# xudoong/EdgeVisionTransformer

Hardware: NVIDIA B200
Metric: images_per_sec (higher is better)
Workload: dtype bf16

## Files before the change

### edgevisiontransformer_b200/_lib.py

```python
from __future__ import annotations

import ctypes as C
import os
import threading

HERE = os.path.dirname(os.path.abspath(__file__))
LIB_PATH = os.environ.get("EVT_LIB_PATH") or os.path.join(HERE, "libevt.so")

EVT_OK, EVT_ERR_INVALID, EVT_ERR_CUDA, EVT_ERR_UNSUPPORTED, EVT_ERR_STATE = 0, -1, -2, -3, -4
EVT_F32, EVT_BF16 = 0, 1
ACT_NONE, ACT_GELU_ERF, ACT_GELU_TANH = 0, 1, 2
DIALECT_HF, DIALECT_TF = 0, 1
PREC_BF16, PREC_TF32 = 0, 1
MAX_LAYERS = 64
STAGES = ("embed", "layernorm", "qkv", "attention", "out_proj", "fc1", "fc2", "head")


class ModelSpec(C.Structure):
    _fields_ = [
        ("dialect", C.c_int), ("hidden", C.c_int), ("layers", C.c_int), ("tokens", C.c_int),
        ("image", C.c_int), ("patch", C.c_int), ("head_size", C.c_int), ("num_labels", C.c_int),
        ("act", C.c_int), ("eps", C.c_float),
        ("heads", C.c_int * MAX_LAYERS), ("inter", C.c_int * MAX_LAYERS),
        ("final_ln", C.c_int), ("head_hidden", C.c_int), ("t2t", C.c_int), ("precision", C.c_int), ("embed_k", C.c_int),
        ("head_rows", C.c_int),
    ]


class ForwardOpts(C.Structure):
    _fields_ = [("pixel_dtype", C.c_int), ("pixel_scale", C.c_float * 3), ("pixel_bias", C.c_float * 3),
                ("head_mask", C.c_void_p), ("head_mask_ld", C.c_int), ("ctx_out", C.POINTER(C.c_void_p))]


PIX_F32, PIX_BF16, PIX_U8 = 0, 1, 2


SWIN_MAX_STAGES = 8


class SwinSpec(C.Structure):
    _fields_ = [("image", C.c_int), ("patch", C.c_int), ("window", C.c_int), ("embed_dim", C.c_int), ("stages", C.c_int),
                ("depths", C.c_int * SWIN_MAX_STAGES), ("heads", C.c_int * SWIN_MAX_STAGES), ("num_labels", C.c_int),
                ("eps", C.c_float)]


class TensorView(C.Structure):
    _fields_ = [("name", C.c_char_p), ("data", C.c_void_p), ("ndim", C.c_int), ("shape", C.c_int64 * 4)]


_i, _i64, _f, _p, _sz = C.c_int, C.c_int64, C.c_float, C.c_void_p, C.c_size_t

SIGNATURES = {
    "evt_last_error": (C.c_char_p, []),
    "evt_version": (_i, []),
    "evt_device_check": (_i, []),
    "evt_launch_count": (_i64, []),
    "evt_launch_count_reset": (None, []),
    "evt_gemm_set_pair_mode": (None, [_i]),
    "evt_gemm_set_split_k": (None, [_i]),
    "evt_gemm_weights_static": (None, [_i]),
    "evt_layernorm_fwd": (_i, [_p, _i64, _p, _p, _p, _i, _i64, _p, _i64, _i, _f, _p]),
    "evt_layernorm2d_fwd": (_i, [_p, _p, _p, _p, _p, _i64, _i64, _f, _p]),
    "evt_gemm_bias_act": (_i, [_p, _i64, _p, _i64, _p, _p, _i64, _i, _i, _p, _i, _i64, _i, _i, _i, _i64, _i, _i, _i, _p]),
    "evt_gemm_bias_act_tf32": (_i, [_p, _i64, _p, _i64, _p, _p, _i64, _i, _i, _p, _i64, _i, _i, _i, _i64, _i, _i, _i, _p]),
    "evt_layernorm_gemm": (_i, [_p, _i64, _p, _p, _f, _p, _p, _i64, _p, _p, _i64, _i64, _i, _i, _i, _p]),
    "evt_gemm_residual_layernorm": (_i, [_p, _i64, _p, _i64, _p, _p, _i64, _p, _p, _f, _p, _i64, _i64, _i, _i, _p]),
    "evt_gemm_residual_layernorm_ex": (_i, [_p, _i64, _p, _i64, _p, _p, _i64, _p, _p, _f, _i, _p, _i64, _i64, _i, _i, _p]),
    "evt_attention_fwd": (_i, [_p, _i64, _p, _i64, _p, _i, _i, _i, _i, _f, _p]),
    "evt_attention_fwd_tf32": (_i, [_p, _i64, _p, _i64, _p, _i, _i, _i, _i, _f, _p]),
    "evt_attention_query_rows_fwd": (_i, [_p, _i64, _p, _i64, _p, _i, _i, _i, _i, _i, _f, _p]),
    "evt_im2col_patch": (_i, [_p, _p, _i, _i, _i, _i, _p]),
    "evt_patch_embed_workspace_bytes": (_i, [_i, _i, _i, _i, _i, C.POINTER(C.c_size_t)]),
    "evt_patch_embed_fwd": (_i, [_p, _i, _p, _p, _p, _i64, _p, _p, _p, _p, _p, _i, _i, _i, _i, _i, _i, _p]),
    "evt_prefix_tokens": (_i, [_p, _p, _p, _i, _i, _i, _i, _p]),
    "evt_cast_f32_bf16": (_i, [_p, _p, _i64, _p]),
    "evt_unfold_nhwc": (_i, [_p, _i, _p, _i64, _i, _i, _i, _i, _i, _i, _i, _p]),
    "evt_gather_layernorm": (_i, [_p, _p, _p, _p, _p, _i, _p, _i64, _i, _i, _i, _i, _f, _p]),
    "evt_window_attention_fwd": (_i, [_p, _i64, _p, _i64, _p, _i, _i64, _i, _i, _i, _f, _p]),
    "evt_layernorm_mean_tokens": (_i, [_p, _p, _p, _p, _i64, _i, _i, _f, _p]),
    "evt_model_create": (_i, [C.POINTER(ModelSpec), C.POINTER(_p)]),
    "evt_model_load_weights": (_i, [_p, C.POINTER(TensorView), _i, _p]),
    "evt_model_workspace_bytes": (_i, [_p, _i, C.POINTER(_sz)]),
    "evt_model_forward": (_i, [_p, _p, _i, _p, _p, _sz, _p]),
    "evt_model_forward_ex": (_i, [_p, _p, C.POINTER(ForwardOpts), _i, _p, _p, _sz, _p]),
    "evt_model_forward_embedded": (_i, [_p, _p, _i64, _i, _p, _p, _sz, _p]),
    "evt_unfold_ln_nhwc": (_i, [_p, _i, _p, _i64, _p, _p, _f, _i, _i, _i, _i, _i, _i, _i, _p]),
    "evt_performer_workspace_bytes": (_i, [_i, _i, C.POINTER(_sz)]),
    "evt_performer_fwd": (_i, [_p, _i64, _p, _p, _p, _p, _i, _i, _i, _i, _f, _p]),
    "evt_performer_mlp_fwd": (_i, [_p, _p, _p, _p, _p, _p, _p, _p, _p, _p, _i64, _f, _p]),
    "evt_performer_block_fwd": (_i, [_p, _i64, _p, _p, _p, _i, _i, _f, _p, _p, _p, _p, _p, _p, _p, _p, _f, _p]),
    "evt_model_launches_per_forward": (_i, [_p]),
    "evt_model_profile_begin": (_i, [_p]),
    "evt_model_profile_end": (_i, [_p, C.POINTER(_f), C.POINTER(_i)]),
    "evt_model_destroy": (_i, [_p]),
    "evt_swin_create": (_i, [C.POINTER(SwinSpec), C.POINTER(_p)]),
    "evt_swin_load_weights": (_i, [_p, C.POINTER(TensorView), _i, _p]),
    "evt_swin_workspace_bytes": (_i, [_p, _i, C.POINTER(_sz)]),
    "evt_swin_forward": (_i, [_p, _p, _i, _p, _p, _sz, _p]),
    "evt_swin_launches_per_forward": (_i, [_p]),
    "evt_swin_destroy": (_i, [_p]),
}

_lib = None
_lock = threading.Lock()


def load(build_if_missing: bool = True) -> C.CDLL:
    global _lib
    with _lock:
        if _lib is not None:
            return _lib
        if not os.path.exists(LIB_PATH):
            if not build_if_missing:
                raise RuntimeError(f"{LIB_PATH} not built; run python -m edgevisiontransformer_b200.build")
            from . import build as _build
            _build.build()
        lib = C.CDLL(LIB_PATH)
        for name, (res, args) in SIGNATURES.items():
            fn = getattr(lib, name)
            fn.restype = res
            fn.argtypes = args
        _lib = lib
        return lib


class EvtError(RuntimeError):
    pass


def check(rc: int, what: str = "") -> None:
    if rc == EVT_OK:
        return
    msg = load().evt_last_error().decode("utf-8", "replace")
    text = f"libevt {what} failed ({rc}): {msg}"
    if rc == EVT_ERR_INVALID:
        raise ValueError(text)
    raise EvtError(text)
```

### edgevisiontransformer_b200/csrc/gemm.cu

```cuda
#include "gemm_common.cuh"
#include "ops.h"

namespace evt {
namespace {

using namespace gemm_detail;

template <int BN, bool TF32, bool OUT_F32, int ACT, bool TMA_OUT>
__global__ void __launch_bounds__(kThreads, 1)
gemm_kernel(const __grid_constant__ CUtensorMap tmA, const __grid_constant__ CUtensorMap tmW,
            const __grid_constant__ CUtensorMap tmO, const GemmParams p) {
  using C = Cfg<BN>;
  extern __shared__ uint8_t smem_raw[];
  uint8_t* smem = reinterpret_cast<uint8_t*>((reinterpret_cast<uintptr_t>(smem_raw) + 1023) & ~uintptr_t(1023));
  uint8_t* stage_base = smem;
  uint8_t* staging = smem + C::kStages * C::kStageBytes;
  uint64_t* bars = reinterpret_cast<uint64_t*>(smem + C::kStages * C::kStageBytes + C::kStagingBytes);
  uint64_t* full = bars;
  uint64_t* empty = bars + C::kStages;
  uint64_t* tfull = bars + 2 * C::kStages;
  uint64_t* tempty = tfull + 2;
  uint32_t* tmem_ptr = reinterpret_cast<uint32_t*>(tempty + 2);

  const int warp = threadIdx.x >> 5;
  const int lane = threadIdx.x & 31;
  const int num_tiles = p.tiles_m * p.tiles_n * p.k_splits;

  if (warp == kProducerWarp && lane == 0) {
    ptx::prefetch_tmap(&tmA);
    ptx::prefetch_tmap(&tmW);
    if (TMA_OUT) ptx::prefetch_tmap(&tmO);
    for (int s = 0; s < C::kStages; ++s) {
      ptx::mbar_init(&full[s], 1);
      ptx::mbar_init(&empty[s], 1);
    }
    for (int s = 0; s < 2; ++s) {
      ptx::mbar_init(&tfull[s], 1);
      ptx::mbar_init(&tempty[s], kEpiWarps);
    }
    ptx::fence_mbar_init();
  }
  if (warp == kMmaWarp) ptx::tmem_alloc<C::kTmemCols>(tmem_ptr);
  ptx::tc_fence_before();
  __syncthreads();
  ptx::tc_fence_after();
  const uint32_t tmem_base = *tmem_ptr;
  ptx::grid_dep_launch();
  int w_pre = 0;
  if (p.w_static && warp == kProducerWarp && static_cast<int>(blockIdx.x) < num_tiles) {
    const int item = blockIdx.x;
    const int tile = item / p.k_splits;
    const int kb0 = (item - tile * p.k_splits) * p.kb_per_split;
    const int kb1 = min(p.num_kb, kb0 + p.kb_per_split);
    const int n0 = (tile % p.tiles_n) * BN;
    w_pre = min(C::kStages, kb1 - kb0);
    if (ptx::elect_one()) {
      for (int i = 0; i < w_pre; ++i) {
        ptx::mbar_arrive_expect_tx(&full[i], C::kStageBytes);
        ptx::tma_load_2d_hint(stage_base + i * C::kStageBytes + C::kABytes, &tmW, &full[i], (kb0 + i) * p.k_step, n0, ptx::kEvictLast);
      }
    }
  }
  ptx::grid_dep_wait();

  if (warp == kProducerWarp) {
    if (ptx::elect_one()) {
      int stage = 0;
      uint32_t phase = 0;
      for (int item = blockIdx.x; item < num_tiles; item += gridDim.x) {
        const int tile = item / p.k_splits;
        const int kb0 = (item - tile * p.k_splits) * p.kb_per_split;
        const int kb1 = min(p.num_kb, kb0 + p.kb_per_split);
        const int m0 = (tile / p.tiles_n) * BM;
        const int n0 = (tile % p.tiles_n) * BN;
        for (int kb = kb0; kb < kb1; ++kb) {
          uint8_t* sa = stage_base + stage * C::kStageBytes;
          uint8_t* sb = sa + C::kABytes;
          if (w_pre > 0) {
            --w_pre;
            ptx::tma_load_2d(sa, &tmA, &full[stage], kb * p.k_step, m0);
            if (++stage == C::kStages) {
              stage = 0;
              phase ^= 1;
            }
            continue;
          }
          ptx::mbar_wait(&empty[stage], phase ^ 1);
          ptx::mbar_arrive_expect_tx(&full[stage], C::kStageBytes);
          ptx::tma_load_2d(sa, &tmA, &full[stage], kb * p.k_step, m0);
          ptx::tma_load_2d_hint(sb, &tmW, &full[stage], kb * p.k_step, n0, ptx::kEvictLast);
          if (++stage == C::kStages) {
            stage = 0;
            phase ^= 1;
          }
        }
      }
    }
  } else if (warp == kMmaWarp) {
    if (ptx::elect_one()) {
      constexpr uint32_t idesc = ptx::make_idesc(BM, BN, TF32 ? 2 : 1, 0, 0);
      int stage = 0;
      uint32_t phase = 0;
      int as = 0;
      uint32_t aphase = 0;
      for (int item = blockIdx.x; item < num_tiles; item += gridDim.x) {
        const int kb0 = (item % p.k_splits) * p.kb_per_split;
        const int kb1 = min(p.num_kb, kb0 + p.kb_per_split);
        ptx::mbar_wait(&tempty[as], aphase ^ 1);
        ptx::tc_fence_after();
        const uint32_t d_tmem = tmem_base + as * BN;
        for (int kb = kb0; kb < kb1; ++kb) {
          ptx::mbar_wait(&full[stage], phase);
          ptx::tc_fence_after();
          const uint32_t sa = ptx::smem_u32(stage_base + stage * C::kStageBytes);
          const uint64_t adesc = ptx::smem_desc_sw128(sa);
          const uint64_t bdesc = ptx::smem_desc_sw128(sa + C::kABytes);
#pragma unroll
          for (int k = 0; k < 4; ++k) {
            const uint32_t acc = (kb != kb0 || k != 0) ? 1u : 0u;
            if (TF32) ptx::mma_tf32_ss(d_tmem, adesc + 2 * k, bdesc + 2 * k, idesc, acc);
            else ptx::mma_f16_ss(d_tmem, adesc + 2 * k, bdesc + 2 * k, idesc, acc);
          }
          ptx::mma_commit(&empty[stage]);
          if (++stage == C::kStages) {
            stage = 0;
            phase ^= 1;
          }
        }
        ptx::mma_commit(&tfull[as]);
        if (++as == 2) {
          as = 0;
          aphase ^= 1;
        }
      }
    }
  } else {
    const int quad = warp & 3;
    const int grp = warp >> 2;
    uint8_t* stg = staging + warp * kStgBytes;
    int as = 0;
    uint32_t aphase = 0;
    GemmParams pe = p;
    for (int item = blockIdx.x; item < num_tiles; item += gridDim.x) {
      const int tile = item / p.k_splits;
      pe.bias = item - tile * p.k_splits == 0 ? p.bias : nullptr;
      const int m0 = (tile / p.tiles_n) * BM + quad * 32;
      const int nt0 = (tile % p.tiles_n) * BN;
      prefetch_bias<BN, OUT_F32>(pe, grp, lane, nt0);
      ptx::mbar_wait(&tfull[as], aphase);
      ptx::tc_fence_after();
      const uint32_t t_row = tmem_base + (static_cast<uint32_t>(quad * 32) << 16) + as * BN;
      epilogue_tile<BN, TF32, OUT_F32, ACT, TMA_OUT>(pe, &tmO, stg, grp, lane, m0, nt0, t_row);
      ptx::tc_fence_before();
      __syncwarp();
      if (lane == 0) ptx::mbar_arrive(&tempty[as]);
      if (++as == 2) {
        as = 0;
        aphase ^= 1;
      }
    }
    if (TMA_OUT && ptx::elect_one()) ptx::bulk_wait<0>();
  }

  ptx::tc_fence_before();
  __syncthreads();
  if (warp == kMmaWarp) {
    ptx::tc_fence_after();
    ptx::tmem_dealloc<C::kTmemCols>(tmem_base);
  }
}

int choose_bn(int64_t M, int N) {
  const int cands[4] = {256, 192, 128, 64};
  const long tiles_m = static_cast<long>((M + BM - 1) / BM);
  int best = 256;
  long best_cost = -1;
  for (int bn : cands) {
    long cost = static_cast<long>((N + bn - 1) / bn) * bn;
    if (best_cost < 0 || cost < best_cost) {
      best_cost = cost;
      best = bn;
    }
  }
  const long sms = num_sms();
  if (tiles_m * ((N + best - 1) / best) >= sms) return best;
  long best_busy = -1;
  for (int bn : cands) {
    if (bn > best) continue;
    const long tiles = tiles_m * ((N + bn - 1) / bn);
    const long busy = tiles < sms ? tiles : sms;
    if (busy > best_busy) {
      best_busy = busy;
      best = bn;
    }
  }
  return best;
}

template <int BN, bool TF32, bool OUT_F32, int ACT, bool TMA_OUT>
int launch(const CUtensorMap& tmA, const CUtensorMap& tmW, const CUtensorMap& tmO, const GemmParams& p, cudaStream_t stream) {
  using C = Cfg<BN>;
  constexpr auto kern = gemm_kernel<BN, TF32, OUT_F32, ACT, TMA_OUT>;
  EVT_TRY(opt_in_smem<kern>(C::kSmemBytes));
  const int num_tiles = p.tiles_m * p.tiles_n * p.k_splits;
  const int grid = num_tiles < num_sms() ? num_tiles : num_sms();
  EVT_CUDA(launch_pdl(kern, dim3(grid), dim3(kThreads), C::kSmemBytes, stream, pdl_for_gemm(p.M, p.N, p.K), tmA, tmW, tmO, p));
  EVT_LAUNCH_CHECK("gemm_kernel");
  return EVT_OK;
}

template <int BN, bool TF32, bool TMA_OUT>
int dispatch_epi(const CUtensorMap& a, const CUtensorMap& w, const CUtensorMap& o, const GemmParams& p, bool out_f32, int act,
                 cudaStream_t s) {
  if (out_f32) {
    switch (act) {
      case EVT_ACT_NONE: return launch<BN, TF32, true, EVT_ACT_NONE, TMA_OUT>(a, w, o, p, s);
      case EVT_ACT_GELU_ERF: return launch<BN, TF32, true, EVT_ACT_GELU_ERF, TMA_OUT>(a, w, o, p, s);
      default: return launch<BN, TF32, true, EVT_ACT_GELU_TANH, TMA_OUT>(a, w, o, p, s);
    }
  }
  switch (act) {
    case EVT_ACT_NONE: return launch<BN, TF32, false, EVT_ACT_NONE, TMA_OUT>(a, w, o, p, s);
    case EVT_ACT_GELU_ERF: return launch<BN, TF32, false, EVT_ACT_GELU_ERF, TMA_OUT>(a, w, o, p, s);
    default: return launch<BN, TF32, false, EVT_ACT_GELU_TANH, TMA_OUT>(a, w, o, p, s);
  }
}

bool tma_out_ok(const GemmOp& op) {
  const int oeb = op.out_dtype != EVT_BF16 ? 4 : 2;
  return op.map.out_group == 0 && op.map.res_row_mod == 0 && reinterpret_cast<uintptr_t>(op.out) % 16 == 0 && (op.ldo * oeb) % 16 == 0 &&
         (op.residual == nullptr || (oeb == 4 && op.residual == reinterpret_cast<const float*>(op.out) && op.ldr == op.ldo));
}

int k_splits(const GemmOp& op, bool tma_out, long tiles, int num_kb) {
  if (op.in_dtype == EVT_F32 || !tma_out || op.residual == nullptr || gemm_pair_mode() >= 0 || !gemm_split_k_enabled()) return 1;
  if (tiles * 2 > num_sms() || num_kb < 4) return 1;
  int splits = static_cast<int>(num_sms() / tiles);
  if (splits > num_kb / 2) splits = num_kb / 2;
  if (op.max_k_splits > 0 && splits > op.max_k_splits) splits = op.max_k_splits;
  return splits > 1 ? splits : 1;
}

}

int gemm_k_splits(const GemmOp& op) {
  const int k_step = kStageRowBytes / (op.in_dtype == EVT_F32 ? 4 : 2);
  const int bn = choose_bn(op.M, op.N);
  const long tiles = static_cast<long>((op.M + BM - 1) / BM) * ((op.N + bn - 1) / bn);
  const int num_kb = (op.K + k_step - 1) / k_step;
  const int splits = k_splits(op, tma_out_ok(op), tiles, num_kb);
  if (splits == 1) return 1;
  const int kb_per_split = (num_kb + splits - 1) / splits;
  return (num_kb + kb_per_split - 1) / kb_per_split;
}

int gemm_launch(const GemmOp& op, cudaStream_t stream) {
  EVT_CHECK_ARG(op.A && op.W && op.out, "gemm: null pointer");
  EVT_CHECK_ARG(op.M > 0 && op.N > 0 && op.K > 0, "gemm: M, N, K must be positive");
  EVT_CHECK_ARG(op.M < (1ll << 31) - 256, "gemm: M too large");
  EVT_CHECK_ARG(op.in_dtype == EVT_BF16 || op.in_dtype == EVT_F32, "gemm: input dtype must be bf16 or f32(tf32)");
  EVT_CHECK_ARG(op.out_dtype == EVT_BF16 || op.out_dtype == EVT_F32 || op.out_dtype == EVT_TF32, "gemm: out dtype must be bf16, f32 or tf32");
  EVT_CHECK_ARG(!(op.out_dtype == EVT_TF32 && op.residual != nullptr), "gemm: a tf32-rounded output cannot take a residual");
  EVT_CHECK_ARG(op.act >= EVT_ACT_NONE && op.act <= EVT_ACT_GELU_TANH, "gemm: unknown activation");
  EVT_CHECK_ARG(op.lda >= op.K && op.ldw >= op.K && op.ldo >= op.N, "gemm: leading dimension smaller than the row length");
  EVT_CHECK_ARG(op.map.out_group >= 0 && op.map.res_row_mod >= 0, "gemm: negative row-group parameter");
  EVT_CHECK_ARG(op.residual == nullptr || op.ldr >= op.N, "gemm: residual leading dimension smaller than N");
  const bool tf32 = op.in_dtype == EVT_F32;
  const int eb = tf32 ? 4 : 2;
  const int k_step = kStageRowBytes / eb;
  const int bn = choose_bn(op.M, op.N);
  CUtensorMap tmA, tmW;
  int rc = make_tmap_2d(&tmA, op.A, eb, static_cast<uint64_t>(op.M), static_cast<uint64_t>(op.K), static_cast<uint64_t>(op.lda), BM, k_step);
  if (rc != EVT_OK) return rc;
  rc = make_tmap_2d(&tmW, op.W, eb, static_cast<uint64_t>(op.N), static_cast<uint64_t>(op.K), static_cast<uint64_t>(op.ldw), bn, k_step);
  if (rc != EVT_OK) return rc;
  GemmParams p;
  p.bias = op.bias;
  p.residual = op.residual;
  p.out = op.out;
  p.ldr = op.ldr;
  p.ldo = op.ldo;
  p.M = static_cast<int>(op.M);
  p.N = op.N;
  p.K = op.K;
  p.res_row_mod = op.map.res_row_mod;
  p.res_row_off = op.map.res_row_off;
  p.out_group = op.map.out_group;
  p.out_group_stride = op.map.out_group_stride;
  p.out_group_off = op.map.out_group_off;
  p.tiles_m = static_cast<int>((op.M + BM - 1) / BM);
  p.tiles_n = (op.N + bn - 1) / bn;
  p.num_kb = (op.K + k_step - 1) / k_step;
  p.k_step = k_step;
  p.w_static = gemm_weights_static() ? 1 : 0;
  {
    const int oe = op.out_dtype != EVT_BF16 ? 4 : 2;
    bool ok = reinterpret_cast<uintptr_t>(op.out) % 16 == 0 && (op.ldo * oe) % 16 == 0;
    if (op.bias) ok = ok && reinterpret_cast<uintptr_t>(op.bias) % 16 == 0;
    if (op.residual) ok = ok && reinterpret_cast<uintptr_t>(op.residual) % 16 == 0 && (op.ldr * 4) % 16 == 0;
    p.vec_ok = ok ? 1 : 0;
  }
  const bool of32 = op.out_dtype != EVT_BF16;
  p.round_tf32 = op.out_dtype == EVT_TF32 ? 1 : 0;
  const int oeb = of32 ? 4 : 2;
  const bool tma_out = tma_out_ok(op);
  CUtensorMap tmO = tmA;
  if (tma_out) {
    rc = make_tmap_2d(&tmO, op.out, oeb, static_cast<uint64_t>(op.M), static_cast<uint64_t>(op.N), static_cast<uint64_t>(op.ldo), 32,
                      128 / oeb);
    if (rc != EVT_OK) return rc;
  }
  p.k_splits = 1;
  p.kb_per_split = p.num_kb;
  const int splits = k_splits(op, tma_out, static_cast<long>(p.tiles_m) * p.tiles_n, p.num_kb);
  if (splits > 1) {
    p.kb_per_split = (p.num_kb + splits - 1) / splits;
    p.k_splits = (p.num_kb + p.kb_per_split - 1) / p.kb_per_split;
  }
  if (!tf32 && tma_out && pair_supported(bn)) {
    const int pair_mode = gemm_pair_mode();
    const long pair_tiles = static_cast<long>((op.M + 2 * BM - 1) / (2 * BM)) * p.tiles_n;
    const bool use_pair = pair_mode < 0 ? pair_tiles >= num_sms() : pair_mode != 0;
    if (use_pair) return gemm_pair_launch(bn, op.W, op.ldw, tmA, tmO, p, of32, op.act, stream);
  }
#define EVT_BN_CASE(BNV)                                                                                      \
  case BNV:                                                                                                   \
    if (tma_out)                                                                                              \
      return tf32 ? dispatch_epi<BNV, true, true>(tmA, tmW, tmO, p, of32, op.act, stream)                     \
                  : dispatch_epi<BNV, false, true>(tmA, tmW, tmO, p, of32, op.act, stream);                   \
    return tf32 ? dispatch_epi<BNV, true, false>(tmA, tmW, tmO, p, of32, op.act, stream)                      \
                : dispatch_epi<BNV, false, false>(tmA, tmW, tmO, p, of32, op.act, stream);
  switch (bn) {
    EVT_BN_CASE(256)
    EVT_BN_CASE(192)
    EVT_BN_CASE(128)
    EVT_BN_CASE(64)
  }
#undef EVT_BN_CASE
  return fail(EVT_ERR_INVALID, "gemm: no tile configuration");
}

}

extern "C" int evt_gemm_bias_act(const void* A, int64_t lda, const void* W, int64_t ldw, const float* bias,
                                 const float* residual, int64_t ldr, int res_row_mod, int res_row_off, void* out,
                                 int out_dtype, int64_t ldo, int out_group, int out_group_stride, int out_group_off,
                                 int64_t M, int N, int K, int act, evt_stream stream) {
  int rc = evt_device_check();
  if (rc != EVT_OK) return rc;
  return evt::gemm_launch({.A = A, .lda = lda, .W = W, .ldw = ldw, .in_dtype = EVT_BF16, .bias = bias, .residual = residual, .ldr = ldr,
                           .out = out, .out_dtype = out_dtype, .ldo = ldo, .M = M, .N = N, .K = K, .act = act,
                           .map = {.res_row_mod = res_row_mod, .res_row_off = res_row_off, .out_group = out_group, .out_group_stride = out_group_stride,
                                    .out_group_off = out_group_off}}, static_cast<cudaStream_t>(stream));
}

extern "C" int evt_gemm_bias_act_tf32(const float* A, int64_t lda, const float* W, int64_t ldw, const float* bias,
                                      const float* residual, int64_t ldr, int res_row_mod, int res_row_off, float* out,
                                      int64_t ldo, int out_group, int out_group_stride, int out_group_off, int64_t M,
                                      int N, int K, int act, evt_stream stream) {
  int rc = evt_device_check();
  if (rc != EVT_OK) return rc;
  return evt::gemm_launch({.A = A, .lda = lda, .W = W, .ldw = ldw, .in_dtype = EVT_F32, .bias = bias, .residual = residual, .ldr = ldr,
                           .out = out, .out_dtype = EVT_F32, .ldo = ldo, .M = M, .N = N, .K = K, .act = act,
                           .map = {.res_row_mod = res_row_mod, .res_row_off = res_row_off, .out_group = out_group, .out_group_stride = out_group_stride,
                                    .out_group_off = out_group_off}}, static_cast<cudaStream_t>(stream));
}
```

### edgevisiontransformer_b200/csrc/gemm2.cu

```cuda
#include <stdio.h>
#include <stdlib.h>

#include "gemm_common.cuh"
#include "ops.h"

namespace evt {
namespace {

using namespace gemm_detail;

template <int BN, int EW>
struct Cfg2 {
  static constexpr int kABytes = BM * kStageRowBytes;
  static constexpr int kBBytes = (BN / 2) * kStageRowBytes;
  static constexpr int kStageBytes = kABytes + kBBytes;
  static constexpr int kStagingBytes = EW * kStgBytes;
  static constexpr int kMaxStages = (232448 - 1024 - kStagingBytes - 256) / kStageBytes;
  static constexpr int kStages = kMaxStages < (BN == 128 ? 8 : 6) ? kMaxStages : (BN == 128 ? 8 : 6);
  static constexpr int kTmemCols = BN == 128 ? 256 : 512;
  static constexpr int kProducer = EW, kMma = EW + 1, kThreadsCta = 32 * (EW + 2);
  static constexpr int kBarBytes = (2 * kStages + 4) * 8 + 16;
  static constexpr int kSmemBytes = 1024  + kStages * kStageBytes + kStagingBytes + kBarBytes;
  static_assert(kSmemBytes <= 232448, "exceeds the 227 KB of shared memory a CTA can opt in to");
};

template <int BN, bool OUT_F32, int ACT, int EW>
__global__ void __cluster_dims__(2, 1, 1) __launch_bounds__(32 * (EW + 2), 1)
gemm_pair_kernel(const __grid_constant__ CUtensorMap tmA, const __grid_constant__ CUtensorMap tmW,
                 const __grid_constant__ CUtensorMap tmO, const GemmParams p) {
  using C = Cfg2<BN, EW>;
  constexpr int kProducerWarp = C::kProducer, kMmaWarp = C::kMma, kEpiWarps = EW;
  extern __shared__ uint8_t smem_raw[];
  uint8_t* smem = reinterpret_cast<uint8_t*>((reinterpret_cast<uintptr_t>(smem_raw) + 1023) & ~uintptr_t(1023));
  uint8_t* stage_base = smem;
  uint8_t* staging = smem + C::kStages * C::kStageBytes;
  uint64_t* bars = reinterpret_cast<uint64_t*>(smem + C::kStages * C::kStageBytes + C::kStagingBytes);
  uint64_t* full = bars;
  uint64_t* empty = bars + C::kStages;
  uint64_t* tfull = bars + 2 * C::kStages;
  uint64_t* tempty = tfull + 2;
  uint32_t* tmem_ptr = reinterpret_cast<uint32_t*>(tempty + 2);

  const int warp = threadIdx.x >> 5;
  const int lane = threadIdx.x & 31;
  const uint32_t rank = ptx::cluster_ctarank();
  const int pair = blockIdx.x >> 1;
  const int num_pairs = gridDim.x >> 1;
  const int num_tiles = p.tiles_m * p.tiles_n;

  if (warp == kProducerWarp && lane == 0) {
    ptx::prefetch_tmap(&tmA);
    ptx::prefetch_tmap(&tmW);
    ptx::prefetch_tmap(&tmO);
    for (int s = 0; s < C::kStages; ++s) {
      ptx::mbar_init(&full[s], 1);
      ptx::mbar_init(&empty[s], 1);
    }
    for (int s = 0; s < 2; ++s) {
      ptx::mbar_init(&tfull[s], 1);
      ptx::mbar_init(&tempty[s], 2 * kEpiWarps);
    }
    ptx::fence_mbar_init();
  }
  if (warp == kMmaWarp) ptx::tmem_alloc_pair<C::kTmemCols>(tmem_ptr);
  ptx::tc_fence_before();
  __syncthreads();
  ptx::cluster_sync();
  ptx::tc_fence_after();
  const uint32_t tmem_base = *tmem_ptr;
  ptx::grid_dep_launch();
  int w_pre = 0;
  if (p.w_static && warp == kProducerWarp && pair < num_tiles) {
    const int n0 = (pair % p.tiles_n) * BN + static_cast<int>(rank) * (BN / 2);
    w_pre = min(C::kStages, p.num_kb);
    if (ptx::elect_one()) {
      for (int i = 0; i < w_pre; ++i) {
        if (rank == 0) ptx::mbar_arrive_expect_tx(&full[i], 2 * C::kStageBytes);
        ptx::tma_load_2d_pair(stage_base + i * C::kStageBytes + C::kABytes, &tmW, ptx::mapa(&full[i], 0), i * p.k_step, n0, ptx::kEvictLast);
      }
    }
  }
  ptx::grid_dep_wait();

  if (warp == kProducerWarp) {
    if (ptx::elect_one()) {
      int stage = 0;
      uint32_t phase = 0;
      for (int tile = pair; tile < num_tiles; tile += num_pairs) {
        const int m0 = (tile / p.tiles_n) * (2 * BM) + static_cast<int>(rank) * BM;
        const int n0 = (tile % p.tiles_n) * BN + static_cast<int>(rank) * (BN / 2);
        for (int kb = 0; kb < p.num_kb; ++kb) {
          uint8_t* sa = stage_base + stage * C::kStageBytes;
          uint8_t* sb = sa + C::kABytes;
          const uint32_t lead_full = ptx::mapa(&full[stage], 0);
          if (w_pre > 0) {
            --w_pre;
            ptx::tma_load_2d_pair(sa, &tmA, lead_full, kb * p.k_step, m0, ptx::kEvictNormal);
          } else {
            ptx::mbar_wait(&empty[stage], phase ^ 1);
            if (rank == 0) ptx::mbar_arrive_expect_tx(&full[stage], 2 * C::kStageBytes);
            ptx::tma_load_2d_pair(sa, &tmA, lead_full, kb * p.k_step, m0, ptx::kEvictNormal);
            ptx::tma_load_2d_pair(sb, &tmW, lead_full, kb * p.k_step, n0, ptx::kEvictLast);
          }
          if (++stage == C::kStages) {
            stage = 0;
            phase ^= 1;
          }
        }
      }
    }
  } else if (warp == kMmaWarp) {
    if (rank == 0 && ptx::elect_one()) {
      constexpr uint32_t idesc = ptx::make_idesc(2 * BM, BN, 1, 0, 0);
      int stage = 0;
      uint32_t phase = 0;
      int as = 0;
      uint32_t aphase = 0;
      for (int tile = pair; tile < num_tiles; tile += num_pairs) {
        ptx::mbar_wait(&tempty[as], aphase ^ 1);
        ptx::tc_fence_after();
        const uint32_t d_tmem = tmem_base + as * BN;
        for (int kb = 0; kb < p.num_kb; ++kb) {
          ptx::mbar_wait(&full[stage], phase);
          ptx::tc_fence_after();
          const uint32_t sa = ptx::smem_u32(stage_base + stage * C::kStageBytes);
          const uint64_t adesc = ptx::smem_desc_sw128(sa);
          const uint64_t bdesc = ptx::smem_desc_sw128(sa + C::kABytes);
#pragma unroll
          for (int k = 0; k < 4; ++k)
            ptx::mma_f16_ss_pair(d_tmem, adesc + 2 * k, bdesc + 2 * k, idesc, (kb | k) != 0 ? 1u : 0u);
          ptx::mma_commit_pair(&empty[stage], 3);
          if (++stage == C::kStages) {
            stage = 0;
            phase ^= 1;
          }
        }
        ptx::mma_commit_pair(&tfull[as], 3);
        if (++as == 2) {
          as = 0;
          aphase ^= 1;
        }
      }
    }
  } else {
    const int quad = warp & 3;
    uint8_t* stg = staging + warp * kStgBytes;
    int as = 0;
    uint32_t aphase = 0;
    constexpr int kGroups = EW / 4;
    constexpr bool kRotate = ((BN / (OUT_F32 ? 32 : 64)) % kGroups) != 0;
    const int grp0 = warp >> 2;
    int rot = 0;
    for (int tile = pair; tile < num_tiles; tile += num_pairs) {
      const int m0 = (tile / p.tiles_n) * (2 * BM) + static_cast<int>(rank) * BM + quad * 32;
      const int nt0 = (tile % p.tiles_n) * BN;
      int grp = grp0;
      if (kRotate) {
        grp = grp0 + rot;
        if (grp >= kGroups) grp -= kGroups;
        if (++rot == kGroups) rot = 0;
      }
      prefetch_bias<BN, OUT_F32, EW / 4>(p, grp, lane, nt0);
      ptx::mbar_wait(&tfull[as], aphase);
      ptx::tc_fence_after();
      const uint32_t t_row = tmem_base + (static_cast<uint32_t>(quad * 32) << 16) + as * BN;
      epilogue_tile<BN, false, OUT_F32, ACT, true, EW / 4>(p, &tmO, stg, grp, lane, m0, nt0, t_row);
      ptx::tc_fence_before();
      __syncwarp();
      if (lane == 0) ptx::mbar_arrive_cluster(ptx::mapa(&tempty[as], 0));
      if (++as == 2) {
        as = 0;
        aphase ^= 1;
      }
    }
    if (ptx::elect_one()) ptx::bulk_wait<0>();
  }

  ptx::tc_fence_before();
  __syncthreads();
  ptx::cluster_sync();
  if (warp == kMmaWarp) {
    ptx::tc_fence_after();
    ptx::tmem_dealloc_pair<C::kTmemCols>(tmem_base);
  }
}

template <int BN, bool OUT_F32, int ACT, int EW>
int launch_pair_ew(const void* W, int64_t ldw, const CUtensorMap& tmA, const CUtensorMap& tmO, GemmParams p, cudaStream_t stream) {
  using C = Cfg2<BN, EW>;
  constexpr int kThreads = C::kThreadsCta;
  constexpr auto kern = gemm_pair_kernel<BN, OUT_F32, ACT, EW>;
  EVT_TRY(opt_in_smem<kern>(C::kSmemBytes));
  static int pairs_dev = -1;
  static int max_pairs = 0;
  int dev = 0;
  EVT_CUDA(cudaGetDevice(&dev));
  if (pairs_dev != dev) {
    cudaLaunchConfig_t cfg = {};
    cfg.gridDim = dim3(num_sms() & ~1, 1, 1);
    cfg.blockDim = dim3(kThreads, 1, 1);
    cfg.dynamicSmemBytes = C::kSmemBytes;
    int n = 0;
    EVT_CUDA(cudaOccupancyMaxActiveClusters(&n, kern, &cfg));
    if (n <= 0) return fail(EVT_ERR_CUDA, "gemm: no CTA pair of this configuration fits on the device");
    max_pairs = n;
    if (getenv("EVT_DEBUG")) fprintf(stderr, "evt: gemm_pair_kernel<%d> max active clusters %d, smem %d\n", BN, n, C::kSmemBytes);
    pairs_dev = dev;
  }
  CUtensorMap tmW;
  int rc = make_tmap_2d(&tmW, W, 2, static_cast<uint64_t>(p.N), static_cast<uint64_t>(p.K), static_cast<uint64_t>(ldw), BN / 2,
                        p.k_step);
  if (rc != EVT_OK) return rc;
  p.tiles_m = (p.M + 2 * BM - 1) / (2 * BM);
  const int num_tiles = p.tiles_m * p.tiles_n;
  const int pairs = num_tiles < max_pairs ? num_tiles : max_pairs;
  EVT_CUDA(launch_pdl(kern, dim3(2 * pairs), dim3(kThreads), C::kSmemBytes, stream, pdl_for_gemm(p.M, p.N, p.K), tmA, tmW, tmO, p));
  EVT_LAUNCH_CHECK("gemm_pair_kernel");
  return EVT_OK;
}

template <int BN, bool OUT_F32, int ACT>
int launch_pair(const void* W, int64_t ldw, const CUtensorMap& tmA, const CUtensorMap& tmO, const GemmParams& p, cudaStream_t stream) {
  if constexpr (ACT != EVT_ACT_NONE && !OUT_F32) {
    if (p.K <= 384) return launch_pair_ew<BN, OUT_F32, ACT, 16>(W, ldw, tmA, tmO, p, stream);
    return launch_pair_ew<BN, OUT_F32, ACT, 8>(W, ldw, tmA, tmO, p, stream);
  } else {
    return launch_pair_ew<BN, OUT_F32, ACT, 8>(W, ldw, tmA, tmO, p, stream);
  }
}

template <int BN>
int dispatch_pair(const void* W, int64_t ldw, const CUtensorMap& a, const CUtensorMap& o, const GemmParams& p, bool out_f32,
                  int act, cudaStream_t s) {
  if (out_f32) {
    switch (act) {
      case EVT_ACT_NONE: return launch_pair<BN, true, EVT_ACT_NONE>(W, ldw, a, o, p, s);
      case EVT_ACT_GELU_ERF: return launch_pair<BN, true, EVT_ACT_GELU_ERF>(W, ldw, a, o, p, s);
      default: return launch_pair<BN, true, EVT_ACT_GELU_TANH>(W, ldw, a, o, p, s);
    }
  }
  switch (act) {
    case EVT_ACT_NONE: return launch_pair<BN, false, EVT_ACT_NONE>(W, ldw, a, o, p, s);
    case EVT_ACT_GELU_ERF: return launch_pair<BN, false, EVT_ACT_GELU_ERF>(W, ldw, a, o, p, s);
    default: return launch_pair<BN, false, EVT_ACT_GELU_TANH>(W, ldw, a, o, p, s);
  }
}

}

namespace gemm_detail {

bool pair_supported(int bn) { return bn == 256 || bn == 192 || bn == 128; }

int gemm_pair_launch(int bn, const void* W, int64_t ldw, const CUtensorMap& tmA, const CUtensorMap& tmO, const GemmParams& p,
                     bool out_f32, int act, cudaStream_t stream) {
  switch (bn) {
    case 256: return dispatch_pair<256>(W, ldw, tmA, tmO, p, out_f32, act, stream);
    case 192: return dispatch_pair<192>(W, ldw, tmA, tmO, p, out_f32, act, stream);
    case 128: return dispatch_pair<128>(W, ldw, tmA, tmO, p, out_f32, act, stream);
  }
  return fail(EVT_ERR_INVALID, "gemm: no CTA-pair tile configuration");
}

}
}
```

### edgevisiontransformer_b200/csrc/gemm_common.cuh

```cuda
#pragma once
#include <cuda_bf16.h>

#include "common.h"
#include "ptx.cuh"

namespace evt {
namespace gemm_detail {


constexpr int BM = 128;
constexpr int kStageRowBytes = 128;
constexpr int kEpiWarps = 8;
constexpr int kProducerWarp = kEpiWarps;
constexpr int kMmaWarp = kEpiWarps + 1;
constexpr int kThreads = 32 * (kEpiWarps + 2);
constexpr int kStgBytes = 32 * 128;

template <int BN>
struct Cfg {
  static constexpr int kABytes = BM * kStageRowBytes;
  static constexpr int kBBytes = BN * kStageRowBytes;
  static constexpr int kStageBytes = kABytes + kBBytes;
  static constexpr int kStages = BN == 256 ? 4 : BN == 192 ? 4 : BN == 128 ? 6 : 8;
  static constexpr int kTmemCols = BN == 256 ? 512 : BN == 192 ? 512 : BN == 128 ? 256 : 128;
  static constexpr int kStagingBytes = kEpiWarps * kStgBytes;
  static constexpr int kBarBytes = (2 * kStages + 4) * 8 + 16;
  static constexpr int kSmemBytes = 1024  + kStages * kStageBytes + kStagingBytes + kBarBytes;
  static_assert(kSmemBytes <= 232448, "exceeds the 227 KB of shared memory a CTA can opt in to");
};

struct GemmParams {
  const float* bias;
  const float* residual;
  void* out;
  long long ldr, ldo;
  int M, N, K;
  int res_row_mod, res_row_off;
  int out_group, out_group_stride, out_group_off;
  int tiles_m, tiles_n, num_kb;
  int k_splits, kb_per_split;
  int k_step;
  int vec_ok;
  int round_tf32;
  int w_static;
};

__device__ __forceinline__ long long map_out_row(const GemmParams& p, long long row) {
  if (p.out_group <= 0) return row;
  const long long g = row / p.out_group;
  return g * p.out_group_stride + p.out_group_off + (row - g * p.out_group);
}
__device__ __forceinline__ uint32_t pack_bf16x2(float a, float b) {
  __nv_bfloat162 h = __floats2bfloat162_rn(a, b);
  return *reinterpret_cast<uint32_t*>(&h);
}

__device__ __forceinline__ float ex2_approx(float x) {
  float y;
  asm("ex2.approx.ftz.f32 %0, %1;" : "=f"(y) : "f"(x));
  return y;
}
__device__ __forceinline__ float rcp_approx(float x) {
  float y;
  asm("rcp.approx.ftz.f32 %0, %1;" : "=f"(y) : "f"(x));
  return y;
}

__device__ __forceinline__ uint64_t pk2(float lo, float hi) {
  uint64_t r;
  asm("mov.b64 %0, {%1, %2};" : "=l"(r) : "f"(lo), "f"(hi));
  return r;
}
__device__ __forceinline__ void upk2(uint64_t v, float& lo, float& hi) {
  asm("mov.b64 {%0, %1}, %2;" : "=f"(lo), "=f"(hi) : "l"(v));
}
__device__ __forceinline__ uint64_t fma2(uint64_t a, uint64_t b, uint64_t c) {
  uint64_t d;
  asm("fma.rn.f32x2 %0, %1, %2, %3;" : "=l"(d) : "l"(a), "l"(b), "l"(c));
  return d;
}
__device__ __forceinline__ uint64_t mul2(uint64_t a, uint64_t b) {
  uint64_t d;
  asm("mul.rn.f32x2 %0, %1, %2;" : "=l"(d) : "l"(a), "l"(b));
  return d;
}
__device__ __forceinline__ uint64_t add2(uint64_t a, uint64_t b) {
  uint64_t d;
  asm("add.rn.f32x2 %0, %1, %2;" : "=l"(d) : "l"(a), "l"(b));
  return d;
}

template <bool HI>
__device__ __forceinline__ void gelu_erf_pair(float& x0, float& x1) {
  constexpr float kAmax = 5.65685424949238f;
  const uint64_t a = pk2(fminf(fabsf(x0), kAmax), fminf(fabsf(x1), kAmax));
  uint64_t q;
  if (HI) {
    q = fma2(a, pk2(-1.765649017e-06f, -1.765649017e-06f), pk2(6.025074981e-05f, 6.025074981e-05f));
    q = fma2(q, a, pk2(-9.201008943e-04f, -9.201008943e-04f));
    q = fma2(q, a, pk2(8.467212319e-03f, 8.467212319e-03f));
    q = fma2(q, a, pk2(-5.387612060e-02f, -5.387612060e-02f));
    q = fma2(q, a, pk2(-4.585517347e-01f, -4.585517347e-01f));
    q = fma2(q, a, pk2(-1.151212096e+00f, -1.151212096e+00f));
  } else {
    q = fma2(a, pk2(2.554092680e-05f, 2.554092680e-05f), pk2(-6.528479280e-04f, -6.528479280e-04f));
    q = fma2(q, a, pk2(7.452332415e-03f, 7.452332415e-03f));
    q = fma2(q, a, pk2(-5.191940814e-02f, -5.191940814e-02f));
    q = fma2(q, a, pk2(-4.602991641e-01f, -4.602991641e-01f));
    q = fma2(q, a, pk2(-1.150684714e+00f, -1.150684714e+00f));
  }
  float t0, t1;
  upk2(fma2(q, a, pk2(-1.0f, -1.0f)), t0, t1);
  const float e0 = ex2_approx(t0), e1 = ex2_approx(t1);
  x0 = fmaf(-fabsf(x0), e0, fmaxf(x0, 0.0f));
  x1 = fmaf(-fabsf(x1), e1, fmaxf(x1, 0.0f));
}
__device__ __forceinline__ void gelu_tanh_pair(float& x0, float& x1) {
  constexpr float k0 = -2.0f * 1.4426950408889634f * 0.7978845608028654f;
  constexpr float k1 = k0 * 0.044715f;
  const uint64_t x = pk2(x0, x1);
  const uint64_t w = fma2(mul2(x, x), pk2(k1, k1), pk2(k0, k0));
  float t0, t1;
  upk2(mul2(x, w), t0, t1);
  x0 *= rcp_approx(1.0f + ex2_approx(t0));
  x1 *= rcp_approx(1.0f + ex2_approx(t1));
}
template <int ACT, bool EXACT, bool HI>
__device__ __forceinline__ void apply_act_pair(float& x0, float& x1) {
  if (ACT == EVT_ACT_GELU_ERF) {
    if (EXACT) {
      x0 = 0.5f * x0 * (1.0f + erff(x0 * 0.70710678118654752f));
      x1 = 0.5f * x1 * (1.0f + erff(x1 * 0.70710678118654752f));
    } else {
      gelu_erf_pair<HI>(x0, x1);
    }
  } else if (ACT == EVT_ACT_GELU_TANH) {
    if (EXACT) {
      x0 = 0.5f * x0 * (1.0f + tanhf(0.7978845608028654f * (x0 + 0.044715f * x0 * x0 * x0)));
      x1 = 0.5f * x1 * (1.0f + tanhf(0.7978845608028654f * (x1 + 0.044715f * x1 * x1 * x1)));
    } else {
      gelu_tanh_pair(x0, x1);
    }
  }
}
template <int CH, int ACT, bool EXACT, bool HI>
__device__ __forceinline__ void bias_act(float (&v)[CH], const float* __restrict__ bias, int n0, int N, bool full) {
  if (bias != nullptr) {
    if (full) {
      const float4* b4 = reinterpret_cast<const float4*>(bias + n0);
#pragma unroll
      for (int i = 0; i < CH / 4; ++i) {
        const float4 b = __ldg(b4 + i);
        upk2(add2(pk2(v[4 * i], v[4 * i + 1]), pk2(b.x, b.y)), v[4 * i], v[4 * i + 1]);
        upk2(add2(pk2(v[4 * i + 2], v[4 * i + 3]), pk2(b.z, b.w)), v[4 * i + 2], v[4 * i + 3]);
      }
    } else {
#pragma unroll
      for (int j = 0; j < CH; ++j)
        if (n0 + j < N) v[j] += __ldg(bias + n0 + j);
    }
  }
  if (ACT != EVT_ACT_NONE) {
#pragma unroll
    for (int j = 0; j < CH; j += 2) apply_act_pair<ACT, EXACT, HI>(v[j], v[j + 1]);
  }
}


template <int BN, bool OUT_F32, int NGRP = 2>
__device__ __forceinline__ void prefetch_bias(const GemmParams& p, int grp, int lane, int nt0) {
  constexpr int CH = OUT_F32 ? 32 : 64;
  constexpr int NCH = BN / CH;
  if (p.bias == nullptr) return;
  constexpr int kLinesPerChunk = CH / 32;
  const int k = lane / kLinesPerChunk;
  const int c = grp + NGRP * k;
  const int col = nt0 + c * CH + (lane % kLinesPerChunk) * 32;
  if (c < NCH && col < p.N) asm volatile("prefetch.global.L1 [%0];" ::"l"(p.bias + col));
}

template <int BN, bool TF32, bool OUT_F32, int ACT, bool TMA_OUT, int NGRP = 2>
__device__ __forceinline__ void epilogue_tile(const GemmParams& p, const CUtensorMap* tmO, uint8_t* stg, int grp, int lane,
                                              int m0, int nt0, uint32_t t_row) {
  constexpr int CH = OUT_F32 ? 32 : 64;
  constexpr int NCH = BN / CH;
  const int sw = lane & 7;
  const bool has_res = p.residual != nullptr;
  const int rows_here = min(32, p.M - m0);
  float4 rnext[8];
  auto load_res = [&](int n0c) {
#pragma unroll
    for (int it = 0; it < 8; ++it) {
      const int rr = it * 4 + (lane >> 3);
      rnext[it] = make_float4(0.f, 0.f, 0.f, 0.f);
      if (rr < rows_here && p.vec_ok && n0c + CH <= p.N) {
        const long long row = m0 + rr;
        const long long rrow = p.res_row_mod > 0 ? p.res_row_off + row % p.res_row_mod : map_out_row(p, row);
        rnext[it] = *reinterpret_cast<const float4*>(p.residual + rrow * p.ldr + n0c + (lane & 7) * 4);
      }
    }
  };
  if constexpr (OUT_F32 && !TMA_OUT) {
    if (has_res && grp < NCH) load_res(nt0 + grp * CH);
  }
  if (rows_here > 0) {
#pragma unroll 1
    for (int c = grp; c < NCH; c += NGRP) {
      const int n0 = nt0 + c * CH;
      if (n0 >= p.N) break;
      float v[CH];
      {
        uint32_t r[32];
        ptx::tmem_ld_x32(t_row + c * CH, r);
        if constexpr (CH == 64) {
          uint32_t r2[32];
          ptx::tmem_ld_x32(t_row + c * CH + 32, r2);
          ptx::tmem_ld_wait();
#pragma unroll
          for (int j = 0; j < 32; ++j) v[32 + j] = __uint_as_float(r2[j]);
        } else {
          ptx::tmem_ld_wait();
        }
#pragma unroll
        for (int j = 0; j < 32; ++j) v[j] = __uint_as_float(r[j]);
      }
      const bool full = p.vec_ok && (n0 + CH <= p.N);
      float4 rcur[8];
      if constexpr (OUT_F32 && !TMA_OUT) {
        if (has_res) {
#pragma unroll
          for (int it = 0; it < 8; ++it) rcur[it] = rnext[it];
          if (c + NGRP < NCH && n0 + NGRP * CH < p.N) load_res(n0 + NGRP * CH);
        }
      }
      bias_act<CH, ACT, TF32, OUT_F32>(v, p.bias, n0, p.N, full);
      if constexpr (OUT_F32) {
        if (p.round_tf32) {
#pragma unroll
          for (int j = 0; j < CH; ++j) v[j] = ptx::round_tf32(v[j]);
        }
      }
      if constexpr (!OUT_F32) if (has_res && lane < rows_here) {
        const long long orow = map_out_row(p, m0 + lane);
        const long long rrow = p.res_row_mod > 0 ? p.res_row_off + (m0 + lane) % p.res_row_mod : orow;
#pragma unroll
        for (int j = 0; j < CH; ++j)
          if (n0 + j < p.N) v[j] += p.residual[rrow * p.ldr + n0 + j];
      }
      if constexpr (TMA_OUT) {
        if (ptx::elect_one()) ptx::bulk_wait_read<0>();
      }
      __syncwarp();
      const uint32_t sb = ptx::smem_u32(stg) + lane * 128;
      if constexpr (OUT_F32) {
#pragma unroll
        for (int i = 0; i < 8; ++i) ptx::sts_f4(sb + ((i ^ sw) << 4), v[4 * i], v[4 * i + 1], v[4 * i + 2], v[4 * i + 3]);
      } else {
#pragma unroll
        for (int i = 0; i < 8; ++i)
          ptx::sts_u4(sb + ((i ^ sw) << 4), pack_bf16x2(v[8 * i], v[8 * i + 1]), pack_bf16x2(v[8 * i + 2], v[8 * i + 3]),
                      pack_bf16x2(v[8 * i + 4], v[8 * i + 5]), pack_bf16x2(v[8 * i + 6], v[8 * i + 7]));
      }
      if constexpr (TMA_OUT) {
        ptx::fence_proxy_async_smem();
        __syncwarp();
        if (ptx::elect_one()) {
          if (has_res) ptx::tma_reduce_add_2d(tmO, stg, n0, m0);
          else ptx::tma_store_2d(tmO, stg, n0, m0);
          ptx::bulk_commit();
        }
        continue;
      }
      __syncwarp();
      const int piece = lane & 7;
#pragma unroll
      for (int it = 0; it < 8; ++it) {
        const int rr = it * 4 + (lane >> 3);
        if (rr < rows_here) {
          const long long row = m0 + rr;
          const long long orow = map_out_row(p, row);
          const uint8_t* src = stg + rr * 128 + ((piece ^ (rr & 7)) << 4);
          if constexpr (OUT_F32) {
            float4 val = *reinterpret_cast<const float4*>(src);
            const int col = n0 + piece * 4;
            float* dst = reinterpret_cast<float*>(p.out) + orow * p.ldo + col;
            if (full) {
              if (has_res) {
                const float4 rs = rcur[it];
                val.x += rs.x;
                val.y += rs.y;
                val.z += rs.z;
                val.w += rs.w;
              }
              *reinterpret_cast<float4*>(dst) = val;
            } else {
              const float e[4] = {val.x, val.y, val.z, val.w};
              const long long rrow = p.res_row_mod > 0 ? p.res_row_off + row % p.res_row_mod : orow;
#pragma unroll
              for (int q = 0; q < 4; ++q)
                if (col + q < p.N) dst[q] = e[q] + (has_res ? p.residual[rrow * p.ldr + col + q] : 0.f);
            }
          } else {
            const uint4 val = *reinterpret_cast<const uint4*>(src);
            const int col = n0 + piece * 8;
            __nv_bfloat16* dst = reinterpret_cast<__nv_bfloat16*>(p.out) + orow * p.ldo + col;
            if (full) {
              *reinterpret_cast<uint4*>(dst) = val;
            } else {
              const uint32_t e[4] = {val.x, val.y, val.z, val.w};
#pragma unroll
              for (int q = 0; q < 8; ++q)
                if (col + q < p.N) {
                  const uint16_t h = static_cast<uint16_t>(e[q >> 1] >> ((q & 1) * 16));
                  reinterpret_cast<uint16_t*>(dst)[q] = h;
                }
            }
          }
        }
      }
    }
  }
}

bool pair_supported(int bn);
int gemm_pair_launch(int bn, const void* W, int64_t ldw, const CUtensorMap& tmA, const CUtensorMap& tmO, const GemmParams& p,
                     bool out_f32, int act, cudaStream_t stream);

}
}
```

### edgevisiontransformer_b200/csrc/layernorm.cu

```cuda
#include <cuda_bf16.h>

#include "common.h"
#include "ptx.cuh"

namespace evt {
namespace {

constexpr int kMaxVec = 16;

__device__ __forceinline__ float warp_sum(float v) {
#pragma unroll
  for (int o = 16; o > 0; o >>= 1) v += __shfl_xor_sync(0xffffffffu, v, o);
  return v;
}

template <int NV, int OUT>
__global__ void __launch_bounds__(256) ln_rows_kernel(const float* x, long long x_stride,
                                                      const float* __restrict__ gamma, const float* __restrict__ beta,
                                                      void* __restrict__ y, long long y_stride, float* y_copy,
                                                      long long rows, int D, float eps) {
  ptx::grid_dep_launch();
  ptx::grid_dep_wait();
  const int lane = threadIdx.x & 31;
  const long long row = static_cast<long long>(blockIdx.x) * (blockDim.x >> 5) + (threadIdx.x >> 5);
  if (row >= rows) return;
  const float* xr = x + row * x_stride;
  float2 v[NV];
  float s = 0.f;
#pragma unroll
  for (int i = 0; i < NV; ++i) {
    const int c = i * 64 + lane * 2;
    if (c < D) {
      v[i] = *reinterpret_cast<const float2*>(xr + c);
      s += v[i].x + v[i].y;
    } else {
      v[i] = make_float2(0.f, 0.f);
    }
  }
  const float mean = warp_sum(s) / static_cast<float>(D);
  float q = 0.f;
#pragma unroll
  for (int i = 0; i < NV; ++i) {
    const int c = i * 64 + lane * 2;
    if (c < D) {
      const float a = v[i].x - mean, b = v[i].y - mean;
      q += a * a + b * b;
    }
  }
  const float rstd = rsqrtf(warp_sum(q) / static_cast<float>(D) + eps);
#pragma unroll
  for (int i = 0; i < NV; ++i) {
    const int c = i * 64 + lane * 2;
    if (c < D) {
      const float2 g = *reinterpret_cast<const float2*>(gamma + c);
      const float2 b = *reinterpret_cast<const float2*>(beta + c);
      float o0 = (v[i].x - mean) * rstd * g.x + b.x;
      float o1 = (v[i].y - mean) * rstd * g.y + b.y;
      if (y_copy != nullptr) *reinterpret_cast<float2*>(y_copy + row * x_stride + c) = make_float2(o0, o1);
      if (OUT == EVT_TF32) {
        o0 = ptx::round_tf32(o0);
        o1 = ptx::round_tf32(o1);
      }
      if (OUT == EVT_BF16) {
        __nv_bfloat162 h = __floats2bfloat162_rn(o0, o1);
        *reinterpret_cast<__nv_bfloat162*>(reinterpret_cast<__nv_bfloat16*>(y) + row * y_stride + c) = h;
      } else {
        *reinterpret_cast<float2*>(reinterpret_cast<float*>(y) + row * y_stride + c) = make_float2(o0, o1);
      }
    }
  }
}

template <int NV, int OUT, bool PRE = false>
__global__ void __launch_bounds__(256) ln_rows4_kernel(const float* x, long long x_stride,
                                                       const float* __restrict__ gamma, const float* __restrict__ beta,
                                                       void* __restrict__ y, long long y_stride, float* y_copy,
                                                       long long rows, int D, float eps) {
  ptx::grid_dep_launch();
  const int lane = threadIdx.x & 31;
  float4 gpre[PRE ? NV : 1], bpre[PRE ? NV : 1];
  if (PRE) {
#pragma unroll
    for (int i = 0; i < NV; ++i) {
      const int c = i * 128 + lane * 4;
      if (c < D) {
        gpre[i] = __ldg(reinterpret_cast<const float4*>(gamma + c));
        bpre[i] = __ldg(reinterpret_cast<const float4*>(beta + c));
      }
    }
  }
  ptx::grid_dep_wait();
  const long long row = static_cast<long long>(blockIdx.x) * (blockDim.x >> 5) + (threadIdx.x >> 5);
  if (row >= rows) return;
  const float* xr = x + row * x_stride;
  float4 v[NV];
  float s = 0.f;
#pragma unroll
  for (int i = 0; i < NV; ++i) {
    const int c = i * 128 + lane * 4;
    v[i] = make_float4(0.f, 0.f, 0.f, 0.f);
    if (c < D) {
      asm volatile("ld.global.L1::no_allocate.v4.f32 {%0, %1, %2, %3}, [%4];"
                   : "=f"(v[i].x), "=f"(v[i].y), "=f"(v[i].z), "=f"(v[i].w)
                   : "l"(xr + c));
      s += (v[i].x + v[i].y) + (v[i].z + v[i].w);
    }
  }
  const float mean = warp_sum(s) / static_cast<float>(D);
  float q = 0.f;
#pragma unroll
  for (int i = 0; i < NV; ++i) {
    const int c = i * 128 + lane * 4;
    if (c < D) {
      const float a0 = v[i].x - mean, a1 = v[i].y - mean, a2 = v[i].z - mean, a3 = v[i].w - mean;
      q += (a0 * a0 + a1 * a1) + (a2 * a2 + a3 * a3);
    }
  }
  const float rstd = rsqrtf(warp_sum(q) / static_cast<float>(D) + eps);
#pragma unroll
  for (int i = 0; i < NV; ++i) {
    const int c = i * 128 + lane * 4;
    if (c < D) {
      const float4 g = PRE ? gpre[i] : __ldg(reinterpret_cast<const float4*>(gamma + c));
      const float4 b = PRE ? bpre[i] : __ldg(reinterpret_cast<const float4*>(beta + c));
      float o0 = (v[i].x - mean) * rstd * g.x + b.x;
      float o1 = (v[i].y - mean) * rstd * g.y + b.y;
      float o2 = (v[i].z - mean) * rstd * g.z + b.z;
      float o3 = (v[i].w - mean) * rstd * g.w + b.w;
      if (y_copy != nullptr) *reinterpret_cast<float4*>(y_copy + row * x_stride + c) = make_float4(o0, o1, o2, o3);
      if (OUT == EVT_TF32) {
        o0 = ptx::round_tf32(o0);
        o1 = ptx::round_tf32(o1);
        o2 = ptx::round_tf32(o2);
        o3 = ptx::round_tf32(o3);
      }
      if (OUT == EVT_BF16) {
        __nv_bfloat162 h0 = __floats2bfloat162_rn(o0, o1), h1 = __floats2bfloat162_rn(o2, o3);
        uint2 w;
        w.x = *reinterpret_cast<uint32_t*>(&h0);
        w.y = *reinterpret_cast<uint32_t*>(&h1);
        *reinterpret_cast<uint2*>(reinterpret_cast<__nv_bfloat16*>(y) + row * y_stride + c) = w;
      } else {
        *reinterpret_cast<float4*>(reinterpret_cast<float*>(y) + row * y_stride + c) = make_float4(o0, o1, o2, o3);
      }
    }
  }
}

template <int LPR, int NV, int OUT>
__global__ void __launch_bounds__(256) ln_rows4_sub_kernel(const float* x, long long x_stride, const float* __restrict__ gamma,
                                                           const float* __restrict__ beta, void* __restrict__ y,
                                                           long long y_stride, float* y_copy, long long rows, float eps) {
  ptx::grid_dep_launch();
  ptx::grid_dep_wait();
  constexpr int D = 4 * LPR * NV;
  constexpr int RPW = 32 / LPR;
  const int lane = threadIdx.x & 31;
  const int sub = lane / LPR, l = lane % LPR;
  const long long row = (static_cast<long long>(blockIdx.x) * (blockDim.x >> 5) + (threadIdx.x >> 5)) * RPW + sub;
  const bool live = row < rows;
  const float* xr = x + (live ? row : 0) * x_stride;
  float4 v[NV];
  float s = 0.f;
#pragma unroll
  for (int i = 0; i < NV; ++i) {
    const int c = (i * LPR + l) * 4;
    asm volatile("ld.global.L1::no_allocate.v4.f32 {%0, %1, %2, %3}, [%4];"
                 : "=f"(v[i].x), "=f"(v[i].y), "=f"(v[i].z), "=f"(v[i].w)
                 : "l"(xr + c));
    s += (v[i].x + v[i].y) + (v[i].z + v[i].w);
  }
#pragma unroll
  for (int o = LPR / 2; o > 0; o >>= 1) s += __shfl_xor_sync(0xffffffffu, s, o);
  const float mean = s / static_cast<float>(D);
  float q = 0.f;
#pragma unroll
  for (int i = 0; i < NV; ++i) {
    const float a0 = v[i].x - mean, a1 = v[i].y - mean, a2 = v[i].z - mean, a3 = v[i].w - mean;
    q += (a0 * a0 + a1 * a1) + (a2 * a2 + a3 * a3);
  }
#pragma unroll
  for (int o = LPR / 2; o > 0; o >>= 1) q += __shfl_xor_sync(0xffffffffu, q, o);
  const float rstd = rsqrtf(q / static_cast<float>(D) + eps);
  if (!live) return;
#pragma unroll
  for (int i = 0; i < NV; ++i) {
    const int c = (i * LPR + l) * 4;
    const float4 g = __ldg(reinterpret_cast<const float4*>(gamma + c));
    const float4 b = __ldg(reinterpret_cast<const float4*>(beta + c));
    float o0 = (v[i].x - mean) * rstd * g.x + b.x;
    float o1 = (v[i].y - mean) * rstd * g.y + b.y;
    float o2 = (v[i].z - mean) * rstd * g.z + b.z;
    float o3 = (v[i].w - mean) * rstd * g.w + b.w;
    if (y_copy != nullptr) *reinterpret_cast<float4*>(y_copy + row * x_stride + c) = make_float4(o0, o1, o2, o3);
    if (OUT == EVT_TF32) {
      o0 = ptx::round_tf32(o0);
      o1 = ptx::round_tf32(o1);
      o2 = ptx::round_tf32(o2);
      o3 = ptx::round_tf32(o3);
    }
    if (OUT == EVT_BF16) {
      __nv_bfloat162 h0 = __floats2bfloat162_rn(o0, o1), h1 = __floats2bfloat162_rn(o2, o3);
      uint2 w;
      w.x = *reinterpret_cast<uint32_t*>(&h0);
      w.y = *reinterpret_cast<uint32_t*>(&h1);
      *reinterpret_cast<uint2*>(reinterpret_cast<__nv_bfloat16*>(y) + row * y_stride + c) = w;
    } else {
      *reinterpret_cast<float4*>(reinterpret_cast<float*>(y) + row * y_stride + c) = make_float4(o0, o1, o2, o3);
    }
  }
}

template <int OUT>
__global__ void __launch_bounds__(256) ln_rows_generic_kernel(const float* x, long long x_stride,
                                                              const float* __restrict__ gamma,
                                                              const float* __restrict__ beta, void* __restrict__ y,
                                                              long long y_stride, float* y_copy, long long rows, int D,
                                                              float eps) {
  ptx::grid_dep_launch();
  ptx::grid_dep_wait();
  const int lane = threadIdx.x & 31;
  const long long row = static_cast<long long>(blockIdx.x) * (blockDim.x >> 5) + (threadIdx.x >> 5);
  if (row >= rows) return;
  const float* xr = x + row * x_stride;
  float s = 0.f;
  for (int c = lane; c < D; c += 32) s += xr[c];
  const float mean = warp_sum(s) / static_cast<float>(D);
  float q = 0.f;
  for (int c = lane; c < D; c += 32) {
    const float a = xr[c] - mean;
    q += a * a;
  }
  const float rstd = rsqrtf(warp_sum(q) / static_cast<float>(D) + eps);
  for (int c = lane; c < D; c += 32) {
    float o = (xr[c] - mean) * rstd * gamma[c] + beta[c];
    if (y_copy != nullptr) y_copy[row * x_stride + c] = o;
    if (OUT == EVT_TF32) o = ptx::round_tf32(o);
    if (OUT == EVT_BF16) reinterpret_cast<__nv_bfloat16*>(y)[row * y_stride + c] = __float2bfloat16_rn(o);
    else reinterpret_cast<float*>(y)[row * y_stride + c] = o;
  }
}

__global__ void __launch_bounds__(1024) ln2d_kernel(const float* __restrict__ x, const float* __restrict__ addend,
                                                    const float* __restrict__ gamma, const float* __restrict__ beta,
                                                    float* __restrict__ y, long long nh, float eps) {
  __shared__ float red[32];
  __shared__ float stat;
  const long long base = static_cast<long long>(blockIdx.x) * nh;
  const int tid = threadIdx.x, lane = tid & 31, warp = tid >> 5, nwarp = blockDim.x >> 5;
  auto block_sum = [&](float v) -> float {
    v = warp_sum(v);
    if (lane == 0) red[warp] = v;
    __syncthreads();
    if (warp == 0) {
      float t = lane < nwarp ? red[lane] : 0.f;
      t = warp_sum(t);
      if (lane == 0) stat = t;
    }
    __syncthreads();
    const float r = stat;
    __syncthreads();
    return r;
  };
  float s = 0.f;
  for (long long i = tid; i < nh; i += blockDim.x) s += x[base + i] + (addend ? addend[base + i] : 0.f);
  const float mean = block_sum(s) / static_cast<float>(nh);
  float q = 0.f;
  for (long long i = tid; i < nh; i += blockDim.x) {
    const float a = x[base + i] + (addend ? addend[base + i] : 0.f) - mean;
    q += a * a;
  }
  const float rstd = rsqrtf(block_sum(q) / static_cast<float>(nh) + eps);
  for (long long i = tid; i < nh; i += blockDim.x) {
    const float a = x[base + i] + (addend ? addend[base + i] : 0.f);
    y[base + i] = (a - mean) * rstd * gamma[i] + beta[i];
  }
}

template <int OUT>
int launch_rows(const float* x, long long xs, const float* g, const float* b, void* y, long long ys, float* yc,
                long long rows, int D, float eps, cudaStream_t st) {
  constexpr int wpb = 4;
  const unsigned grid = static_cast<unsigned>((rows + wpb - 1) / wpb);
  const bool fast = (D % 2 == 0) && D <= 64 * kMaxVec && (xs % 2 == 0) && (ys % 2 == 0) &&
                    (reinterpret_cast<uintptr_t>(x) % 8 == 0) && (reinterpret_cast<uintptr_t>(y) % 8 == 0) &&
                    (reinterpret_cast<uintptr_t>(g) % 8 == 0) && (reinterpret_cast<uintptr_t>(b) % 8 == 0) &&
                    (yc == nullptr || reinterpret_cast<uintptr_t>(yc) % 8 == 0);
  const bool fast4 = (D % 4 == 0) && D <= 1024 && (xs % 4 == 0) && (ys % 4 == 0) &&
                     (reinterpret_cast<uintptr_t>(x) % 16 == 0) && (reinterpret_cast<uintptr_t>(y) % 16 == 0) &&
                     (reinterpret_cast<uintptr_t>(g) % 16 == 0) && (reinterpret_cast<uintptr_t>(b) % 16 == 0) &&
                     (yc == nullptr || reinterpret_cast<uintptr_t>(yc) % 16 == 0);
  int lpr = 0, nvs = 0;
  if (fast4 && D == 64) lpr = 16, nvs = 1;
  else if (fast4 && D == 96) lpr = 8, nvs = 3;
  else if (fast4 && D == 192) lpr = 16, nvs = 3;
  if (lpr != 0) {
    const int rpw = 32 / lpr;
    const unsigned gsub = static_cast<unsigned>((rows + wpb * rpw - 1) / (wpb * rpw));
    if (D == 64)
      EVT_CUDA(launch_pdl(ln_rows4_sub_kernel<16, 1, OUT>, dim3(gsub), dim3(wpb * 32), 0, st, pdl_for_work(rows, D), x, xs, g, b, y, ys, yc, rows, eps));
    else if (D == 96)
      EVT_CUDA(launch_pdl(ln_rows4_sub_kernel<8, 3, OUT>, dim3(gsub), dim3(wpb * 32), 0, st, pdl_for_work(rows, D), x, xs, g, b, y, ys, yc, rows, eps));
    else
      EVT_CUDA(launch_pdl(ln_rows4_sub_kernel<16, 3, OUT>, dim3(gsub), dim3(wpb * 32), 0, st, pdl_for_work(rows, D), x, xs, g, b, y, ys, yc, rows, eps));
  } else if (fast4) {
    const int nv = (D + 127) / 128;
#define EVT_LN4_CASE(NVV)                                                                          \
  case NVV:                                                                                        \
    if (rows <= 4096)                                                                              \
      EVT_CUDA(launch_pdl(ln_rows4_kernel<NVV, OUT, true>, dim3(grid), dim3(wpb * 32), 0, st, pdl_for_work(rows, D), x, xs, g, b, y, ys, yc, rows, D, eps)); \
    else                                                                                           \
      EVT_CUDA(launch_pdl(ln_rows4_kernel<NVV, OUT>, dim3(grid), dim3(wpb * 32), 0, st, pdl_for_work(rows, D), x, xs, g, b, y, ys, yc, rows, D, eps)); \
    break;
    switch (nv) {
      EVT_LN4_CASE(1) EVT_LN4_CASE(2) EVT_LN4_CASE(3) EVT_LN4_CASE(4) EVT_LN4_CASE(5) EVT_LN4_CASE(6) EVT_LN4_CASE(7)
      EVT_LN4_CASE(8)
    }
#undef EVT_LN4_CASE
  } else if (!fast) {
    EVT_CUDA(launch_pdl(ln_rows_generic_kernel<OUT>, dim3(grid), dim3(wpb * 32), 0, st, pdl_for_work(rows, D), x, xs, g, b, y, ys, yc, rows, D, eps));
  } else {
    const int nv = (D + 63) / 64;
#define EVT_LN_CASE(NVV)                                                                          \
  case NVV:                                                                                       \
    EVT_CUDA(launch_pdl(ln_rows_kernel<NVV, OUT>, dim3(grid), dim3(wpb * 32), 0, st, pdl_for_work(rows, D), x, xs, g, b, y, ys, yc, rows, D, eps)); \
    break;
    switch (nv) {
      EVT_LN_CASE(1) EVT_LN_CASE(2) EVT_LN_CASE(3) EVT_LN_CASE(4) EVT_LN_CASE(5) EVT_LN_CASE(6) EVT_LN_CASE(7)
      EVT_LN_CASE(8) EVT_LN_CASE(9) EVT_LN_CASE(10) EVT_LN_CASE(11) EVT_LN_CASE(12) EVT_LN_CASE(13) EVT_LN_CASE(14)
      EVT_LN_CASE(15) EVT_LN_CASE(16)
    }
#undef EVT_LN_CASE
  }
  EVT_LAUNCH_CHECK("layernorm");
  return EVT_OK;
}

}

int layernorm_launch(const float* x, int64_t x_stride, const float* gamma, const float* beta, void* y, int y_dtype,
                     int64_t y_stride, float* y_copy, int64_t rows, int D, float eps, cudaStream_t st) {
  EVT_CHECK_ARG(x && gamma && beta && y, "layernorm: null pointer");
  EVT_CHECK_ARG(rows > 0 && D > 0, "layernorm: rows and D must be positive");
  EVT_CHECK_ARG(x_stride >= D && y_stride >= D, "layernorm: stride smaller than D");
  EVT_CHECK_ARG(y_dtype == EVT_BF16 || y_dtype == EVT_F32 || y_dtype == EVT_TF32, "layernorm: y dtype must be bf16, f32 or tf32");
  EVT_CHECK_ARG(eps >= 0.f, "layernorm: negative eps");
  if (y_dtype == EVT_BF16) return launch_rows<EVT_BF16>(x, x_stride, gamma, beta, y, y_stride, y_copy, rows, D, eps, st);
  if (y_dtype == EVT_TF32) return launch_rows<EVT_TF32>(x, x_stride, gamma, beta, y, y_stride, y_copy, rows, D, eps, st);
  return launch_rows<EVT_F32>(x, x_stride, gamma, beta, y, y_stride, y_copy, rows, D, eps, st);
}

}

extern "C" int evt_layernorm_fwd(const float* x, int64_t x_stride, const float* gamma, const float* beta, void* y,
                                 int y_dtype, int64_t y_stride, float* y_copy_f32, int64_t rows, int D, float eps,
                                 evt_stream stream) {
  int rc = evt_device_check();
  if (rc != EVT_OK) return rc;
  return evt::layernorm_launch(x, x_stride, gamma, beta, y, y_dtype, y_stride, y_copy_f32, rows, D, eps,
                               static_cast<cudaStream_t>(stream));
}

extern "C" int evt_layernorm2d_fwd(const float* x, const float* addend, const float* gamma, const float* beta, float* y,
                                   int64_t batch, int64_t nh, float eps, evt_stream stream) {
  int rc = evt_device_check();
  if (rc != EVT_OK) return rc;
  EVT_CHECK_ARG(x && gamma && beta && y, "layernorm2d: null pointer");
  EVT_CHECK_ARG(batch > 0 && nh > 0, "layernorm2d: batch and nh must be positive");
  evt::ln2d_kernel<<<static_cast<unsigned>(batch), 1024, 0, static_cast<cudaStream_t>(stream)>>>(x, addend, gamma, beta,
                                                                                                 y, nh, eps);
  EVT_LAUNCH_CHECK("layernorm2d");
  return EVT_OK;
}
```

### edgevisiontransformer_b200/csrc/loader.h

```cpp
#pragma once
#include <cuda_bf16.h>

#include <map>
#include <string>
#include <vector>

#include "common.h"

namespace evt {

struct Loader {
  std::vector<void*>* allocs;
  cudaStream_t st;
  int es;
  std::map<std::string, const evt_tensor_view*> by_name = {};

  int index(const evt_tensor_view* tensors, int n);
  const evt_tensor_view* find(const std::string& name) const;
  int need(const std::string& name, int64_t n, const evt_tensor_view** out) const;
  int alloc(size_t bytes, void** out);
  int vec_into(const std::string& name, int64_t n, bool optional, float* dst);
  int vec(const std::string& name, int64_t n, bool optional, float** out);
  int mat_into(const std::string& name, int64_t rows, int cols, int ld, void* dst);
  template <typename T>
  int mat(const std::string& name, int64_t rows, int cols, int ld, T** out) {
    void* p;
    EVT_TRY(alloc(static_cast<size_t>(rows) * ld * es, &p));
    *out = static_cast<T*>(p);
    return mat_into(name, rows, cols, ld, p);
  }
  int mat_t(const std::string& name, int rows_out, int cols_out, int ld, __nv_bfloat16** out);
  template <typename T>
  int upload(const std::vector<T>& h, T** out) {
    void* p;
    EVT_TRY(alloc(h.size() * sizeof(T), &p));
    EVT_CUDA(cudaMemcpyAsync(p, h.data(), h.size() * sizeof(T), cudaMemcpyHostToDevice, st));
    EVT_CUDA(cudaStreamSynchronize(st));
    *out = static_cast<T*>(p);
    return EVT_OK;
  }
  int host_copy(const std::string& name, int64_t n, std::vector<float>* out);
};

}
```

### edgevisiontransformer_b200/csrc/model.cu

```cuda
#include <cuda_bf16.h>

#include <string>
#include <vector>

#include "loader.h"
#include "ops.h"
#include "ptx.cuh"

namespace evt {
namespace {

__device__ __forceinline__ void store_as(__nv_bfloat16* p, float v) { *p = __float2bfloat16_rn(v); }
__device__ __forceinline__ void store_as(float* p, float v) { *p = ptx::round_tf32(v); }

template <typename T>
__global__ void __launch_bounds__(256) convert_pad_kernel(const float* __restrict__ src, T* __restrict__ dst, long long rows,
                                                          int cols, int ld) {
  const long long t = static_cast<long long>(blockIdx.x) * blockDim.x + threadIdx.x;
  if (t >= rows * ld) return;
  const int c = static_cast<int>(t % ld);
  const long long r = t / ld;
  store_as(dst + t, c < cols ? src[r * cols + c] : 0.f);
}

__global__ void __launch_bounds__(256) convert_pad_transposed_kernel(const float* __restrict__ src, __nv_bfloat16* __restrict__ dst,
                                                                     int rows_out, int cols_out, int ld) {
  const long long t = static_cast<long long>(blockIdx.x) * blockDim.x + threadIdx.x;
  if (t >= static_cast<long long>(rows_out) * ld) return;
  const int c = static_cast<int>(t % ld);
  const int r = static_cast<int>(t / ld);
  dst[t] = __float2bfloat16_rn(c < cols_out ? src[static_cast<long long>(c) * rows_out + r] : 0.f);
}

template <typename T>
__global__ void __launch_bounds__(256) gather_rows_cast_kernel(const float* __restrict__ x, long long x_stride,
                                                               T* __restrict__ y, long long rows, int D) {
  ptx::grid_dep_launch();
  ptx::grid_dep_wait();
  const long long t = static_cast<long long>(blockIdx.x) * blockDim.x + threadIdx.x;
  if (t >= rows * D) return;
  const int c = static_cast<int>(t % D);
  const long long r = t / D;
  store_as(y + t, x[r * x_stride + c]);
}

inline int padn(int v, int n) { return (v + n - 1) / n * n; }

struct LayerW {
  uint8_t *wqkv = nullptr, *wo = nullptr, *w1 = nullptr, *w2 = nullptr;
  float *bqkv = nullptr, *bo = nullptr, *b1 = nullptr, *b2 = nullptr;
  float *ln1_g = nullptr, *ln1_b = nullptr, *ln2_g = nullptr, *ln2_b = nullptr;
  int a = 0, inter = 0, inter_ld = 0;
};

struct PerformerW {
  int in_dim = 0, in_ld = 0;
  float *g1 = nullptr, *b1 = nullptr;
  __nv_bfloat16 *wkqv = nullptr, *wo = nullptr, *w1 = nullptr, *w2 = nullptr;
  float *bkqv = nullptr, *w = nullptr, *bo = nullptr, *g2 = nullptr, *b2 = nullptr, *bb1 = nullptr, *bb2 = nullptr;
};

}
}

struct evt_model {
  evt_model_spec spec;
  int device = 0;
  bool loaded = false;
  int patches = 0, n_prefix = 0, patch_k = 0;
  int es = 2;
  int pad = 8;
  std::vector<evt::LayerW> layers;
  uint8_t* w_patch = nullptr;
  float* b_patch = nullptr;
  float* prefix = nullptr;
  float* pos = nullptr;
  float *lnf_g = nullptr, *lnf_b = nullptr;
  uint8_t* w_pre = nullptr;
  float* b_pre = nullptr;
  uint8_t* w_cls = nullptr;
  float* b_cls = nullptr;
  evt::PerformerW perf[2];
  std::vector<void*> allocs;
  bool profiling = false;
  std::vector<cudaEvent_t> prof_events;
  size_t prof_used = 0;
  std::vector<std::pair<int, std::pair<size_t, size_t>>> prof_spans;
};

namespace evt {
namespace {

struct Workspace {
  float* resid;
  uint8_t *xn, *qkv, *ctx, *big, *clsn, *hh;
  uint8_t *t_x[2], *t_kqv[2], *t_ws[2], *t_pm;
  float* t_y[2];
  size_t bytes;
};

inline int t2t_side(int image, int stage) {
  int s = (image + 2 * 2 - 7) / 4 + 1;
  for (int i = 0; i < stage; ++i) s = (s + 2 * 1 - 3) / 2 + 1;
  return s;
}

Workspace plan_workspace(const evt_model* m, int batch, uint8_t* base) {
  const evt_model_spec& s = m->spec;
  const size_t M = static_cast<size_t>(batch) * s.tokens;
  const size_t Mp = static_cast<size_t>(batch) * m->patches;
  int amax = 0, imax_ld = 0;
  for (int l = 0; l < s.layers; ++l) {
    amax = std::max(amax, s.heads[l] * s.head_size);
    imax_ld = std::max(imax_ld, padn(s.inter[l], m->pad));
  }
  WorkspaceCarver c{base};
  Workspace w;
  const size_t es = m->es;
  w.resid = c.take<float>(M * s.hidden * 4);
  w.xn = c.take(M * s.hidden * es);
  w.qkv = c.take(M * 3 * amax * es);
  w.ctx = c.take(M * amax * es);
  w.big = c.take(std::max(M * imax_ld, (s.embed_k > 0 ? Mp : M) * static_cast<size_t>(m->patch_k)) * es);
  w.clsn = c.take(static_cast<size_t>(batch) * s.hidden * (s.head_rows > 1 ? s.head_rows : 1) * es);
  w.hh = c.take(static_cast<size_t>(batch) * std::max(padn(s.head_hidden, m->pad), 8) * es);
  if (s.t2t) {
    for (int i = 0; i < 2; ++i) {
      const size_t T = static_cast<size_t>(t2t_side(s.image, i)) * t2t_side(s.image, i) * batch;
      const size_t in_ld = i == 0 ? 152 : 576;
      w.t_x[i] = c.take(T * in_ld * 2);
      w.t_kqv[i] = c.take(T * 192 * 2);
      w.t_y[i] = c.take<float>(T * 64 * 4);
      w.t_ws[i] = c.take(performer_workspace_bytes(batch, t2t_side(s.image, i) * t2t_side(s.image, i)));
    }
    w.t_pm = c.take(Mp * 576 * 2);
  }
  w.bytes = c.bytes;
  return w;
}

int validate_spec(const evt_model_spec* s) {
  EVT_CHECK_ARG(s != nullptr, "model spec is null");
  EVT_CHECK_ARG(s->dialect == EVT_DIALECT_HF || s->dialect == EVT_DIALECT_TF, "unknown dialect");
  EVT_CHECK_ARG(s->hidden > 0 && s->hidden % 8 == 0, "hidden size must be a positive multiple of 8");
  EVT_CHECK_ARG(s->layers > 0 && s->layers <= EVT_MAX_LAYERS, "layer count out of range");
  EVT_CHECK_ARG(s->patch > 0 && s->image > 0 && s->image % s->patch == 0, "image size must be a multiple of the patch size");
  EVT_CHECK_ARG(s->patch % 8 == 0, "patch size must be a multiple of 8");
  const int patches = (s->image / s->patch) * (s->image / s->patch);
  EVT_CHECK_ARG(s->tokens == patches + 1 || s->tokens == patches + 2, "tokens must be patches + 1 (cls) or + 2 (cls, distillation)");
  if (s->tokens > EVT_ATTN_MAX_TOKENS)
    return fail(EVT_ERR_UNSUPPORTED, "more than " + std::to_string(EVT_ATTN_MAX_TOKENS) + " tokens per image is not implemented");
  if (s->tokens > 256 && s->precision == EVT_PREC_TF32)
    return fail(EVT_ERR_UNSUPPORTED, "the tf32 mode supports at most 256 tokens per image; use the bf16 mode");
  if (s->head_size != 64) return fail(EVT_ERR_UNSUPPORTED, "only head size 64 is implemented");
  EVT_CHECK_ARG(s->num_labels > 0, "num_labels must be positive");
  EVT_CHECK_ARG(s->act == EVT_ACT_GELU_ERF || s->act == EVT_ACT_GELU_TANH, "FFN activation must be erf- or tanh-GELU");
  EVT_CHECK_ARG(s->eps > 0.f, "LayerNorm eps must be positive");
  EVT_CHECK_ARG(s->head_hidden >= 0, "head_hidden must be >= 0");
  EVT_CHECK_ARG(s->head_rows >= 0 && s->head_rows <= 2, "head_rows must be 0 / 1 (cls row) or 2 (cls + distillation rows)");
  if (s->head_rows == 2)
    EVT_CHECK_ARG(s->tokens == patches + 2 && s->final_ln != 0 && s->head_hidden == 0,
                  "head_rows = 2 (two-head distilled DeiT) needs 198 tokens, the final LayerNorm and a single Linear head");
  EVT_CHECK_ARG(s->precision == EVT_PREC_BF16 || s->precision == EVT_PREC_TF32, "precision must be bf16 (0) or tf32 (1)");
  EVT_CHECK_ARG(s->embed_k >= 0 && s->embed_k % 8 == 0, "embed_k must be a non-negative multiple of 8");
  if (s->t2t) {
    EVT_CHECK_ARG(s->embed_k == 576 && s->precision == EVT_PREC_BF16, "the T2T front-end needs embed_k = 576 (3 x 3 x 64) and the bf16 mode");
    EVT_CHECK_ARG(t2t_side(s->image, 2) * t2t_side(s->image, 2) == patches, "image size does not give image/16 squared T2T tokens");
  }
  for (int l = 0; l < s->layers; ++l) {
    EVT_CHECK_ARG(s->heads[l] > 0, "every layer must keep at least one head");
    EVT_CHECK_ARG(s->inter[l] > 0, "every layer must keep at least one FFN unit");
  }
  return EVT_OK;
}

}

int Loader::index(const evt_tensor_view* tensors, int n) {
  for (int i = 0; i < n; ++i) {
    EVT_CHECK_ARG(tensors[i].name != nullptr, "tensor view without a name");
    EVT_CHECK_ARG(tensors[i].ndim >= 1 && tensors[i].ndim <= 4, "tensor view rank must be 1..4");
    by_name[tensors[i].name] = &tensors[i];
  }
  return EVT_OK;
}

const evt_tensor_view* Loader::find(const std::string& name) const {
  auto it = by_name.find(name);
  return it == by_name.end() ? nullptr : it->second;
}

int Loader::need(const std::string& name, int64_t n, const evt_tensor_view** out) const {
  const evt_tensor_view* v = find(name);
  if (!v) return fail(EVT_ERR_INVALID, "missing weight '" + name + "'");
  if (!v->data) return fail(EVT_ERR_INVALID, "weight '" + name + "' has a null data pointer");
  int64_t numel = 1;
  for (int i = 0; i < v->ndim; ++i) numel *= v->shape[i];
  if (numel != n)
    return fail(EVT_ERR_INVALID, "weight '" + name + "' has " + std::to_string(numel) + " elements, expected " + std::to_string(n));
  *out = v;
  return EVT_OK;
}

int Loader::alloc(size_t bytes, void** out) {
  void* p = nullptr;
  cudaError_t e = cudaMalloc(&p, std::max<size_t>(bytes, 16));
  if (e != cudaSuccess) return fail(EVT_ERR_CUDA, std::string("cudaMalloc: ") + cudaGetErrorString(e));
  allocs->push_back(p);
  *out = p;
  return EVT_OK;
}

int Loader::vec_into(const std::string& name, int64_t n, bool optional, float* dst) {
  const evt_tensor_view* v = find(name);
  if (!v && optional) {
    EVT_CUDA(cudaMemsetAsync(dst, 0, n * 4, st));
  } else {
    EVT_TRY(need(name, n, &v));
    EVT_CUDA(cudaMemcpyAsync(dst, v->data, n * 4, cudaMemcpyDeviceToDevice, st));
  }
  return EVT_OK;
}

int Loader::vec(const std::string& name, int64_t n, bool optional, float** out) {
  void* p;
  EVT_TRY(alloc(n * 4, &p));
  *out = static_cast<float*>(p);
  return vec_into(name, n, optional, *out);
}

int Loader::mat_into(const std::string& name, int64_t rows, int cols, int ld, void* dst) {
  const evt_tensor_view* v;
  EVT_TRY(need(name, rows * cols, &v));
  const long long total = rows * ld;
  const unsigned grid = static_cast<unsigned>((total + 255) / 256);
  const float* src = static_cast<const float*>(v->data);
  if (es == 2) convert_pad_kernel<<<grid, 256, 0, st>>>(src, static_cast<__nv_bfloat16*>(dst), rows, cols, ld);
  else convert_pad_kernel<<<grid, 256, 0, st>>>(src, static_cast<float*>(dst), rows, cols, ld);
  cudaError_t e = cudaGetLastError();
  if (e != cudaSuccess) return fail(EVT_ERR_CUDA, std::string("convert_pad: ") + cudaGetErrorString(e));
  return EVT_OK;
}

int Loader::mat_t(const std::string& name, int rows_out, int cols_out, int ld, __nv_bfloat16** out) {
  const evt_tensor_view* v;
  EVT_TRY(need(name, static_cast<int64_t>(rows_out) * cols_out, &v));
  void* p;
  EVT_TRY(alloc(static_cast<size_t>(rows_out) * ld * 2, &p));
  *out = static_cast<__nv_bfloat16*>(p);
  const long long total = static_cast<long long>(rows_out) * ld;
  convert_pad_transposed_kernel<<<static_cast<unsigned>((total + 255) / 256), 256, 0, st>>>(static_cast<const float*>(v->data), *out,
                                                                                             rows_out, cols_out, ld);
  cudaError_t e = cudaGetLastError();
  if (e != cudaSuccess) return fail(EVT_ERR_CUDA, std::string("convert_pad_transposed: ") + cudaGetErrorString(e));
  return EVT_OK;
}

int Loader::host_copy(const std::string& name, int64_t n, std::vector<float>* out) {
  const evt_tensor_view* v;
  EVT_TRY(need(name, n, &v));
  out->resize(n);
  EVT_CUDA(cudaMemcpyAsync(out->data(), v->data, n * 4, cudaMemcpyDeviceToHost, st));
  EVT_CUDA(cudaStreamSynchronize(st));
  return EVT_OK;
}

}

using namespace evt;

extern "C" int evt_model_create(const evt_model_spec* spec, evt_model** out) {
  int rc = evt_device_check();
  if (rc != EVT_OK) return rc;
  EVT_CHECK_ARG(out != nullptr, "evt_model_create: out is null");
  rc = validate_spec(spec);
  if (rc != EVT_OK) return rc;
  evt_model* m = new evt_model();
  m->spec = *spec;
  cudaGetDevice(&m->device);
  m->patches = (spec->image / spec->patch) * (spec->image / spec->patch);
  m->n_prefix = spec->tokens - m->patches;
  m->patch_k = spec->embed_k > 0 ? spec->embed_k : 3 * spec->patch * spec->patch;
  m->es = spec->precision == EVT_PREC_TF32 ? 4 : 2;
  m->pad = 16 / m->es;
  m->layers.resize(spec->layers);
  *out = m;
  return EVT_OK;
}

extern "C" int evt_model_destroy(evt_model* m) {
  if (!m) return EVT_OK;
  for (void* p : m->allocs) cudaFree(p);
  for (cudaEvent_t ev : m->prof_events) cudaEventDestroy(ev);
  delete m;
  return EVT_OK;
}

extern "C" int evt_model_load_weights(evt_model* m, const evt_tensor_view* tensors, int n, evt_stream stream) {
  EVT_CHECK_ARG(m != nullptr && tensors != nullptr && n > 0, "evt_model_load_weights: bad arguments");
  if (m->loaded) return fail(EVT_ERR_STATE, "weights already loaded; create a new model to reload");
  const evt_model_spec& s = m->spec;
  Loader L{&m->allocs, static_cast<cudaStream_t>(stream), m->es};
  EVT_TRY(L.index(tensors, n));
  const int D = s.hidden;
  const std::string e = "vit.embeddings.";
  EVT_TRY(L.mat(e + "patch_embeddings.projection.weight", D, m->patch_k, m->patch_k, &m->w_patch));
  EVT_TRY(L.vec(e + "patch_embeddings.projection.bias", D, false, &m->b_patch));
  EVT_TRY(L.vec(e + "position_embeddings", static_cast<int64_t>(s.tokens) * D, false, &m->pos));
  {
    void* p;
    EVT_TRY(L.alloc(static_cast<size_t>(m->n_prefix) * D * 4, &p));
    m->prefix = reinterpret_cast<float*>(p);
    EVT_TRY(L.vec_into(e + "cls_token", D, false, m->prefix));
    if (m->n_prefix == 2) EVT_TRY(L.vec_into(e + "distillation_token", D, false, m->prefix + D));
  }
  for (int l = 0; l < s.layers; ++l) {
    LayerW& w = m->layers[l];
    const std::string p = "vit.encoder.layer." + std::to_string(l) + ".";
    w.a = s.heads[l] * s.head_size;
    w.inter = s.inter[l];
    w.inter_ld = padn(w.inter, m->pad);
    void* q;
    EVT_TRY(L.alloc(static_cast<size_t>(3) * w.a * D * m->es, &q));
    w.wqkv = reinterpret_cast<uint8_t*>(q);
    EVT_TRY(L.alloc(static_cast<size_t>(3) * w.a * 4, &q));
    w.bqkv = reinterpret_cast<float*>(q);
    const char* names[3] = {"query", "key", "value"};
    for (int t = 0; t < 3; ++t) {
      const std::string base = p + "attention.attention." + names[t];
      EVT_TRY(L.mat_into(base + ".weight", w.a, D, D, w.wqkv + static_cast<size_t>(t) * w.a * D * m->es));
      EVT_TRY(L.vec_into(base + ".bias", w.a, true, w.bqkv + t * w.a));
    }
    EVT_TRY(L.mat(p + "attention.output.dense.weight", D, w.a, w.a, &w.wo));
    EVT_TRY(L.vec(p + "attention.output.dense.bias", D, true, &w.bo));
    EVT_TRY(L.mat(p + "intermediate.dense.weight", w.inter, D, D, &w.w1));
    EVT_TRY(L.vec(p + "intermediate.dense.bias", w.inter, true, &w.b1));
    EVT_TRY(L.mat(p + "output.dense.weight", D, w.inter, w.inter_ld, &w.w2));
    EVT_TRY(L.vec(p + "output.dense.bias", D, true, &w.b2));
    EVT_TRY(L.vec(p + "layernorm_before.weight", D, false, &w.ln1_g));
    EVT_TRY(L.vec(p + "layernorm_before.bias", D, false, &w.ln1_b));
    EVT_TRY(L.vec(p + "layernorm_after.weight", D, false, &w.ln2_g));
    EVT_TRY(L.vec(p + "layernorm_after.bias", D, false, &w.ln2_b));
  }
  if (s.t2t) {
    for (int i = 0; i < 2; ++i) {
      PerformerW& pw = m->perf[i];
      const std::string p = "t2t.performer" + std::to_string(i + 1) + ".";
      pw.in_dim = i == 0 ? 7 * 7 * 3 : 3 * 3 * 64;
      pw.in_ld = padn(pw.in_dim, 8);
      EVT_TRY(L.vec(p + "norm1.gamma", pw.in_dim, false, &pw.g1));
      EVT_TRY(L.vec(p + "norm1.beta", pw.in_dim, false, &pw.b1));
      EVT_TRY(L.mat_t(p + "kqv.kernel", 192, pw.in_dim, pw.in_ld, &pw.wkqv));
      EVT_TRY(L.vec(p + "kqv.bias", 192, true, &pw.bkqv));
      EVT_TRY(L.vec(p + "w", 32 * 64, false, &pw.w));
      EVT_TRY(L.mat_t(p + "attn_output.kernel", 64, 64, 64, &pw.wo));
      EVT_TRY(L.vec(p + "attn_output.bias", 64, true, &pw.bo));
      EVT_TRY(L.vec(p + "norm2.gamma", 64, false, &pw.g2));
      EVT_TRY(L.vec(p + "norm2.beta", 64, false, &pw.b2));
      EVT_TRY(L.mat_t(p + "mlp.fc1.kernel", 64, 64, 64, &pw.w1));
      EVT_TRY(L.vec(p + "mlp.fc1.bias", 64, true, &pw.bb1));
      EVT_TRY(L.mat_t(p + "mlp.fc2.kernel", 64, 64, 64, &pw.w2));
      EVT_TRY(L.vec(p + "mlp.fc2.bias", 64, true, &pw.bb2));
    }
  }
  if (s.final_ln) {
    EVT_TRY(L.vec("vit.layernorm.weight", D, false, &m->lnf_g));
    EVT_TRY(L.vec("vit.layernorm.bias", D, false, &m->lnf_b));
  }
  int cls_in = D * (s.head_rows > 1 ? s.head_rows : 1);
  if (s.head_hidden > 0) {
    EVT_TRY(L.mat("pre_classifier.weight", s.head_hidden, D, D, &m->w_pre));
    EVT_TRY(L.vec("pre_classifier.bias", s.head_hidden, true, &m->b_pre));
    cls_in = s.head_hidden;
  }
  EVT_TRY(L.mat("classifier.weight", s.num_labels, cls_in, padn(cls_in, m->pad), &m->w_cls));
  EVT_TRY(L.vec("classifier.bias", s.num_labels, true, &m->b_cls));
  EVT_CUDA(cudaStreamSynchronize(L.st));
  m->loaded = true;
  return EVT_OK;
}

extern "C" int evt_model_workspace_bytes(const evt_model* m, int batch, size_t* out) {
  EVT_CHECK_ARG(m != nullptr && out != nullptr, "evt_model_workspace_bytes: null argument");
  EVT_CHECK_ARG(batch > 0, "batch must be positive");
  *out = plan_workspace(m, batch, nullptr).bytes + 1024;
  return EVT_OK;
}

extern "C" int evt_model_launches_per_forward(const evt_model* m) {
  if (!m) return 0;
  const evt_model_spec& s = m->spec;
  return (s.t2t ? 2 * 5 + 1 : 0) + (s.embed_k > 0 ? 2 : 3) + 7 * s.layers + (s.final_ln && s.head_rows > 1 ? s.head_rows : 1) + (s.head_hidden > 0 ? 2 : 1);
}

static int forward_impl(evt_model* m, const void* pixels, const evt_forward_opts* opts, const void* patch_matrix, int64_t patch_ld,
                        int batch, float* logits, void* workspace, size_t workspace_bytes, evt_stream stream) {
  EVT_CHECK_ARG(m != nullptr, "evt_model_forward: model is null");
  if (!m->loaded) return fail(EVT_ERR_STATE, "evt_model_forward called before evt_model_load_weights");
  EVT_CHECK_ARG((pixels || patch_matrix) && logits && workspace, "evt_model_forward: null pointer");
  EVT_CHECK_ARG(batch > 0 && batch <= 65535, "batch must be in 1..65535");
  const evt_model_spec& s = m->spec;
  static const evt_forward_opts kNoOpts = {};
  const evt_forward_opts& o = opts != nullptr ? *opts : kNoOpts;
  EVT_CHECK_ARG(o.head_mask == nullptr || o.head_mask_ld > 0, "head_mask_ld must be positive when a head mask is given");
  Workspace w;
  EVT_TRY(place_workspace(workspace, workspace_bytes, [&](uint8_t* base) { return plan_workspace(m, batch, base); }, &w,
                          "workspace too small for this batch (see evt_model_workspace_bytes)"));
  cudaStream_t st = static_cast<cudaStream_t>(stream);
  StaticWeightsScope weights_are_static;
  const int D = s.hidden;
  const int64_t M = static_cast<int64_t>(batch) * s.tokens;
  const int64_t Mp = static_cast<int64_t>(batch) * m->patches;
  const bool tf = s.dialect == EVT_DIALECT_TF;
  const float scale = 1.0f / sqrtf(static_cast<float>(s.head_size));
  auto mark = [&](int stage) -> int {
    if (!m->profiling) return EVT_OK;
    if (m->prof_used == m->prof_events.size()) {
      cudaEvent_t ev;
      EVT_CUDA(cudaEventCreate(&ev));
      m->prof_events.push_back(ev);
    }
    EVT_CUDA(cudaEventRecord(m->prof_events[m->prof_used], st));
    if (stage >= 0) m->prof_spans.push_back({stage, {m->prof_used - 1, m->prof_used}});
    ++m->prof_used;
    return EVT_OK;
  };
#define EVT_STAGE(stage, expr) \
  do {                         \
    EVT_TRY(expr);             \
    EVT_TRY(mark(stage));      \
  } while (0)
  EVT_TRY(mark(-1));
  const bool tf32 = s.precision == EVT_PREC_TF32;
  const int dt = tf32 ? EVT_F32 : EVT_BF16;
  const int adt = tf32 ? EVT_TF32 : EVT_BF16;
  if (s.t2t && patch_matrix == nullptr) {
    const float tf_eps = 1e-5f;
    const void* src = pixels;
    int src_dt = EVT_F32, side = s.image, ch = 3;
    EVT_CHECK_ARG(o.pixel_dtype == EVT_PIX_F32, "the T2T front-end takes f32 NHWC pixels");
    for (int i = 0; i < 2; ++i) {
      const PerformerW& pw = m->perf[i];
      const int k = i == 0 ? 7 : 3, st_ = i == 0 ? 4 : 2, pad_ = i == 0 ? 2 : 1;
      const int so = t2t_side(s.image, i), T = so * so;
      const int64_t rows = static_cast<int64_t>(batch) * T;
      EVT_STAGE(EVT_STAGE_EMBED, unfold_ln_launch(src, src_dt, w.t_x[i], pw.in_ld, pw.g1, pw.b1, tf_eps, batch, side, side, ch, k, st_, pad_, st));
      EVT_STAGE(EVT_STAGE_EMBED, gemm_launch({.A = w.t_x[i], .lda = pw.in_ld, .W = pw.wkqv, .ldw = pw.in_ld, .bias = pw.bkqv, .out = w.t_kqv[i],
                                              .out_dtype = EVT_BF16, .ldo = 192, .M = rows, .N = 192, .K = pw.in_dim}, st));
      EVT_TRY(performer_block_launch(w.t_kqv[i], 192, pw.w, w.t_y[i], w.t_ws[i], batch, T, 1e-8f, pw.wo, pw.bo, pw.g2, pw.b2, pw.w1,
                                     pw.bb1, pw.w2, pw.bb2, tf_eps, st));
      EVT_TRY(mark(EVT_STAGE_EMBED));
      src = w.t_y[i], src_dt = EVT_F32, side = so, ch = 64;
    }
    EVT_STAGE(EVT_STAGE_EMBED, unfold_ln_launch(src, src_dt, w.t_pm, 576, nullptr, nullptr, tf_eps, batch, side, side, 64, 3, 2, 1, st));
    patch_matrix = w.t_pm;
    patch_ld = 576;
  }
  if (patch_matrix == nullptr) {
    EVT_CHECK_ARG(s.embed_k == 0, "this model takes a caller-built patch matrix (evt_model_forward_embedded)");
    const size_t row_bytes = static_cast<size_t>(m->patch_k) * m->es;
    EVT_CUDA(cudaMemset2DAsync(w.big, s.tokens * row_bytes, 0, m->n_prefix * row_bytes, batch, st));
    EVT_STAGE(EVT_STAGE_EMBED, im2col_launch(pixels, o.pixel_dtype, o.pixel_scale, o.pixel_bias, w.big, dt, batch, s.image, s.image, s.patch, st,
                                             s.tokens, m->n_prefix));
    EVT_STAGE(EVT_STAGE_EMBED, embed_fill_launch(m->prefix, m->pos, m->b_patch, w.resid, batch, s.tokens, m->n_prefix, D, st));
    EVT_STAGE(EVT_STAGE_EMBED, gemm_launch({.A = w.big, .lda = m->patch_k, .W = m->w_patch, .ldw = m->patch_k, .in_dtype = dt, .residual = w.resid,
                                            .ldr = D, .out = w.resid, .out_dtype = EVT_F32, .ldo = D, .M = M, .N = D, .K = m->patch_k}, st));
  } else {
    EVT_CHECK_ARG(patch_ld >= m->patch_k, "patch matrix leading dimension smaller than the embedding K");
    EVT_STAGE(EVT_STAGE_EMBED,
              gemm_launch({.A = patch_matrix, .lda = patch_ld, .W = m->w_patch, .ldw = m->patch_k, .in_dtype = dt, .bias = m->b_patch,
                           .residual = m->pos, .ldr = D, .out = w.resid, .out_dtype = EVT_F32, .ldo = D, .M = Mp, .N = D, .K = m->patch_k,
                           .map = {.res_row_mod = m->patches, .res_row_off = m->n_prefix, .out_group = m->patches,
                                   .out_group_stride = s.tokens, .out_group_off = m->n_prefix}}, st));
    EVT_STAGE(EVT_STAGE_EMBED, prefix_tokens_launch(m->prefix, m->pos, w.resid, batch, s.tokens, m->n_prefix, D, st));
  }
  const bool row_ln = !tf32 && gemm_rowln_supported(M, D, D, tf);
  const int64_t tok_stride = static_cast<int64_t>(s.tokens) * D;
  const bool cls_tail = !tf32 && s.head_rows <= 1 && !(o.ctx_out != nullptr && o.ctx_out[s.layers - 1] != nullptr);
  bool xn_ready = false;
  for (int l = 0; l < s.layers; ++l) {
    const LayerW& lw = m->layers[l];
    const int a = lw.a;
    const bool tail = cls_tail && l == s.layers - 1;
    const int64_t rows = tail ? batch : M;
    const int64_t rs = tail ? tok_stride : D;
    auto on_rows = [&](GemmOp op) {
      if (!tail) return op;
      op.max_k_splits = gemm_k_splits(op) > 1 ? 0 : 1;
      op.M = rows;
      op.ldr = op.ldo = rs;
      return op;
    };
    if (!xn_ready)
      EVT_STAGE(EVT_STAGE_LN, layernorm_launch(w.resid, D, lw.ln1_g, lw.ln1_b, w.xn, adt, D, tf ? w.resid : nullptr, M, D, s.eps, st));
    EVT_STAGE(EVT_STAGE_QKV, gemm_launch({.A = w.xn, .lda = D, .W = lw.wqkv, .ldw = D, .in_dtype = dt, .bias = lw.bqkv, .out = w.qkv,
                                          .out_dtype = adt, .ldo = 3 * a, .M = M, .N = 3 * a, .K = D}, st));
    xn_ready = false;
    const float* hmask = o.head_mask != nullptr ? o.head_mask + static_cast<size_t>(l) * o.head_mask_ld : nullptr;
    EVT_CHECK_ARG(hmask == nullptr || o.head_mask_ld >= s.heads[l], "head_mask_ld smaller than a layer's head count");
    uint8_t* ctx = (o.ctx_out != nullptr && o.ctx_out[l] != nullptr) ? reinterpret_cast<uint8_t*>(o.ctx_out[l]) : w.ctx;
    EVT_CHECK_ARG(reinterpret_cast<uintptr_t>(ctx) % 16 == 0, "ctx_out pointers must be 16-byte aligned");
    if (tf32)
      EVT_STAGE(EVT_STAGE_ATTN, attention_tf32_launch(reinterpret_cast<const float*>(w.qkv), 3 * a, reinterpret_cast<float*>(ctx), a, hmask,
                                    batch, s.tokens, s.heads[l], s.head_size, scale, st));
    else
      EVT_STAGE(EVT_STAGE_ATTN, attention_launch(w.qkv, 3 * a, ctx, a, hmask, batch, s.tokens, tail ? 1 : s.tokens, s.heads[l], s.head_size,
                                                 scale, st));
    if (!tail && row_ln && gemm_rowln_pays(D, a, tf)) {
      EVT_STAGE(EVT_STAGE_OPROJ, gemm_rowln_launch(ctx, a, lw.wo, a, lw.bo, w.resid, D, lw.ln2_g, lw.ln2_b, s.eps, tf, w.xn, D, M, D, a, st));
    } else {
      EVT_STAGE(EVT_STAGE_OPROJ, gemm_launch(on_rows({.A = ctx, .lda = a, .W = lw.wo, .ldw = a, .in_dtype = dt, .bias = lw.bo, .residual = w.resid,
                                                      .ldr = D, .out = w.resid, .out_dtype = EVT_F32, .ldo = D, .M = M, .N = D, .K = a}), st));
      EVT_STAGE(EVT_STAGE_LN, layernorm_launch(w.resid, rs, lw.ln2_g, lw.ln2_b, w.xn, adt, D, tf ? w.resid : nullptr, rows, D, s.eps, st));
    }
    EVT_STAGE(EVT_STAGE_FC1, gemm_launch({.A = w.xn, .lda = D, .W = lw.w1, .ldw = D, .in_dtype = dt, .bias = lw.b1, .out = w.big,
                                          .out_dtype = adt, .ldo = lw.inter_ld, .M = rows, .N = lw.inter, .K = D, .act = s.act}, st));
    if (row_ln && l + 1 < s.layers && gemm_rowln_pays(D, lw.inter, tf)) {
      const LayerW& nx = m->layers[l + 1];
      EVT_STAGE(EVT_STAGE_FC2, gemm_rowln_launch(w.big, lw.inter_ld, lw.w2, lw.inter_ld, lw.b2, w.resid, D, nx.ln1_g, nx.ln1_b, s.eps, tf, w.xn,
                                                 D, M, D, lw.inter, st));
      xn_ready = true;
    } else {
      EVT_STAGE(EVT_STAGE_FC2, gemm_launch(on_rows({.A = w.big, .lda = lw.inter_ld, .W = lw.w2, .ldw = lw.inter_ld, .in_dtype = dt, .bias = lw.b2,
                                                    .residual = w.resid, .ldr = D, .out = w.resid, .out_dtype = EVT_F32, .ldo = D, .M = M, .N = D,
                                                    .K = lw.inter}), st));
    }
  }
  const int head_rows = s.head_rows > 1 ? s.head_rows : 1;
  if (s.final_ln) {
    for (int r = 0; r < head_rows; ++r)
      EVT_STAGE(EVT_STAGE_HEAD, layernorm_launch(w.resid + static_cast<size_t>(r) * D, tok_stride, m->lnf_g, m->lnf_b,
                                                 w.clsn + static_cast<size_t>(r) * D * m->es, adt, static_cast<int64_t>(head_rows) * D, nullptr,
                                                 batch, D, s.eps, st));
  } else {
    const long long total = static_cast<long long>(batch) * D;
    const unsigned grid = static_cast<unsigned>((total + 255) / 256);
    const long long nrows = batch;
    if (tf32)
      EVT_CUDA(launch_pdl(gather_rows_cast_kernel<float>, dim3(grid), dim3(256), 0, st, pdl_for_rows(M), static_cast<const float*>(w.resid), tok_stride,
                          reinterpret_cast<float*>(w.clsn), nrows, D));
    else
      EVT_CUDA(launch_pdl(gather_rows_cast_kernel<__nv_bfloat16>, dim3(grid), dim3(256), 0, st, pdl_for_rows(M), static_cast<const float*>(w.resid),
                          tok_stride, reinterpret_cast<__nv_bfloat16*>(w.clsn), nrows, D));
    EVT_LAUNCH_CHECK("gather_rows_cast");
    EVT_TRY(mark(EVT_STAGE_HEAD));
  }
  if (s.head_hidden > 0) {
    const int hl = padn(s.head_hidden, m->pad);
    EVT_STAGE(EVT_STAGE_HEAD, gemm_launch({.A = w.clsn, .lda = D, .W = m->w_pre, .ldw = D, .in_dtype = dt, .bias = m->b_pre, .out = w.hh,
                                           .out_dtype = adt, .ldo = hl, .M = batch, .N = s.head_hidden, .K = D, .act = EVT_ACT_GELU_TANH}, st));
    EVT_STAGE(EVT_STAGE_HEAD, gemm_launch({.A = w.hh, .lda = hl, .W = m->w_cls, .ldw = hl, .in_dtype = dt, .bias = m->b_cls, .out = logits,
                                           .out_dtype = EVT_F32, .ldo = s.num_labels, .M = batch, .N = s.num_labels, .K = s.head_hidden}, st));
  } else {
    const int kc = head_rows * D;
    EVT_STAGE(EVT_STAGE_HEAD, gemm_launch({.A = w.clsn, .lda = kc, .W = m->w_cls, .ldw = kc, .in_dtype = dt, .bias = m->b_cls, .out = logits,
                                           .out_dtype = EVT_F32, .ldo = s.num_labels, .M = batch, .N = s.num_labels, .K = kc}, st));
  }
#undef EVT_STAGE
  return EVT_OK;
}

extern "C" int evt_model_profile_begin(evt_model* m) {
  EVT_CHECK_ARG(m != nullptr, "evt_model_profile_begin: model is null");
  m->profiling = true;
  m->prof_used = 0;
  m->prof_spans.clear();
  return EVT_OK;
}

extern "C" int evt_model_profile_end(evt_model* m, float* stage_ms, int* stage_launches) {
  EVT_CHECK_ARG(m != nullptr && stage_ms != nullptr && stage_launches != nullptr, "evt_model_profile_end: null argument");
  if (!m->profiling) return fail(EVT_ERR_STATE, "evt_model_profile_end without evt_model_profile_begin");
  m->profiling = false;
  for (int i = 0; i < EVT_STAGE_COUNT; ++i) stage_ms[i] = 0.f, stage_launches[i] = 0;
  if (m->prof_used > 0) EVT_CUDA(cudaEventSynchronize(m->prof_events[m->prof_used - 1]));
  for (const auto& sp : m->prof_spans) {
    float ms = 0.f;
    EVT_CUDA(cudaEventElapsedTime(&ms, m->prof_events[sp.second.first], m->prof_events[sp.second.second]));
    stage_ms[sp.first] += ms;
    stage_launches[sp.first] += 1;
  }
  m->prof_spans.clear();
  m->prof_used = 0;
  return EVT_OK;
}

extern "C" int evt_model_forward(evt_model* m, const float* pixels, int batch, float* logits, void* workspace,
                                 size_t workspace_bytes, evt_stream stream) {
  EVT_CHECK_ARG(pixels != nullptr, "evt_model_forward: pixels is null");
  return forward_impl(m, pixels, nullptr, nullptr, 0, batch, logits, workspace, workspace_bytes, stream);
}

extern "C" int evt_model_forward_ex(evt_model* m, const void* pixels, const evt_forward_opts* opts, int batch, float* logits,
                                    void* workspace, size_t workspace_bytes, evt_stream stream) {
  EVT_CHECK_ARG(pixels != nullptr, "evt_model_forward_ex: pixels is null");
  return forward_impl(m, pixels, opts, nullptr, 0, batch, logits, workspace, workspace_bytes, stream);
}

extern "C" int evt_model_forward_embedded(evt_model* m, const void* patch_matrix, int64_t ld, int batch, float* logits,
                                          void* workspace, size_t workspace_bytes, evt_stream stream) {
  EVT_CHECK_ARG(patch_matrix != nullptr, "evt_model_forward_embedded: patch_matrix is null");
  return forward_impl(m, nullptr, nullptr, patch_matrix, ld, batch, logits, workspace, workspace_bytes, stream);
}

extern "C" int evt_gemm_residual_layernorm_ex(const void* A, int64_t lda, const void* W, int64_t ldw, const float* bias, float* resid,
                                              int64_t ldr, const float* gamma, const float* beta, float eps, int copy_ln, void* xn,
                                              int64_t ldxn, int64_t M, int N, int K, evt_stream stream) {
  int rc = evt_device_check();
  if (rc != EVT_OK) return rc;
  EVT_CHECK_ARG(A != nullptr && W != nullptr && resid != nullptr && xn != nullptr && gamma != nullptr && beta != nullptr,
                "gemm_residual_layernorm: null pointer");
  cudaStream_t st = static_cast<cudaStream_t>(stream);
  if (gemm_rowln_supported(M, N, K, copy_ln != 0))
    return gemm_rowln_launch(A, lda, W, ldw, bias, resid, ldr, gamma, beta, eps, copy_ln != 0, xn, ldxn, M, N, K, st);
  EVT_TRY(gemm_launch({.A = A, .lda = lda, .W = W, .ldw = ldw, .bias = bias, .residual = resid, .ldr = ldr, .out = resid,
                       .out_dtype = EVT_F32, .ldo = ldr, .M = M, .N = N, .K = K}, st));
  return layernorm_launch(resid, ldr, gamma, beta, xn, EVT_BF16, ldxn, copy_ln ? resid : nullptr, M, N, eps, st);
}

extern "C" int evt_gemm_residual_layernorm(const void* A, int64_t lda, const void* W, int64_t ldw, const float* bias, float* resid,
                                           int64_t ldr, const float* gamma, const float* beta, float eps, void* xn, int64_t ldxn,
                                           int64_t M, int N, int K, evt_stream stream) {
  int rc = evt_device_check();
  if (rc != EVT_OK) return rc;
  EVT_CHECK_ARG(resid != nullptr && xn != nullptr && gamma != nullptr && beta != nullptr, "gemm_residual_layernorm: null pointer");
  if (N % 64 != 0 || N < 64 || N > 1024) return fail(EVT_ERR_UNSUPPORTED, "gemm+ln: N must be a multiple of 64 in [64, 1024]");
  return evt_gemm_residual_layernorm_ex(A, lda, W, ldw, bias, resid, ldr, gamma, beta, eps, 0, xn, ldxn, M, N, K, stream);
}
```

### edgevisiontransformer_b200/csrc/ops.h

```cpp
#pragma once
#include "common.h"

namespace evt {

struct GemmOp {
  struct RowMap {
    int res_row_mod = 0, res_row_off = 0;
    int out_group = 0, out_group_stride = 0, out_group_off = 0;
  };
  const void* A = nullptr;
  int64_t lda = 0;
  const void* W = nullptr;
  int64_t ldw = 0;
  int in_dtype = EVT_BF16;
  const float* bias = nullptr;
  const float* residual = nullptr;
  int64_t ldr = 0;
  void* out = nullptr;
  int out_dtype = EVT_BF16;
  int64_t ldo = 0;
  int64_t M = 0;
  int N = 0, K = 0;
  int act = EVT_ACT_NONE;
  RowMap map = {};
  int max_k_splits = 0;
};
int gemm_launch(const GemmOp& op, cudaStream_t stream);
int gemm_k_splits(const GemmOp& op);

bool gemm_rowln_supported(int64_t M, int N, int K, bool copy_ln);
bool gemm_rowln_pays(int N, int K, bool copy_ln);
int gemm_rowln_launch(const void* A, int64_t lda, const void* W, int64_t ldw, const float* bias, float* resid, int64_t ldr,
                      const float* gamma, const float* beta, float eps, bool copy_ln, void* xn, int64_t ldxn, int64_t M, int N,
                      int K, cudaStream_t stream);

int attention_launch(const void* qkv, int64_t ldq, void* ctx, int64_t ldc, const float* head_mask, int B, int S, int Sq,
                     int heads, int head_size, float scale, cudaStream_t stream);

int attention_tf32_launch(const float* qkv, int64_t ldq, float* ctx, int64_t ldc, const float* head_mask, int B, int S,
                          int heads, int head_size, float scale, cudaStream_t stream);

int layernorm_launch(const float* x, int64_t x_stride, const float* gamma, const float* beta, void* y, int y_dtype,
                     int64_t y_stride, float* y_copy, int64_t rows, int D, float eps, cudaStream_t st);

int im2col_launch(const void* pixels, int pixel_dtype, const float* scale3, const float* bias3, void* cols, int out_dtype, int B,
                  int H, int W, int P, cudaStream_t st, int row_stride = 0, int row_off = 0);
int embed_fill_launch(const float* prefix, const float* pos, const float* bias, float* out, int B, int tokens, int n_prefix, int D,
                      cudaStream_t st);
int im2col4_launch(const float* pixels, void* cols, int B, int H, int W, int P, cudaStream_t st);
int gather_layernorm_launch(const float* x, const int* idx, const float* gamma, const float* beta, void* y, int y_dtype, float* copy_f32,
                            int64_t images, int T_in, int T_out, int G, int C, float eps, cudaStream_t st);
int window_attention_launch(const void* qkv, int64_t ldq, void* ctx, int64_t ldc, const float* table, int n_tab, int64_t n_windows,
                            int window_tokens, int heads, int head_size, float scale, cudaStream_t st);
int layernorm_mean_tokens_launch(const float* x, const float* gamma, const float* beta, void* y, int64_t images, int T, int D, float eps,
                                 cudaStream_t st);
int prefix_tokens_launch(const float* prefix, const float* pos, float* out, int B, int tokens, int n_prefix, int D,
                         cudaStream_t st);
int cast_launch(const float* x, void* y, int64_t n, cudaStream_t st);
int unfold_ln_launch(const void* x, int x_dtype, void* out, int64_t ldo, const float* gamma, const float* beta, float eps, int B,
                     int H, int W, int C, int k, int s, int p, cudaStream_t st);
size_t performer_workspace_bytes(int B, int T);
int performer_launch(const void* kqv, int64_t ld, const float* w, void* yattn, float* vout, void* workspace, int B, int T, int emb,
                     int m, float eps, cudaStream_t st);
int performer_mlp_launch(const void* ya, float* y, const void* wo, const float* bo, const float* gamma, const float* beta, const void* w1,
                         const float* b1, const void* w2, const float* b2, int64_t rows, float eps, cudaStream_t st);
int performer_block_launch(const void* kqv, int64_t ld, const float* w, float* y, void* workspace, int B, int T, float eps, const void* wo,
                           const float* bo, const float* gamma, const float* beta, const void* w1, const float* b1, const void* w2,
                           const float* b2, float ln_eps, cudaStream_t st);
int unfold_launch(const void* x, int x_dtype, void* out, int64_t ldo, int B, int H, int W, int C, int k, int s, int p,
                  cudaStream_t st);

}
```

### edgevisiontransformer_b200/ops.py

```python
from __future__ import annotations

from typing import Optional

import torch

from . import _lib
from ._lib import ACT_GELU_ERF, ACT_GELU_TANH, ACT_NONE, EVT_BF16, EVT_F32

ACTS = {None: ACT_NONE, "none": ACT_NONE, "gelu": ACT_GELU_ERF, "gelu_erf": ACT_GELU_ERF, "erf": ACT_GELU_ERF,
        "gelu_tanh": ACT_GELU_TANH, "gelu_new": ACT_GELU_TANH, "gelu_pytorch_tanh": ACT_GELU_TANH}


def _stream() -> int:
    return torch.cuda.current_stream().cuda_stream


def _need_cuda(*ts: Optional[torch.Tensor]) -> None:
    for t in ts:
        if t is not None and not t.is_cuda:
            raise RuntimeError("edgevisiontransformer_b200 ops need CUDA tensors on a B200 (sm_100a); "
                               "there is no CPU fallback")


def _dt(t: torch.Tensor) -> int:
    if t.dtype == torch.float32:
        return EVT_F32
    if t.dtype == torch.bfloat16:
        return EVT_BF16
    raise ValueError(f"unsupported dtype {t.dtype}")


def _ptr(t: Optional[torch.Tensor]) -> Optional[int]:
    return None if t is None else t.data_ptr()


def layernorm(x: torch.Tensor, gamma: torch.Tensor, beta: torch.Tensor, eps: float,
              out_dtype: torch.dtype = torch.bfloat16, write_back: bool = False) -> torch.Tensor:
    _need_cuda(x, gamma, beta)
    if x.dtype != torch.float32 or x.stride(-1) != 1:
        raise ValueError("layernorm wants an f32 tensor with unit inner stride")
    D = x.shape[-1]
    x2 = x.reshape(-1, D)
    if x2.data_ptr() != x.data_ptr():
        raise ValueError("layernorm wants a tensor viewable as [rows, D]")
    y = torch.empty(x2.shape, dtype=out_dtype, device=x.device)
    lib = _lib.load()
    _lib.check(lib.evt_layernorm_fwd(x2.data_ptr(), x2.stride(0), gamma.data_ptr(), beta.data_ptr(), y.data_ptr(), _dt(y),
                                     y.stride(0), x2.data_ptr() if write_back else None, x2.shape[0], D, float(eps),
                                     _stream()), "layernorm")
    return y.view(*x.shape)


def layernorm_rows(x: torch.Tensor, row_stride: int, rows: int, D: int, gamma, beta, eps, out_dtype=torch.bfloat16):
    _need_cuda(x, gamma, beta)
    y = torch.empty((rows, D), dtype=out_dtype, device=x.device)
    lib = _lib.load()
    _lib.check(lib.evt_layernorm_fwd(x.data_ptr(), row_stride, gamma.data_ptr(), beta.data_ptr(), y.data_ptr(), _dt(y), D,
                                     None, rows, D, float(eps), _stream()), "layernorm")
    return y


def layernorm2d(x: torch.Tensor, gamma: torch.Tensor, beta: torch.Tensor, eps: float = 1e-5,
                addend: Optional[torch.Tensor] = None) -> torch.Tensor:
    _need_cuda(x, gamma, beta, addend)
    x = x.contiguous()
    if addend is not None:
        addend = addend.contiguous()
    B = x.shape[0]
    nh = x[0].numel()
    if gamma.numel() != nh or beta.numel() != nh:
        raise ValueError("layernorm2d: affine parameters must have n*h elements")
    y = torch.empty_like(x)
    lib = _lib.load()
    _lib.check(lib.evt_layernorm2d_fwd(x.data_ptr(), _ptr(addend), gamma.contiguous().data_ptr(),
                                       beta.contiguous().data_ptr(), y.data_ptr(), B, nh, float(eps), _stream()),
               "layernorm2d")
    return y


def linear(a: torch.Tensor, w: torch.Tensor, bias: Optional[torch.Tensor] = None, act=None,
           residual: Optional[torch.Tensor] = None, out_dtype: torch.dtype = torch.bfloat16,
           out: Optional[torch.Tensor] = None, n: Optional[int] = None, k: Optional[int] = None) -> torch.Tensor:
    _need_cuda(a, w, bias, residual, out)
    if a.dim() != 2 or w.dim() != 2 or a.stride(1) != 1 or w.stride(1) != 1:
        raise ValueError("linear wants 2-D operands with unit inner stride")
    if a.dtype != w.dtype:
        raise ValueError("linear: a and w must have the same dtype")
    M = a.shape[0]
    K = k if k is not None else a.shape[1]
    N = n if n is not None else w.shape[0]
    if w.shape[1] < K or a.shape[1] < K:
        raise ValueError("linear: K exceeds operand width")
    if out is None:
        out = torch.empty((M, N), dtype=out_dtype, device=a.device)
    if residual is not None and (residual.dtype != torch.float32 or residual.stride(1) != 1):
        raise ValueError("linear: residual must be f32 with unit inner stride")
    lib = _lib.load()
    act_id = ACTS[act] if not isinstance(act, int) else act
    if a.dtype == torch.bfloat16:
        rc = lib.evt_gemm_bias_act(a.data_ptr(), a.stride(0), w.data_ptr(), w.stride(0), _ptr(bias), _ptr(residual),
                                   residual.stride(0) if residual is not None else 0, 0, 0, out.data_ptr(), _dt(out),
                                   out.stride(0), 0, 0, 0, M, N, K, act_id, _stream())
    elif a.dtype == torch.float32:
        if out.dtype != torch.float32:
            raise ValueError("linear: tf32 mode writes f32")
        rc = lib.evt_gemm_bias_act_tf32(a.data_ptr(), a.stride(0), w.data_ptr(), w.stride(0), _ptr(bias), _ptr(residual),
                                        residual.stride(0) if residual is not None else 0, 0, 0, out.data_ptr(),
                                        out.stride(0), 0, 0, 0, M, N, K, act_id, _stream())
    else:
        raise ValueError(f"linear: unsupported dtype {a.dtype}")
    _lib.check(rc, "gemm")
    return out


def layernorm_linear(x: torch.Tensor, gamma: torch.Tensor, beta: torch.Tensor, eps: float, w: torch.Tensor,
                     bias: Optional[torch.Tensor] = None, act=None, write_back: bool = False,
                     out: Optional[torch.Tensor] = None) -> torch.Tensor:
    _need_cuda(x, gamma, beta, w, bias, out)
    if x.dtype != torch.float32 or w.dtype != torch.bfloat16 or x.dim() != 2 or w.dim() != 2 or x.stride(1) != 1 or w.stride(1) != 1:
        raise ValueError("layernorm_linear wants a 2-D f32 x and a 2-D bf16 w with unit inner strides")
    M, K = x.shape
    N = w.shape[0]
    if w.shape[1] < K:
        raise ValueError("layernorm_linear: w has fewer columns than x")
    if out is None:
        ld = (N + 7) // 8 * 8
        out = torch.empty((M, ld), dtype=torch.bfloat16, device=x.device)[:, :N]
    lib = _lib.load()
    rc = lib.evt_layernorm_gemm(x.data_ptr(), x.stride(0), gamma.contiguous().data_ptr(), beta.contiguous().data_ptr(), float(eps),
                                x.data_ptr() if write_back else None, w.data_ptr(), w.stride(0), _ptr(bias), out.data_ptr(),
                                out.stride(0), M, N, K, ACTS[act], _stream())
    _lib.check(rc, "layernorm_gemm")
    return out


def linear_residual_layernorm(a: torch.Tensor, w: torch.Tensor, bias: Optional[torch.Tensor], resid: torch.Tensor,
                              gamma: torch.Tensor, beta: torch.Tensor, eps: float, k: Optional[int] = None,
                              xn: Optional[torch.Tensor] = None, copy_ln: bool = False) -> torch.Tensor:
    _need_cuda(a, w, bias, resid, gamma, beta, xn)
    if a.dtype != torch.bfloat16 or w.dtype != torch.bfloat16 or resid.dtype != torch.float32:
        raise ValueError("linear_residual_layernorm wants bf16 operands and an f32 residual stream")
    if a.dim() != 2 or w.dim() != 2 or resid.dim() != 2 or a.stride(1) != 1 or w.stride(1) != 1 or resid.stride(1) != 1:
        raise ValueError("linear_residual_layernorm wants 2-D operands with unit inner stride")
    M, N = resid.shape
    K = k if k is not None else a.shape[1]
    if a.shape[0] != M or w.shape[0] != N or a.shape[1] < K or w.shape[1] < K:
        raise ValueError("linear_residual_layernorm: shape mismatch")
    if xn is None:
        xn = torch.empty((M, N), dtype=torch.bfloat16, device=a.device)
    lib = _lib.load()
    rc = lib.evt_gemm_residual_layernorm_ex(a.data_ptr(), a.stride(0), w.data_ptr(), w.stride(0), _ptr(bias), resid.data_ptr(),
                                            resid.stride(0), gamma.contiguous().data_ptr(), beta.contiguous().data_ptr(),
                                            float(eps), int(copy_ln), xn.data_ptr(), xn.stride(0), M, N, K, _stream())
    _lib.check(rc, "gemm_residual_layernorm")
    return xn


def attention(qkv: torch.Tensor, B: int, S: int, heads: int, head_size: int = 64, scale: Optional[float] = None,
              head_mask: Optional[torch.Tensor] = None, q_rows: Optional[int] = None) -> torch.Tensor:
    _need_cuda(qkv, head_mask)
    if qkv.dtype not in (torch.bfloat16, torch.float32) or qkv.dim() != 2 or qkv.stride(1) != 1:
        raise ValueError("attention wants a 2-D bf16 (or f32 for the tf32 mode) qkv matrix")
    if qkv.shape[0] != B * S or qkv.shape[1] < 3 * heads * head_size:
        raise ValueError("attention: qkv shape does not match B, S, heads")
    if q_rows is not None and qkv.dtype != torch.bfloat16:
        raise ValueError("attention: q_rows is implemented for bf16 only")
    Sq = S if q_rows is None else int(q_rows)
    ctx = torch.empty((B * Sq, heads * head_size), dtype=qkv.dtype, device=qkv.device)
    scale = float(head_size ** -0.5 if scale is None else scale)
    lib = _lib.load()
    if q_rows is not None:
        rc = lib.evt_attention_query_rows_fwd(qkv.data_ptr(), qkv.stride(0), ctx.data_ptr(), ctx.stride(0), _ptr(head_mask), B, S,
                                              Sq, heads, head_size, scale, _stream())
    else:
        fn = lib.evt_attention_fwd if qkv.dtype == torch.bfloat16 else lib.evt_attention_fwd_tf32
        rc = fn(qkv.data_ptr(), qkv.stride(0), ctx.data_ptr(), ctx.stride(0), _ptr(head_mask), B, S, heads, head_size, scale,
                _stream())
    _lib.check(rc, "attention")
    return ctx


def gather_layernorm(x: torch.Tensor, idx: torch.Tensor, gamma: Optional[torch.Tensor], beta: Optional[torch.Tensor], eps: float,
                     images: int, T_in: int, T_out: int, G: int = 1, out_dtype: Optional[torch.dtype] = torch.bfloat16,
                     copy: bool = False):
    _need_cuda(x, idx, gamma, beta)
    if x.dtype != torch.float32 or x.dim() != 2 or not x.is_contiguous() or x.shape[0] != images * T_in:
        raise ValueError("gather_layernorm wants a contiguous f32 [images*T_in, C] matrix")
    if idx.dtype != torch.int32 or idx.numel() != T_out * G or not idx.is_contiguous():
        raise ValueError("gather_layernorm: idx must be a contiguous int32 [T_out*G] tensor")
    C = x.shape[1]
    y = torch.empty((images * T_out, G * C), dtype=out_dtype, device=x.device) if out_dtype is not None else None
    cp = torch.empty((images * T_out, G * C), dtype=torch.float32, device=x.device) if copy else None
    lib = _lib.load()
    _lib.check(lib.evt_gather_layernorm(x.data_ptr(), idx.data_ptr(), _ptr(gamma), _ptr(beta), _ptr(y),
                                        _dt(y) if y is not None else EVT_BF16, _ptr(cp), images, T_in, T_out, G, C, float(eps),
                                        _stream()), "gather_layernorm")
    return y, cp


def window_attention(qkv: torch.Tensor, table: torch.Tensor, n_windows: int, heads: int, window_tokens: int = 49,
                     head_size: int = 32, scale: Optional[float] = None) -> torch.Tensor:
    _need_cuda(qkv, table)
    if qkv.dtype != torch.bfloat16 or qkv.dim() != 2 or qkv.stride(1) != 1 or qkv.shape[0] != n_windows * window_tokens:
        raise ValueError("window_attention wants a bf16 [n_windows*tokens, 3*heads*head_size] matrix")
    if table.dtype != torch.float32 or table.dim() != 4 or tuple(table.shape[1:]) != (heads, 64, 56) or not table.is_contiguous():
        raise ValueError("window_attention: table must be a contiguous f32 [n_tab, heads, 64, 56] tensor")
    ctx = torch.empty((qkv.shape[0], heads * head_size), dtype=torch.bfloat16, device=qkv.device)
    scale = float(head_size ** -0.5 if scale is None else scale)
    lib = _lib.load()
    _lib.check(lib.evt_window_attention_fwd(qkv.data_ptr(), qkv.stride(0), ctx.data_ptr(), ctx.stride(0), table.data_ptr(),
                                            table.shape[0], n_windows, window_tokens, heads, head_size, scale, _stream()),
               "window_attention")
    return ctx


def layernorm_mean_tokens(x: torch.Tensor, gamma: torch.Tensor, beta: torch.Tensor, eps: float, images: int, T: int) -> torch.Tensor:
    _need_cuda(x, gamma, beta)
    if x.dtype != torch.float32 or x.dim() != 2 or not x.is_contiguous() or x.shape[0] != images * T:
        raise ValueError("layernorm_mean_tokens wants a contiguous f32 [images*T, D] matrix")
    y = torch.empty((images, x.shape[1]), dtype=torch.bfloat16, device=x.device)
    lib = _lib.load()
    _lib.check(lib.evt_layernorm_mean_tokens(x.data_ptr(), gamma.data_ptr(), beta.data_ptr(), y.data_ptr(), images, T, x.shape[1],
                                             float(eps), _stream()), "layernorm_mean_tokens")
    return y


def im2col_patch(pixels: torch.Tensor, patch: int = 16) -> torch.Tensor:
    _need_cuda(pixels)
    if pixels.dtype != torch.float32 or pixels.dim() != 4 or pixels.shape[1] != 3:
        raise ValueError("im2col_patch wants f32 NCHW pixels with 3 channels")
    pixels = pixels.contiguous()
    B, _, H, W = pixels.shape
    cols = torch.empty((B * (H // patch) * (W // patch), 3 * patch * patch), dtype=torch.bfloat16, device=pixels.device)
    lib = _lib.load()
    _lib.check(lib.evt_im2col_patch(pixels.data_ptr(), cols.data_ptr(), B, H, W, patch, _stream()), "im2col")
    return cols


def patch_embed(pixels: torch.Tensor, weight: torch.Tensor, bias: torch.Tensor, prefix: torch.Tensor, pos: torch.Tensor,
                patch: int = 16, mean=None, std=None) -> torch.Tensor:
    import ctypes as C
    _need_cuda(pixels, weight, bias, prefix, pos)
    if pixels.dim() != 4 or pixels.shape[1] != 3:
        raise ValueError("patch_embed wants NCHW pixels with 3 channels")
    pix = {torch.float32: _lib.PIX_F32, torch.bfloat16: _lib.PIX_BF16, torch.uint8: _lib.PIX_U8}.get(pixels.dtype)
    if pix is None:
        raise ValueError("patch_embed: pixels must be f32, bf16 or uint8")
    pixels = pixels.contiguous()
    B, _, H, W = pixels.shape
    D = weight.shape[0]
    K = 3 * patch * patch
    w = weight.reshape(D, -1)
    if w.shape[1] != K:
        raise ValueError(f"patch_embed: weight has {w.shape[1]} inputs per filter, expected {K}")
    w = w.to(torch.bfloat16).contiguous()
    prefix = prefix.reshape(-1, D).float().contiguous()
    tokens = prefix.shape[0] + (H // patch) * (W // patch)
    pos = pos.reshape(-1, D).float().contiguous()
    if pos.shape[0] != tokens:
        raise ValueError(f"patch_embed: {pos.shape[0]} position rows for {tokens} tokens")
    scale = shift = None
    if pix == _lib.PIX_U8:
        if mean is None or std is None:
            raise ValueError("patch_embed: uint8 pixels need mean and std")
        scale = (C.c_float * 3)(*[1.0 / (255.0 * float(s_)) for s_ in std])
        shift = (C.c_float * 3)(*[-float(m_) / float(s_) for m_, s_ in zip(mean, std)])
    lib = _lib.load()
    n = C.c_size_t()
    _lib.check(lib.evt_patch_embed_workspace_bytes(B, H, W, patch, prefix.shape[0], C.byref(n)), "patch_embed_workspace_bytes")
    ws = torch.empty(n.value + 1024, dtype=torch.uint8, device=pixels.device)
    ws_ptr = (ws.data_ptr() + 1023) // 1024 * 1024
    out = torch.empty((B, tokens, D), dtype=torch.float32, device=pixels.device)
    _lib.check(lib.evt_patch_embed_fwd(pixels.data_ptr(), pix, scale, shift, w.data_ptr(), K, bias.float().contiguous().data_ptr(),
                                       prefix.data_ptr(), pos.data_ptr(), out.data_ptr(), ws_ptr, B, H, W, patch, D,
                                       prefix.shape[0], _stream()), "patch_embed")
    return out


def cast_bf16(x: torch.Tensor) -> torch.Tensor:
    _need_cuda(x)
    x = x.contiguous()
    if x.dtype != torch.float32:
        raise ValueError("cast_bf16 wants f32")
    y = torch.empty(x.shape, dtype=torch.bfloat16, device=x.device)
    lib = _lib.load()
    _lib.check(lib.evt_cast_f32_bf16(x.data_ptr(), y.data_ptr(), x.numel(), _stream()), "cast")
    return y


def unfold_nhwc(x: torch.Tensor, k: int, s: int, p: int, ld: Optional[int] = None) -> torch.Tensor:
    _need_cuda(x)
    x = x.contiguous()
    B, H, W, Cc = x.shape
    oh, ow = (H + 2 * p - k) // s + 1, (W + 2 * p - k) // s + 1
    ld = ld or (k * k * Cc + 7) // 8 * 8
    out = torch.empty((B * oh * ow, ld), dtype=torch.bfloat16, device=x.device)
    lib = _lib.load()
    _lib.check(lib.evt_unfold_nhwc(x.data_ptr(), _dt(x), out.data_ptr(), ld, B, H, W, Cc, k, s, p, _stream()), "unfold")
    return out


def unfold_ln_nhwc(x: torch.Tensor, k: int, s: int, p: int, gamma: Optional[torch.Tensor] = None,
                   beta: Optional[torch.Tensor] = None, eps: float = 1e-5, ld: Optional[int] = None) -> torch.Tensor:
    _need_cuda(x, gamma, beta)
    x = x.contiguous()
    B, H, W, Cc = x.shape
    oh, ow = (H + 2 * p - k) // s + 1, (W + 2 * p - k) // s + 1
    ld = ld or (k * k * Cc + 7) // 8 * 8
    out = torch.empty((B * oh * ow, ld), dtype=torch.bfloat16, device=x.device)
    lib = _lib.load()
    _lib.check(lib.evt_unfold_ln_nhwc(x.data_ptr(), _dt(x), out.data_ptr(), ld, _ptr(gamma), _ptr(beta), float(eps), B, H, W,
                                      Cc, k, s, p, _stream()), "unfold_ln")
    return out


def performer(kqv: torch.Tensor, w: torch.Tensor, B: int, T: int, eps: float = 1e-8):
    _need_cuda(kqv, w)
    if kqv.dtype != torch.bfloat16 or kqv.dim() != 2 or kqv.shape[0] != B * T or kqv.stride(1) != 1:
        raise ValueError("performer wants a bf16 [B*T, 192] kqv matrix")
    if tuple(w.shape) != (32, 64) or w.dtype != torch.float32:
        raise ValueError("performer: w must be f32 [32, 64]")
    import ctypes as C
    lib = _lib.load()
    n = C.c_size_t()
    _lib.check(lib.evt_performer_workspace_bytes(B, T, C.byref(n)), "performer_workspace_bytes")
    ws = torch.empty(n.value, dtype=torch.uint8, device=kqv.device)
    yattn = torch.empty((B * T, 64), dtype=torch.bfloat16, device=kqv.device)
    vout = torch.empty((B * T, 64), dtype=torch.float32, device=kqv.device)
    _lib.check(lib.evt_performer_fwd(kqv.data_ptr(), kqv.stride(0), w.contiguous().data_ptr(), yattn.data_ptr(),
                                     vout.data_ptr(), ws.data_ptr(), B, T, 64, 32, float(eps), _stream()), "performer")
    return yattn, vout


def performer_mlp(yattn: torch.Tensor, y: torch.Tensor, wo, bo, gamma, beta, w1, b1, w2, b2, eps: float) -> torch.Tensor:
    _need_cuda(yattn, y, wo, bo, gamma, beta, w1, b1, w2, b2)
    if yattn.dtype != torch.bfloat16 or y.dtype != torch.float32 or yattn.shape != y.shape or y.dim() != 2 or y.shape[1] != 64:
        raise ValueError("performer_mlp wants yattn bf16 [rows, 64] and y f32 [rows, 64]")
    if not (yattn.is_contiguous() and y.is_contiguous()):
        raise ValueError("performer_mlp wants contiguous rows")
    for w in (wo, w1, w2):
        if w.dtype != torch.bfloat16 or tuple(w.shape) != (64, 64) or not w.is_contiguous():
            raise ValueError("performer_mlp: weights must be contiguous bf16 [64, 64]")
    lib = _lib.load()
    _lib.check(lib.evt_performer_mlp_fwd(yattn.data_ptr(), y.data_ptr(), wo.data_ptr(), _ptr(bo), gamma.contiguous().data_ptr(),
                                         beta.contiguous().data_ptr(), w1.data_ptr(), _ptr(b1), w2.data_ptr(), _ptr(b2),
                                         y.shape[0], float(eps), _stream()), "performer_mlp")
    return y


def performer_block(kqv: torch.Tensor, w: torch.Tensor, B: int, T: int, wo, bo, gamma, beta, w1, b1, w2, b2, ln_eps: float,
                    eps: float = 1e-8) -> torch.Tensor:
    _need_cuda(kqv, w, wo, bo, gamma, beta, w1, b1, w2, b2)
    if kqv.dtype != torch.bfloat16 or kqv.dim() != 2 or kqv.shape[0] != B * T or kqv.stride(1) != 1:
        raise ValueError("performer_block wants a bf16 [B*T, 192] kqv matrix")
    if tuple(w.shape) != (32, 64) or w.dtype != torch.float32:
        raise ValueError("performer_block: w must be f32 [32, 64]")
    for m in (wo, w1, w2):
        if m.dtype != torch.bfloat16 or tuple(m.shape) != (64, 64) or not m.is_contiguous():
            raise ValueError("performer_block: weights must be contiguous bf16 [64, 64]")
    import ctypes as C
    lib = _lib.load()
    n = C.c_size_t()
    _lib.check(lib.evt_performer_workspace_bytes(B, T, C.byref(n)), "performer_workspace_bytes")
    ws = torch.empty(n.value, dtype=torch.uint8, device=kqv.device)
    y = torch.empty((B * T, 64), dtype=torch.float32, device=kqv.device)
    _lib.check(lib.evt_performer_block_fwd(kqv.data_ptr(), kqv.stride(0), w.contiguous().data_ptr(), y.data_ptr(), ws.data_ptr(), B, T,
                                           float(eps), wo.data_ptr(), _ptr(bo), gamma.contiguous().data_ptr(), beta.contiguous().data_ptr(),
                                           w1.data_ptr(), _ptr(b1), w2.data_ptr(), _ptr(b2), float(ln_eps), _stream()), "performer_block")
    return y


def set_gemm_pair_mode(mode: int) -> None:
    _lib.load().evt_gemm_set_pair_mode(int(mode))


def set_gemm_split_k(enable: bool) -> None:
    _lib.load().evt_gemm_set_split_k(1 if enable else 0)


class static_weights:

    def __enter__(self):
        _lib.load().evt_gemm_weights_static(1)
        return self

    def __exit__(self, *exc):
        _lib.load().evt_gemm_weights_static(-1)
        return False


def launch_count(reset: bool = False) -> int:
    lib = _lib.load()
    n = int(lib.evt_launch_count())
    if reset:
        lib.evt_launch_count_reset()
    return n
```

### include/evt.h

```cpp
#ifndef EVT_H_
#define EVT_H_

#include <stddef.h>
#include <stdint.h>

#ifdef __cplusplus
extern "C" {
#endif

#define EVT_VERSION 100

enum evt_status {
  EVT_OK = 0,
  EVT_ERR_INVALID = -1,
  EVT_ERR_CUDA = -2,
  EVT_ERR_UNSUPPORTED = -3,
  EVT_ERR_STATE = -4
};

enum evt_dtype { EVT_F32 = 0, EVT_BF16 = 1, EVT_TF32 = 2 };

enum evt_act { EVT_ACT_NONE = 0, EVT_ACT_GELU_ERF = 1, EVT_ACT_GELU_TANH = 2 };

typedef void* evt_stream;

const char* evt_last_error(void);
int evt_version(void);
int evt_device_check(void);
int64_t evt_launch_count(void);
void evt_launch_count_reset(void);
void evt_gemm_set_pair_mode(int mode);
void evt_gemm_set_split_k(int enable);
void evt_gemm_weights_static(int delta);


int evt_layernorm_fwd(const float* x, int64_t x_stride, const float* gamma, const float* beta,
                      void* y, int y_dtype, int64_t y_stride, float* y_copy_f32,
                      int64_t rows, int D, float eps, evt_stream stream);

int evt_layernorm2d_fwd(const float* x, const float* addend, const float* gamma, const float* beta,
                        float* y, int64_t batch, int64_t nh, float eps, evt_stream stream);

int evt_gemm_bias_act(const void* A, int64_t lda, const void* W, int64_t ldw, const float* bias,
                      const float* residual, int64_t ldr, int res_row_mod, int res_row_off,
                      void* out, int out_dtype, int64_t ldo,
                      int out_group, int out_group_stride, int out_group_off,
                      int64_t M, int N, int K, int act, evt_stream stream);

int evt_gemm_bias_act_tf32(const float* A, int64_t lda, const float* W, int64_t ldw, const float* bias,
                           const float* residual, int64_t ldr, int res_row_mod, int res_row_off,
                           float* out, int64_t ldo, int out_group, int out_group_stride, int out_group_off,
                           int64_t M, int N, int K, int act, evt_stream stream);

int evt_layernorm_gemm(const float* x, int64_t ldx, const float* gamma, const float* beta, float eps, float* x_copy_f32,
                       const void* W, int64_t ldw, const float* bias, void* out, int64_t ldo, int64_t M, int N, int K,
                       int act, evt_stream stream);

int evt_gemm_residual_layernorm(const void* A, int64_t lda, const void* W, int64_t ldw, const float* bias,
                                float* resid, int64_t ldr, const float* gamma, const float* beta, float eps,
                                void* xn, int64_t ldxn, int64_t M, int N, int K, evt_stream stream);
int evt_gemm_residual_layernorm_ex(const void* A, int64_t lda, const void* W, int64_t ldw, const float* bias,
                                   float* resid, int64_t ldr, const float* gamma, const float* beta, float eps, int copy_ln,
                                   void* xn, int64_t ldxn, int64_t M, int N, int K, evt_stream stream);

#define EVT_ATTN_MAX_TOKENS 1026

int evt_attention_fwd(const void* qkv, int64_t ldq, void* ctx, int64_t ldc, const float* head_mask,
                      int B, int S, int heads, int head_size, float scale, evt_stream stream);

int evt_attention_query_rows_fwd(const void* qkv, int64_t ldq, void* ctx, int64_t ldc, const float* head_mask,
                                 int B, int S, int Sq, int heads, int head_size, float scale, evt_stream stream);

int evt_attention_fwd_tf32(const float* qkv, int64_t ldq, float* ctx, int64_t ldc, const float* head_mask,
                           int B, int S, int heads, int head_size, float scale, evt_stream stream);

int evt_im2col_patch(const float* pixels, void* cols, int B, int H, int W, int P, evt_stream stream);

int evt_patch_embed_workspace_bytes(int B, int H, int W, int P, int n_prefix, size_t* out);
int evt_patch_embed_fwd(const void* pixels, int pixel_dtype, const float* pixel_scale, const float* pixel_bias,
                        const void* W, int64_t ldw, const float* bias, const float* prefix, const float* pos,
                        float* out, void* workspace, int B, int H, int Wd, int P, int D, int n_prefix,
                        evt_stream stream);

int evt_prefix_tokens(const float* prefix, const float* pos, float* out, int B, int tokens, int n_prefix,
                      int D, evt_stream stream);

int evt_cast_f32_bf16(const float* x, void* y, int64_t n, evt_stream stream);

int evt_unfold_nhwc(const void* x, int x_dtype, void* out, int64_t ldo, int B, int H, int W, int C,
                    int k, int s, int p, evt_stream stream);

int evt_unfold_ln_nhwc(const void* x, int x_dtype, void* out, int64_t ldo, const float* gamma, const float* beta,
                       float eps, int B, int H, int W, int C, int k, int s, int p, evt_stream stream);

int evt_performer_workspace_bytes(int B, int T, size_t* out);
int evt_performer_fwd(const void* kqv, int64_t ld, const float* w, void* yattn, float* vout, void* workspace,
                      int B, int T, int emb, int m, float eps, evt_stream stream);

int evt_performer_mlp_fwd(const void* ya, float* y, const void* wo, const float* bo, const float* gamma, const float* beta,
                          const void* w1, const float* b1, const void* w2, const float* b2, int64_t rows, float eps,
                          evt_stream stream);

int evt_performer_block_fwd(const void* kqv, int64_t ld, const float* w, float* y, void* workspace, int B, int T, float eps,
                            const void* wo, const float* bo, const float* gamma, const float* beta, const void* w1,
                            const float* b1, const void* w2, const float* b2, float ln_eps, evt_stream stream);


int evt_gather_layernorm(const float* x, const int* idx, const float* gamma, const float* beta, void* y, int y_dtype,
                         float* copy_f32, int64_t images, int T_in, int T_out, int G, int C, float eps, evt_stream stream);

int evt_window_attention_fwd(const void* qkv, int64_t ldq, void* ctx, int64_t ldc, const float* table, int n_tab,
                             int64_t n_windows, int window_tokens, int heads, int head_size, float scale, evt_stream stream);

int evt_layernorm_mean_tokens(const float* x, const float* gamma, const float* beta, void* y, int64_t images, int T, int D,
                              float eps, evt_stream stream);


typedef struct evt_model evt_model;

#define EVT_MAX_LAYERS 64

enum evt_precision { EVT_PREC_BF16 = 0, EVT_PREC_TF32 = 1 };

enum evt_dialect {
  EVT_DIALECT_HF = 0,
  EVT_DIALECT_TF = 1
};

typedef struct evt_model_spec {
  int dialect;
  int hidden;
  int layers;
  int tokens;
  int image, patch;
  int head_size;
  int num_labels;
  int act;
  float eps;
  int heads[EVT_MAX_LAYERS];
  int inter[EVT_MAX_LAYERS];
  int final_ln;
  int head_hidden;
  int t2t;
  int precision;
  int embed_k;
  int head_rows;
} evt_model_spec;

typedef struct evt_tensor_view {
  const char* name;
  const void* data;
  int ndim;
  int64_t shape[4];
} evt_tensor_view;

int evt_model_create(const evt_model_spec* spec, evt_model** out);
int evt_model_load_weights(evt_model* m, const evt_tensor_view* tensors, int n, evt_stream stream);
int evt_model_workspace_bytes(const evt_model* m, int batch, size_t* out);
int evt_model_forward(evt_model* m, const float* pixels, int batch, float* logits,
                      void* workspace, size_t workspace_bytes, evt_stream stream);
enum evt_pixel_dtype { EVT_PIX_F32 = 0, EVT_PIX_BF16 = 1, EVT_PIX_U8 = 2 };

typedef struct evt_forward_opts {
  int pixel_dtype;
  float pixel_scale[3];
  float pixel_bias[3];
  const float* head_mask;
  int head_mask_ld;
  void* const* ctx_out;
} evt_forward_opts;

int evt_model_forward_ex(evt_model* m, const void* pixels, const evt_forward_opts* opts, int batch, float* logits,
                         void* workspace, size_t workspace_bytes, evt_stream stream);
int evt_model_forward_embedded(evt_model* m, const void* patch_matrix, int64_t ld, int batch, float* logits,
                               void* workspace, size_t workspace_bytes, evt_stream stream);
int evt_model_launches_per_forward(const evt_model* m);
enum evt_stage {
  EVT_STAGE_EMBED = 0,
  EVT_STAGE_LN = 1,
  EVT_STAGE_QKV = 2,
  EVT_STAGE_ATTN = 3,
  EVT_STAGE_OPROJ = 4,
  EVT_STAGE_FC1 = 5,
  EVT_STAGE_FC2 = 6,
  EVT_STAGE_HEAD = 7,
  EVT_STAGE_COUNT = 8
};
int evt_model_profile_begin(evt_model* m);
int evt_model_profile_end(evt_model* m, float* stage_ms , int* stage_launches );
int evt_model_destroy(evt_model* m);


typedef struct evt_swin evt_swin;

#define EVT_SWIN_MAX_STAGES 8

typedef struct evt_swin_spec {
  int image, patch, window;
  int embed_dim;
  int stages;
  int depths[EVT_SWIN_MAX_STAGES];
  int heads[EVT_SWIN_MAX_STAGES];
  int num_labels;
  float eps;
} evt_swin_spec;

int evt_swin_create(const evt_swin_spec* spec, evt_swin** out);
int evt_swin_load_weights(evt_swin* m, const evt_tensor_view* tensors, int n, evt_stream stream);
int evt_swin_workspace_bytes(const evt_swin* m, int batch, size_t* out);
int evt_swin_forward(evt_swin* m, const float* pixels, int batch, float* logits, void* workspace, size_t workspace_bytes,
                     evt_stream stream);
int evt_swin_launches_per_forward(const evt_swin* m);
int evt_swin_destroy(evt_swin* m);

#ifdef __cplusplus
}
#endif
#endif
```

Baseline: 26980.

## Fold LayerNorm into next GEMM via row statistics and write-through residual epilogue

Adds a folded-LayerNorm path. The residual GEMM epilogue writes the updated f32 residual, a mean-shifted bf16 copy and per-chunk mean/M2 records. The following GEMM then applies the normalisation as a per-row scale and shift in its epilogue, using precomputed c and d vectors and weights with gamma folded in. This is meant to remove the standalone LayerNorm pass and its extra read and write of activations. In exchange it adds TMA reloads of the old residual, extra smem and barriers in the pair kernel, and bf16 rounding of the unnormalised values, which can cost accuracy.

```diff
diff --git a/edgevisiontransformer_b200/_lib.py b/edgevisiontransformer_b200/_lib.py
--- a/edgevisiontransformer_b200/_lib.py
+++ b/edgevisiontransformer_b200/_lib.py
@@ -66,6 +66,9 @@
     "evt_layernorm_gemm": (_i, [_p, _i64, _p, _p, _f, _p, _p, _i64, _p, _p, _i64, _i64, _i, _i, _i, _p]),
     "evt_gemm_residual_layernorm": (_i, [_p, _i64, _p, _i64, _p, _p, _i64, _p, _p, _f, _p, _i64, _i64, _i, _i, _p]),
     "evt_gemm_residual_layernorm_ex": (_i, [_p, _i64, _p, _i64, _p, _p, _i64, _p, _p, _f, _i, _p, _i64, _i64, _i, _i, _p]),
+    "evt_layernorm_fold_stats": (_i, [_p, _i64, _p, _i64, _p, _i64, _p, _i64, _i, _p]),
+    "evt_gemm_layernorm_folded": (_i, [_p, _i64, _p, _i64, _p, _p, _p, _f, _p, _i64, _i64, _i, _i, _i, _p]),
+    "evt_gemm_residual_write_through": (_i, [_p, _i64, _p, _i64, _p, _p, _i64, _p, _p, _p, _i64, _i64, _i, _i, _p]),
     "evt_attention_fwd": (_i, [_p, _i64, _p, _i64, _p, _i, _i, _i, _i, _f, _p]),
     "evt_attention_fwd_tf32": (_i, [_p, _i64, _p, _i64, _p, _i, _i, _i, _i, _f, _p]),
     "evt_attention_query_rows_fwd": (_i, [_p, _i64, _p, _i64, _p, _i, _i, _i, _i, _i, _f, _p]),
diff --git a/edgevisiontransformer_b200/csrc/gemm.cu b/edgevisiontransformer_b200/csrc/gemm.cu
--- a/edgevisiontransformer_b200/csrc/gemm.cu
+++ b/edgevisiontransformer_b200/csrc/gemm.cu
@@ -147,10 +147,11 @@
       const int m0 = (tile / p.tiles_n) * BM + quad * 32;
       const int nt0 = (tile % p.tiles_n) * BN;
       prefetch_bias<BN, OUT_F32>(pe, grp, lane, nt0);
+      const float2 fold = fold_coeffs(pe, m0 + lane);
       ptx::mbar_wait(&tfull[as], aphase);
       ptx::tc_fence_after();
       const uint32_t t_row = tmem_base + (static_cast<uint32_t>(quad * 32) << 16) + as * BN;
-      epilogue_tile<BN, TF32, OUT_F32, ACT, TMA_OUT>(pe, &tmO, stg, grp, lane, m0, nt0, t_row);
+      epilogue_tile<BN, TF32, OUT_F32, ACT, TMA_OUT>(pe, &tmO, stg, grp, lane, m0, nt0, t_row, fold);
       ptx::tc_fence_before();
       __syncwarp();
       if (lane == 0) ptx::mbar_arrive(&tempty[as]);
@@ -252,6 +253,16 @@
   if (splits == 1) return 1;
   const int kb_per_split = (num_kb + splits - 1) / splits;
   return (num_kb + kb_per_split - 1) / kb_per_split;
+}
+
+bool gemm_write_through_ok(const GemmOp& op) {
+  if (op.in_dtype != EVT_BF16 || op.out_dtype != EVT_F32 || op.act != EVT_ACT_NONE || op.residual == nullptr || !tma_out_ok(op)) return false;
+  if (op.N % 256 != 0 || op.N > 1024 || choose_bn(op.M, op.N) != 256) return false;
+  const int pair_mode = gemm_pair_mode();
+  const long pair_tiles = static_cast<long>((op.M + 2 * BM - 1) / (2 * BM)) * (op.N / 256);
+  if (!(pair_mode < 0 ? pair_tiles >= num_sms() : pair_mode != 0)) return false;
+  const long tiles = static_cast<long>((op.M + BM - 1) / BM) * (op.N / 256);
+  return k_splits(op, true, tiles, (op.K + 63) / 64) == 1;
 }
 
 int gemm_launch(const GemmOp& op, cudaStream_t stream) {
@@ -265,6 +276,16 @@
   EVT_CHECK_ARG(op.lda >= op.K && op.ldw >= op.K && op.ldo >= op.N, "gemm: leading dimension smaller than the row length");
   EVT_CHECK_ARG(op.map.out_group >= 0 && op.map.res_row_mod >= 0, "gemm: negative row-group parameter");
   EVT_CHECK_ARG(op.residual == nullptr || op.ldr >= op.N, "gemm: residual leading dimension smaller than N");
+  if (op.ln_c != nullptr)
+    EVT_CHECK_ARG(op.ln_in != nullptr && op.bias != nullptr && op.in_dtype == EVT_BF16 && op.out_dtype == EVT_BF16 && op.residual == nullptr &&
+                      op.map.out_group == 0 && op.K % 256 == 0 && op.K <= 1024,
+                  "gemm: the folded-LayerNorm epilogue needs records, d, bf16 in / out, no residual and K a multiple of 256 up to 1024");
+  if (op.xs != nullptr) {
+    EVT_CHECK_ARG(op.ln_in != nullptr && op.ln_out != nullptr && op.ln_c == nullptr && op.ldxs >= op.N &&
+                      reinterpret_cast<uintptr_t>(op.xs) % 16 == 0 && op.ldxs % 8 == 0,
+                  "gemm: write-through epilogue needs records in and out and a 16-byte aligned bf16 output");
+    if (!gemm_write_through_ok(op)) return fail(EVT_ERR_UNSUPPORTED, "gemm: write-through epilogue not available for this problem");
+  }
   const bool tf32 = op.in_dtype == EVT_F32;
   const int eb = tf32 ? 4 : 2;
   const int k_step = kStageRowBytes / eb;
@@ -293,6 +314,13 @@
   p.num_kb = (op.K + k_step - 1) / k_step;
   p.k_step = k_step;
   p.w_static = gemm_weights_static() ? 1 : 0;
+  p.ln_in = op.ln_in;
+  p.ln_out = op.ln_out;
+  p.ln_c = op.ln_c;
+  p.xs = static_cast<__nv_bfloat16*>(op.xs);
+  p.ldxs = op.ldxs;
+  p.ln_parts = ln_fold::parts(op.ln_c != nullptr ? op.K : op.N);
+  p.ln_eps = op.ln_eps;
   {
     const int oe = op.out_dtype != EVT_BF16 ? 4 : 2;
     bool ok = reinterpret_cast<uintptr_t>(op.out) % 16 == 0 && (op.ldo * oe) % 16 == 0;
diff --git a/edgevisiontransformer_b200/csrc/gemm2.cu b/edgevisiontransformer_b200/csrc/gemm2.cu
--- a/edgevisiontransformer_b200/csrc/gemm2.cu
+++ b/edgevisiontransformer_b200/csrc/gemm2.cu
@@ -9,37 +9,41 @@
 
 using namespace gemm_detail;
 
-template <int BN, int EW>
+template <int BN, int EW, bool WT = false>
 struct Cfg2 {
   static constexpr int kABytes = BM * kStageRowBytes;
   static constexpr int kBBytes = (BN / 2) * kStageRowBytes;
   static constexpr int kStageBytes = kABytes + kBBytes;
   static constexpr int kStagingBytes = EW * kStgBytes;
-  static constexpr int kMaxStages = (232448 - 1024 - kStagingBytes - 256) / kStageBytes;
+  static constexpr int kOldBytes = WT ? EW * kStgBytes : 0;
+  static constexpr int kMaxStages = (232448 - 1024 - kStagingBytes - kOldBytes - 256 - (WT ? EW * 8 : 0)) / kStageBytes;
   static constexpr int kStages = kMaxStages < (BN == 128 ? 8 : 6) ? kMaxStages : (BN == 128 ? 8 : 6);
   static constexpr int kTmemCols = BN == 128 ? 256 : 512;
   static constexpr int kProducer = EW, kMma = EW + 1, kThreadsCta = 32 * (EW + 2);
-  static constexpr int kBarBytes = (2 * kStages + 4) * 8 + 16;
-  static constexpr int kSmemBytes = 1024  + kStages * kStageBytes + kStagingBytes + kBarBytes;
+  static constexpr int kBarBytes = (2 * kStages + 4) * 8 + 16 + (WT ? EW * 8 : 0);
+  static constexpr int kSmemBytes = 1024  + kStages * kStageBytes + kStagingBytes + kOldBytes + kBarBytes;
   static_assert(kSmemBytes <= 232448, "exceeds the 227 KB of shared memory a CTA can opt in to");
 };
 
-template <int BN, bool OUT_F32, int ACT, int EW>
+template <int BN, bool OUT_F32, int ACT, int EW, bool WT>
 __global__ void __cluster_dims__(2, 1, 1) __launch_bounds__(32 * (EW + 2), 1)
 gemm_pair_kernel(const __grid_constant__ CUtensorMap tmA, const __grid_constant__ CUtensorMap tmW,
                  const __grid_constant__ CUtensorMap tmO, const GemmParams p) {
-  using C = Cfg2<BN, EW>;
+  using C = Cfg2<BN, EW, WT>;
+  static_assert(!WT || (BN == 256 && OUT_F32 && ACT == EVT_ACT_NONE && EW == 8), "write-through: 256-column f32 tiles, 8 warps");
   constexpr int kProducerWarp = C::kProducer, kMmaWarp = C::kMma, kEpiWarps = EW;
   extern __shared__ uint8_t smem_raw[];
   uint8_t* smem = reinterpret_cast<uint8_t*>((reinterpret_cast<uintptr_t>(smem_raw) + 1023) & ~uintptr_t(1023));
   uint8_t* stage_base = smem;
   uint8_t* staging = smem + C::kStages * C::kStageBytes;
-  uint64_t* bars = reinterpret_cast<uint64_t*>(smem + C::kStages * C::kStageBytes + C::kStagingBytes);
+  uint8_t* old_buf = staging + C::kStagingBytes;
+  uint64_t* bars = reinterpret_cast<uint64_t*>(smem + C::kStages * C::kStageBytes + C::kStagingBytes + C::kOldBytes);
   uint64_t* full = bars;
   uint64_t* empty = bars + C::kStages;
   uint64_t* tfull = bars + 2 * C::kStages;
   uint64_t* tempty = tfull + 2;
   uint32_t* tmem_ptr = reinterpret_cast<uint32_t*>(tempty + 2);
+  uint64_t* old_full = tempty + 4;
 
   const int warp = threadIdx.x >> 5;
   const int lane = threadIdx.x & 31;
@@ -60,6 +64,8 @@
       ptx::mbar_init(&tfull[s], 1);
       ptx::mbar_init(&tempty[s], 2 * kEpiWarps);
     }
+    if (WT)
+      for (int w = 0; w < kEpiWarps; ++w) ptx::mbar_init(&old_full[w], 1);
     ptx::fence_mbar_init();
   }
   if (warp == kMmaWarp) ptx::tmem_alloc_pair<C::kTmemCols>(tmem_ptr);
@@ -142,6 +148,109 @@
         }
       }
     }
+  } else if constexpr (WT) {
+    const int quad = warp & 3, grp = warp >> 2;
+    const int sw = lane & 7;
+    uint8_t* stg = staging + warp * kStgBytes;
+    uint8_t* ob = old_buf + warp * kStgBytes;
+    uint64_t* of = &old_full[warp];
+    const uint32_t ob_a = ptx::smem_u32(ob) + lane * 128, sb = ptx::smem_u32(stg) + lane * 128;
+    const int P = p.ln_parts;
+    uint32_t ophase = 0;
+    int as = 0;
+    uint32_t aphase = 0;
+    auto tile_m0 = [&](int tile) { return (tile / p.tiles_n) * (2 * BM) + static_cast<int>(rank) * BM + quad * 32; };
+    auto load_old = [&](int tile, int c) {
+      if (ptx::elect_one()) {
+        ptx::mbar_arrive_expect_tx(of, kStgBytes);
+        ptx::tma_load_2d(ob, &tmO, of, (tile % p.tiles_n) * BN + c * 32, tile_m0(tile));
+      }
+      __syncwarp();
+    };
+    if (pair < num_tiles) load_old(pair, grp);
+    for (int tile = pair; tile < num_tiles; tile += num_pairs) {
+      const int m0 = tile_m0(tile);
+      const int tn = tile % p.tiles_n;
+      const int nt0 = tn * BN;
+      const int row = m0 + lane;
+      const bool live = row < p.M;
+      prefetch_bias<BN, true, 2>(p, grp, lane, nt0);
+      const float s = live ? ln_fold::row_mean(p.ln_in + static_cast<long long>(row) * (P + 1), P) : 0.f;
+      ptx::mbar_wait(&tfull[as], aphase);
+      ptx::tc_fence_after();
+      const uint32_t t_row = tmem_base + (static_cast<uint32_t>(quad * 32) << 16) + as * BN;
+      float mean = 0.f, m2 = 0.f;
+#pragma unroll 1
+      for (int j = 0; j < BN / 64; ++j) {
+        const int c = grp + 2 * j;
+        const int n0 = nt0 + c * 32;
+        float v[32];
+        {
+          uint32_t r[32];
+          ptx::tmem_ld_x32(t_row + c * 32, r);
+          ptx::tmem_ld_wait();
+#pragma unroll
+          for (int k = 0; k < 32; ++k) v[k] = __uint_as_float(r[k]);
+        }
+        if (j == BN / 64 - 1) {
+          ptx::tc_fence_before();
+          __syncwarp();
+          if (lane == 0) ptx::mbar_arrive_cluster(ptx::mapa(&tempty[as], 0));
+        }
+        bias_act<32, EVT_ACT_NONE, false, true>(v, p.bias, n0, p.N, true);
+        ptx::mbar_wait(of, ophase);
+        ophase ^= 1;
+#pragma unroll
+        for (int i = 0; i < 8; ++i) {
+          const float4 x = ptx::lds_f4(ob_a + ((i ^ sw) << 4));
+          v[4 * i] = x.x + v[4 * i];
+          v[4 * i + 1] = x.y + v[4 * i + 1];
+          v[4 * i + 2] = x.z + v[4 * i + 2];
+          v[4 * i + 3] = x.w + v[4 * i + 3];
+        }
+        ptx::fence_proxy_async_smem();
+        __syncwarp();
+        if (j + 1 < BN / 64) load_old(tile, c + 2);
+        else if (tile + num_pairs < num_tiles) load_old(tile + num_pairs, grp);
+        if (ptx::elect_one()) ptx::bulk_wait_read<0>();
+        __syncwarp();
+#pragma unroll
+        for (int i = 0; i < 8; ++i) ptx::sts_f4(sb + ((i ^ sw) << 4), v[4 * i], v[4 * i + 1], v[4 * i + 2], v[4 * i + 3]);
+        ptx::fence_proxy_async_smem();
+        __syncwarp();
+        if (ptx::elect_one()) {
+          ptx::tma_store_2d(&tmO, stg, n0, m0);
+          ptx::bulk_commit();
+        }
+#pragma unroll
+        for (int k = 0; k < 32; ++k) v[k] = __fsub_rn(v[k], s);
+        if (live) {
+          uint4* dst = reinterpret_cast<uint4*>(p.xs + static_cast<long long>(row) * p.ldxs + n0);
+#pragma unroll
+          for (int i = 0; i < 4; ++i)
+            dst[i] = make_uint4(pack_bf16x2(v[8 * i], v[8 * i + 1]), pack_bf16x2(v[8 * i + 2], v[8 * i + 3]),
+                                pack_bf16x2(v[8 * i + 4], v[8 * i + 5]), pack_bf16x2(v[8 * i + 6], v[8 * i + 7]));
+        }
+        float cm, cm2;
+        ln_fold::chunk_stats(v, cm, cm2);
+        if (j == 0) {
+          mean = cm;
+          m2 = cm2;
+        } else {
+          ln_fold::merge(mean, m2, j, cm, cm2);
+        }
+      }
+      if (live) {
+        float2* rec = p.ln_out + static_cast<long long>(row) * (P + 1);
+        rec[2 * tn + grp] = make_float2(mean, m2);
+        if (tn == 0 && grp == 0) rec[P] = make_float2(s, 0.f);
+      }
+      if (++as == 2) {
+        as = 0;
+        aphase ^= 1;
+      }
+    }
+    if (ptx::elect_one()) ptx::bulk_wait<0>();
   } else {
     const int quad = warp & 3;
     uint8_t* stg = staging + warp * kStgBytes;
@@ -161,10 +270,11 @@
         if (++rot == kGroups) rot = 0;
       }
       prefetch_bias<BN, OUT_F32, EW / 4>(p, grp, lane, nt0);
+      const float2 fold = fold_coeffs(p, m0 + lane);
       ptx::mbar_wait(&tfull[as], aphase);
       ptx::tc_fence_after();
       const uint32_t t_row = tmem_base + (static_cast<uint32_t>(quad * 32) << 16) + as * BN;
-      epilogue_tile<BN, false, OUT_F32, ACT, true, EW / 4>(p, &tmO, stg, grp, lane, m0, nt0, t_row);
+      epilogue_tile<BN, false, OUT_F32, ACT, true, EW / 4>(p, &tmO, stg, grp, lane, m0, nt0, t_row, fold);
       ptx::tc_fence_before();
       __syncwarp();
       if (lane == 0) ptx::mbar_arrive_cluster(ptx::mapa(&tempty[as], 0));
@@ -185,11 +295,11 @@
   }
 }
 
-template <int BN, bool OUT_F32, int ACT, int EW>
+template <int BN, bool OUT_F32, int ACT, int EW, bool WT = false>
 int launch_pair_ew(const void* W, int64_t ldw, const CUtensorMap& tmA, const CUtensorMap& tmO, GemmParams p, cudaStream_t stream) {
-  using C = Cfg2<BN, EW>;
+  using C = Cfg2<BN, EW, WT>;
   constexpr int kThreads = C::kThreadsCta;
-  constexpr auto kern = gemm_pair_kernel<BN, OUT_F32, ACT, EW>;
+  constexpr auto kern = gemm_pair_kernel<BN, OUT_F32, ACT, EW, WT>;
   EVT_TRY(opt_in_smem<kern>(C::kSmemBytes));
   static int pairs_dev = -1;
   static int max_pairs = 0;
@@ -254,6 +364,10 @@
 
 int gemm_pair_launch(int bn, const void* W, int64_t ldw, const CUtensorMap& tmA, const CUtensorMap& tmO, const GemmParams& p,
                      bool out_f32, int act, cudaStream_t stream) {
+  if (p.xs != nullptr) {
+    if (bn != 256 || !out_f32 || act != EVT_ACT_NONE) return fail(EVT_ERR_INVALID, "gemm: write-through epilogue needs 256-column f32 tiles");
+    return launch_pair_ew<256, true, EVT_ACT_NONE, 8, true>(W, ldw, tmA, tmO, p, stream);
+  }
   switch (bn) {
     case 256: return dispatch_pair<256>(W, ldw, tmA, tmO, p, out_f32, act, stream);
     case 192: return dispatch_pair<192>(W, ldw, tmA, tmO, p, out_f32, act, stream);
diff --git a/edgevisiontransformer_b200/csrc/gemm_common.cuh b/edgevisiontransformer_b200/csrc/gemm_common.cuh
--- a/edgevisiontransformer_b200/csrc/gemm_common.cuh
+++ b/edgevisiontransformer_b200/csrc/gemm_common.cuh
@@ -2,6 +2,7 @@
 #include <cuda_bf16.h>
 
 #include "common.h"
+#include "ln_fold.cuh"
 #include "ptx.cuh"
 
 namespace evt {
@@ -43,7 +44,19 @@
   int vec_ok;
   int round_tf32;
   int w_static;
+  const float2* ln_in = nullptr;
+  float2* ln_out = nullptr;
+  const float* ln_c = nullptr;
+  __nv_bfloat16* xs = nullptr;
+  long long ldxs = 0;
+  int ln_parts = 0;
+  float ln_eps = 0.f;
 };
+
+__device__ __forceinline__ float2 fold_coeffs(const GemmParams& p, int row) {
+  if (p.ln_c == nullptr || row >= p.M) return make_float2(1.f, 0.f);
+  return ln_fold::coeffs(p.ln_in + static_cast<long long>(row) * (p.ln_parts + 1), p.ln_parts, p.ln_eps);
+}
 
 __device__ __forceinline__ long long map_out_row(const GemmParams& p, long long row) {
   if (p.out_group <= 0) return row;
@@ -144,8 +157,27 @@
   }
 }
 template <int CH, int ACT, bool EXACT, bool HI>
-__device__ __forceinline__ void bias_act(float (&v)[CH], const float* __restrict__ bias, int n0, int N, bool full) {
-  if (bias != nullptr) {
+__device__ __forceinline__ void bias_act(float (&v)[CH], const float* __restrict__ bias, int n0, int N, bool full,
+                                         const float* __restrict__ c = nullptr, float2 fold = {}) {
+  if (c != nullptr) {
+    if (full) {
+      const float4* b4 = reinterpret_cast<const float4*>(bias + n0);
+      const float4* c4 = reinterpret_cast<const float4*>(c + n0);
+      const uint64_t r2 = pk2(fold.x, fold.x), n2 = pk2(fold.y, fold.y);
+#pragma unroll
+      for (int i = 0; i < CH / 4; ++i) {
+        if (i % 4 == 0) asm volatile("" ::: "memory");
+        const float4 b = __ldg(b4 + i), cc = __ldg(c4 + i);
+        const uint64_t t0 = fma2(n2, pk2(cc.x, cc.y), pk2(b.x, b.y)), t1 = fma2(n2, pk2(cc.z, cc.w), pk2(b.z, b.w));
+        upk2(fma2(r2, pk2(v[4 * i], v[4 * i + 1]), t0), v[4 * i], v[4 * i + 1]);
+        upk2(fma2(r2, pk2(v[4 * i + 2], v[4 * i + 3]), t1), v[4 * i + 2], v[4 * i + 3]);
+      }
+    } else {
+#pragma unroll
+      for (int j = 0; j < CH; ++j)
+        if (n0 + j < N) v[j] = fmaf(fold.x, v[j], fmaf(fold.y, __ldg(c + n0 + j), __ldg(bias + n0 + j)));
+    }
+  } else if (bias != nullptr) {
     if (full) {
       const float4* b4 = reinterpret_cast<const float4*>(bias + n0);
 #pragma unroll
@@ -176,12 +208,15 @@
   const int k = lane / kLinesPerChunk;
   const int c = grp + NGRP * k;
   const int col = nt0 + c * CH + (lane % kLinesPerChunk) * 32;
-  if (c < NCH && col < p.N) asm volatile("prefetch.global.L1 [%0];" ::"l"(p.bias + col));
+  if (c < NCH && col < p.N) {
+    asm volatile("prefetch.global.L1 [%0];" ::"l"(p.bias + col));
+    if (p.ln_c != nullptr) asm volatile("prefetch.global.L1 [%0];" ::"l"(p.ln_c + col));
+  }
 }
 
 template <int BN, bool TF32, bool OUT_F32, int ACT, bool TMA_OUT, int NGRP = 2>
 __device__ __forceinline__ void epilogue_tile(const GemmParams& p, const CUtensorMap* tmO, uint8_t* stg, int grp, int lane,
-                                              int m0, int nt0, uint32_t t_row) {
+                                              int m0, int nt0, uint32_t t_row, float2 fold = {1.f, 0.f}) {
   constexpr int CH = OUT_F32 ? 32 : 64;
   constexpr int NCH = BN / CH;
   const int sw = lane & 7;
@@ -233,7 +268,7 @@
           if (c + NGRP < NCH && n0 + NGRP * CH < p.N) load_res(n0 + NGRP * CH);
         }
       }
-      bias_act<CH, ACT, TF32, OUT_F32>(v, p.bias, n0, p.N, full);
+      bias_act<CH, ACT, TF32, OUT_F32>(v, p.bias, n0, p.N, full, p.ln_c, fold);
       if constexpr (OUT_F32) {
         if (p.round_tf32) {
 #pragma unroll
diff --git a/edgevisiontransformer_b200/csrc/layernorm.cu b/edgevisiontransformer_b200/csrc/layernorm.cu
--- a/edgevisiontransformer_b200/csrc/layernorm.cu
+++ b/edgevisiontransformer_b200/csrc/layernorm.cu
@@ -1,6 +1,8 @@
 #include <cuda_bf16.h>
 
 #include "common.h"
+#include "ln_fold.cuh"
+#include "ops.h"
 #include "ptx.cuh"
 
 namespace evt {
@@ -275,6 +277,61 @@
     const float a = x[base + i] + (addend ? addend[base + i] : 0.f);
     y[base + i] = (a - mean) * rstd * gamma[i] + beta[i];
   }
+}
+
+template <int NC>
+__global__ void __launch_bounds__(128) ln_stats_kernel(const float* x, long long x_stride, const float2* rec_in, long long rec_in_rows,
+                                                       __nv_bfloat16* __restrict__ xs, long long ldxs, float2* __restrict__ rec_out,
+                                                       long long rows) {
+  ptx::grid_dep_launch();
+  ptx::grid_dep_wait();
+  constexpr int D = NC * ln_fold::kChunk, P = ln_fold::parts(D);
+  const int lane = threadIdx.x & 31;
+  const long long row = static_cast<long long>(blockIdx.x) * (blockDim.x >> 5) + (threadIdx.x >> 5);
+  if (row >= rows) return;
+  const bool has = lane < NC;
+  const float* xr = x + row * x_stride + lane * ln_fold::kChunk;
+  float v[ln_fold::kChunk];
+#pragma unroll
+  for (int i = 0; i < 8; ++i) {
+    float4 q = make_float4(0.f, 0.f, 0.f, 0.f);
+    if (has)
+      asm volatile("ld.global.L1::evict_last.v4.f32 {%0, %1, %2, %3}, [%4];" : "=f"(q.x), "=f"(q.y), "=f"(q.z), "=f"(q.w) : "l"(xr + 4 * i));
+    v[4 * i] = q.x, v[4 * i + 1] = q.y, v[4 * i + 2] = q.z, v[4 * i + 3] = q.w;
+  }
+  float s;
+  if (rec_in != nullptr) {
+    s = ln_fold::row_mean(rec_in + row * rec_in_rows * (P + 1), P);
+  } else {
+    float t = 0.f;
+#pragma unroll
+    for (int j = 0; j < ln_fold::kChunk; ++j) t += v[j];
+    s = warp_sum(t) / static_cast<float>(D);
+  }
+#pragma unroll
+  for (int j = 0; j < ln_fold::kChunk; ++j) v[j] = __fsub_rn(v[j], s);
+  if (has) {
+    uint4* dst = reinterpret_cast<uint4*>(xs + row * ldxs + lane * ln_fold::kChunk);
+#pragma unroll
+    for (int i = 0; i < 4; ++i) {
+      __nv_bfloat162 h[4];
+#pragma unroll
+      for (int k = 0; k < 4; ++k) h[k] = __floats2bfloat162_rn(v[8 * i + 2 * k], v[8 * i + 2 * k + 1]);
+      dst[i] = *reinterpret_cast<const uint4*>(h);
+    }
+  }
+  float cm, cm2;
+  ln_fold::chunk_stats(v, cm, cm2);
+  const int base = lane < P ? 8 * (lane >> 1) + (lane & 1) : 0;
+  float mean = __shfl_sync(0xffffffffu, cm, base), m2 = __shfl_sync(0xffffffffu, cm2, base);
+#pragma unroll
+  for (int j = 1; j < 4; ++j) {
+    const float a = __shfl_sync(0xffffffffu, cm, base + 2 * j), b = __shfl_sync(0xffffffffu, cm2, base + 2 * j);
+    ln_fold::merge(mean, m2, j, a, b);
+  }
+  float2* rec = rec_out + row * (P + 1);
+  if (lane < P) rec[lane] = make_float2(mean, m2);
+  else if (lane == P) rec[P] = make_float2(s, 0.f);
 }
 
 template <int OUT>
@@ -338,6 +395,24 @@
 
 }
 
+int ln_stats_launch(const float* x, int64_t x_stride, const float2* rec_in, int64_t rec_in_rows, void* xs, int64_t ldxs, float2* rec_out,
+                    int64_t rows, int D, cudaStream_t st) {
+  EVT_CHECK_ARG(x && xs && rec_out && rows > 0, "layernorm statistics: bad arguments");
+  EVT_CHECK_ARG(D % 256 == 0 && D <= 1024 && x_stride % 4 == 0 && ldxs % 8 == 0 && ldxs >= D && x_stride >= D,
+                "layernorm statistics: D must be a multiple of 256 up to 1024, rows 16-byte aligned");
+  constexpr int wpb = 4;
+  const unsigned grid = static_cast<unsigned>((rows + wpb - 1) / wpb);
+  auto* y = static_cast<__nv_bfloat16*>(xs);
+  switch (D) {
+    case 512: EVT_CUDA(launch_pdl(ln_stats_kernel<16>, dim3(grid), dim3(wpb * 32), 0, st, pdl_for_work(rows, D), x, x_stride, rec_in, rec_in_rows, y, ldxs, rec_out, rows)); break;
+    case 768: EVT_CUDA(launch_pdl(ln_stats_kernel<24>, dim3(grid), dim3(wpb * 32), 0, st, pdl_for_work(rows, D), x, x_stride, rec_in, rec_in_rows, y, ldxs, rec_out, rows)); break;
+    case 1024: EVT_CUDA(launch_pdl(ln_stats_kernel<32>, dim3(grid), dim3(wpb * 32), 0, st, pdl_for_work(rows, D), x, x_stride, rec_in, rec_in_rows, y, ldxs, rec_out, rows)); break;
+    default: return fail(EVT_ERR_UNSUPPORTED, "layernorm statistics: D must be 512, 768 or 1024");
+  }
+  EVT_LAUNCH_CHECK("layernorm statistics");
+  return EVT_OK;
+}
+
 int layernorm_launch(const float* x, int64_t x_stride, const float* gamma, const float* beta, void* y, int y_dtype,
                      int64_t y_stride, float* y_copy, int64_t rows, int D, float eps, cudaStream_t st) {
   EVT_CHECK_ARG(x && gamma && beta && y, "layernorm: null pointer");
diff --git a/edgevisiontransformer_b200/csrc/ln_fold.cuh b/edgevisiontransformer_b200/csrc/ln_fold.cuh
--- /dev/null
+++ b/edgevisiontransformer_b200/csrc/ln_fold.cuh
@@ -0,0 +1,55 @@
+#pragma once
+#include <cuda_runtime.h>
+
+namespace evt {
+namespace ln_fold {
+
+constexpr int kSlice = 128;
+constexpr int kChunk = 32;
+
+__host__ __device__ constexpr int parts(int D) { return D / kSlice; }
+__host__ __device__ constexpr int record_len(int D) { return D / kSlice + 1; }
+
+__device__ __forceinline__ float row_mean(const float2* __restrict__ rec, int P) {
+  float m = 0.f;
+  for (int i = 0; i < P; ++i) m = __fadd_rn(m, rec[i].x);
+  return __fadd_rn(rec[P].x, __fdiv_rn(m, static_cast<float>(P)));
+}
+
+__device__ __forceinline__ float2 coeffs(const float2* __restrict__ rec, int P, float eps) {
+  float m = 0.f;
+  for (int i = 0; i < P; ++i) m = __fadd_rn(m, rec[i].x);
+  m = __fdiv_rn(m, static_cast<float>(P));
+  float q = 0.f;
+  for (int i = 0; i < P; ++i) {
+    const float2 r = rec[i];
+    const float dm = __fsub_rn(r.x, m);
+    q = __fadd_rn(q, __fmaf_rn(static_cast<float>(kSlice) * dm, dm, r.y));
+  }
+  const float rstd = rsqrtf(__fdiv_rn(q, static_cast<float>(P * kSlice)) + eps);
+  return make_float2(rstd, -rstd * m);
+}
+
+__device__ __forceinline__ void chunk_stats(const float (&d)[kChunk], float& mean, float& m2) {
+  float s[4] = {0.f, 0.f, 0.f, 0.f};
+#pragma unroll
+  for (int j = 0; j < kChunk; ++j) s[j & 3] = __fadd_rn(s[j & 3], d[j]);
+  mean = __fmul_rn(__fadd_rn(__fadd_rn(s[0], s[1]), __fadd_rn(s[2], s[3])), 1.0f / kChunk);
+  float q[4] = {0.f, 0.f, 0.f, 0.f};
+#pragma unroll
+  for (int j = 0; j < kChunk; ++j) {
+    const float a = __fsub_rn(d[j], mean);
+    q[j & 3] = __fmaf_rn(a, a, q[j & 3]);
+  }
+  m2 = __fadd_rn(__fadd_rn(q[0], q[1]), __fadd_rn(q[2], q[3]));
+}
+
+__device__ __forceinline__ void merge(float& mean, float& m2, int j, float cmean, float cm2) {
+  const float na = static_cast<float>(j * kChunk), n = na + kChunk;
+  const float delta = __fsub_rn(cmean, mean);
+  mean = __fmaf_rn(delta, __fdiv_rn(static_cast<float>(kChunk), n), mean);
+  m2 = __fadd_rn(__fadd_rn(m2, cm2), __fmul_rn(__fmul_rn(delta, delta), __fdiv_rn(na * kChunk, n)));
+}
+
+}
+}
diff --git a/edgevisiontransformer_b200/csrc/loader.h b/edgevisiontransformer_b200/csrc/loader.h
--- a/edgevisiontransformer_b200/csrc/loader.h
+++ b/edgevisiontransformer_b200/csrc/loader.h
@@ -29,6 +29,8 @@
     *out = static_cast<T*>(p);
     return mat_into(name, rows, cols, ld, p);
   }
+  int mat_fold_into(const std::string& name, int rows, int cols, int ld, const float* gamma, const float* beta, void* dst, float* bias,
+                    float* c);
   int mat_t(const std::string& name, int rows_out, int cols_out, int ld, __nv_bfloat16** out);
   template <typename T>
   int upload(const std::vector<T>& h, T** out) {
diff --git a/edgevisiontransformer_b200/csrc/model.cu b/edgevisiontransformer_b200/csrc/model.cu
--- a/edgevisiontransformer_b200/csrc/model.cu
+++ b/edgevisiontransformer_b200/csrc/model.cu
@@ -3,6 +3,7 @@
 #include <string>
 #include <vector>
 
+#include "ln_fold.cuh"
 #include "loader.h"
 #include "ops.h"
 #include "ptx.cuh"
@@ -44,12 +45,41 @@
   store_as(y + t, x[r * x_stride + c]);
 }
 
+__global__ void __launch_bounds__(256) fold_ln_weight_kernel(const float* __restrict__ W, const float* __restrict__ gamma,
+                                                             const float* __restrict__ beta, __nv_bfloat16* __restrict__ dst, float* bias,
+                                                             float* __restrict__ c, int rows, int cols, int ld) {
+  const int n = blockIdx.x * (blockDim.x >> 5) + (threadIdx.x >> 5);
+  const int lane = threadIdx.x & 31;
+  if (n >= rows) return;
+  double cs = 0.0, ds = 0.0;
+  for (int k = lane; k < ld; k += 32) {
+    float w = 0.f;
+    if (k < cols) {
+      w = W[static_cast<long long>(n) * cols + k];
+      ds += static_cast<double>(w) * beta[k];
+    }
+    const __nv_bfloat16 h = __float2bfloat16_rn(k < cols ? w * gamma[k] : 0.f);
+    dst[static_cast<long long>(n) * ld + k] = h;
+    cs += static_cast<double>(__bfloat162float(h));
+  }
+#pragma unroll
+  for (int o = 16; o > 0; o >>= 1) {
+    cs += __shfl_xor_sync(0xffffffffu, cs, o);
+    ds += __shfl_xor_sync(0xffffffffu, ds, o);
+  }
+  if (lane == 0) {
+    c[n] = static_cast<float>(cs);
+    bias[n] = static_cast<float>(ds + bias[n]);
+  }
+}
+
 inline int padn(int v, int n) { return (v + n - 1) / n * n; }
 
 struct LayerW {
   uint8_t *wqkv = nullptr, *wo = nullptr, *w1 = nullptr, *w2 = nullptr;
   float *bqkv = nullptr, *bo = nullptr, *b1 = nullptr, *b2 = nullptr;
   float *ln1_g = nullptr, *ln1_b = nullptr, *ln2_g = nullptr, *ln2_b = nullptr;
+  float *cqkv = nullptr, *c1 = nullptr;
   int a = 0, inter = 0, inter_ld = 0;
 };
 
@@ -70,6 +100,7 @@
   int patches = 0, n_prefix = 0, patch_k = 0;
   int es = 2;
   int pad = 8;
+  bool fold = false;
   std::vector<evt::LayerW> layers;
   uint8_t* w_patch = nullptr;
   float* b_patch = nullptr;
@@ -94,6 +125,7 @@
 struct Workspace {
   float* resid;
   uint8_t *xn, *qkv, *ctx, *big, *clsn, *hh;
+  float2* rec[2];
   uint8_t *t_x[2], *t_kqv[2], *t_ws[2], *t_pm;
   float* t_y[2];
   size_t bytes;
@@ -124,6 +156,7 @@
   w.big = c.take(std::max(M * imax_ld, (s.embed_k > 0 ? Mp : M) * static_cast<size_t>(m->patch_k)) * es);
   w.clsn = c.take(static_cast<size_t>(batch) * s.hidden * (s.head_rows > 1 ? s.head_rows : 1) * es);
   w.hh = c.take(static_cast<size_t>(batch) * std::max(padn(s.head_hidden, m->pad), 8) * es);
+  for (int i = 0; i < 2; ++i) w.rec[i] = m->fold ? c.take<float2>(M * ln_fold::record_len(s.hidden) * sizeof(float2)) : nullptr;
   if (s.t2t) {
     for (int i = 0; i < 2; ++i) {
       const size_t T = static_cast<size_t>(t2t_side(s.image, i)) * t2t_side(s.image, i) * batch;
@@ -242,6 +275,18 @@
   return EVT_OK;
 }
 
+int Loader::mat_fold_into(const std::string& name, int rows, int cols, int ld, const float* gamma, const float* beta, void* dst,
+                          float* bias, float* c) {
+  const evt_tensor_view* v;
+  EVT_TRY(need(name, static_cast<int64_t>(rows) * cols, &v));
+  EVT_CHECK_ARG(es == 2, "folded LayerNorm weights are bf16");
+  fold_ln_weight_kernel<<<static_cast<unsigned>((rows + 7) / 8), 256, 0, st>>>(static_cast<const float*>(v->data), gamma, beta,
+                                                                              static_cast<__nv_bfloat16*>(dst), bias, c, rows, cols, ld);
+  cudaError_t e = cudaGetLastError();
+  if (e != cudaSuccess) return fail(EVT_ERR_CUDA, std::string("fold_ln_weight: ") + cudaGetErrorString(e));
+  return EVT_OK;
+}
+
 int Loader::mat_t(const std::string& name, int rows_out, int cols_out, int ld, __nv_bfloat16** out) {
   const evt_tensor_view* v;
   EVT_TRY(need(name, static_cast<int64_t>(rows_out) * cols_out, &v));
@@ -283,6 +328,8 @@
   m->patch_k = spec->embed_k > 0 ? spec->embed_k : 3 * spec->patch * spec->patch;
   m->es = spec->precision == EVT_PREC_TF32 ? 4 : 2;
   m->pad = 16 / m->es;
+  m->fold = spec->dialect == EVT_DIALECT_HF && spec->precision == EVT_PREC_BF16 && spec->hidden > 384 && spec->hidden % 256 == 0 &&
+            spec->hidden <= 1024;
   m->layers.resize(spec->layers);
   *out = m;
   return EVT_OK;
@@ -320,27 +367,41 @@
     w.a = s.heads[l] * s.head_size;
     w.inter = s.inter[l];
     w.inter_ld = padn(w.inter, m->pad);
+    EVT_TRY(L.vec(p + "layernorm_before.weight", D, false, &w.ln1_g));
+    EVT_TRY(L.vec(p + "layernorm_before.bias", D, false, &w.ln1_b));
+    EVT_TRY(L.vec(p + "layernorm_after.weight", D, false, &w.ln2_g));
+    EVT_TRY(L.vec(p + "layernorm_after.bias", D, false, &w.ln2_b));
     void* q;
     EVT_TRY(L.alloc(static_cast<size_t>(3) * w.a * D * m->es, &q));
     w.wqkv = reinterpret_cast<uint8_t*>(q);
     EVT_TRY(L.alloc(static_cast<size_t>(3) * w.a * 4, &q));
     w.bqkv = reinterpret_cast<float*>(q);
+    if (m->fold) {
+      EVT_TRY(L.alloc(static_cast<size_t>(3) * w.a * 4, &q));
+      w.cqkv = reinterpret_cast<float*>(q);
+      EVT_TRY(L.alloc(static_cast<size_t>(w.inter) * 4, &q));
+      w.c1 = reinterpret_cast<float*>(q);
+    }
     const char* names[3] = {"query", "key", "value"};
     for (int t = 0; t < 3; ++t) {
       const std::string base = p + "attention.attention." + names[t];
-      EVT_TRY(L.mat_into(base + ".weight", w.a, D, D, w.wqkv + static_cast<size_t>(t) * w.a * D * m->es));
+      uint8_t* dst = w.wqkv + static_cast<size_t>(t) * w.a * D * m->es;
       EVT_TRY(L.vec_into(base + ".bias", w.a, true, w.bqkv + t * w.a));
+      if (m->fold) EVT_TRY(L.mat_fold_into(base + ".weight", w.a, D, D, w.ln1_g, w.ln1_b, dst, w.bqkv + t * w.a, w.cqkv + t * w.a));
+      else EVT_TRY(L.mat_into(base + ".weight", w.a, D, D, dst));
     }
     EVT_TRY(L.mat(p + "attention.output.dense.weight", D, w.a, w.a, &w.wo));
     EVT_TRY(L.vec(p + "attention.output.dense.bias", D, true, &w.bo));
-    EVT_TRY(L.mat(p + "intermediate.dense.weight", w.inter, D, D, &w.w1));
     EVT_TRY(L.vec(p + "intermediate.dense.bias", w.inter, true, &w.b1));
+    if (m->fold) {
+      EVT_TRY(L.alloc(static_cast<size_t>(w.inter) * D * m->es, &q));
+      w.w1 = reinterpret_cast<uint8_t*>(q);
+      EVT_TRY(L.mat_fold_into(p + "intermediate.dense.weight", w.inter, D, D, w.ln2_g, w.ln2_b, w.w1, w.b1, w.c1));
+    } else {
+      EVT_TRY(L.mat(p + "intermediate.dense.weight", w.inter, D, D, &w.w1));
+    }
     EVT_TRY(L.mat(p + "output.dense.weight", D, w.inter, w.inter_ld, &w.w2));
     EVT_TRY(L.vec(p + "output.dense.bias", D, true, &w.b2));
-    EVT_TRY(L.vec(p + "layernorm_before.weight", D, false, &w.ln1_g));
-    EVT_TRY(L.vec(p + "layernorm_before.bias", D, false, &w.ln1_b));
-    EVT_TRY(L.vec(p + "layernorm_after.weight", D, false, &w.ln2_g));
-    EVT_TRY(L.vec(p + "layernorm_after.bias", D, false, &w.ln2_b));
   }
   if (s.t2t) {
     for (int i = 0; i < 2; ++i) {
@@ -478,6 +539,28 @@
   const int64_t tok_stride = static_cast<int64_t>(s.tokens) * D;
   const bool cls_tail = !tf32 && s.head_rows <= 1 && !(o.ctx_out != nullptr && o.ctx_out[s.layers - 1] != nullptr);
   bool xn_ready = false;
+  int cur = 0;
+  bool have_rec = false;
+  auto ln_fold_rows = [&](const float* x, int64_t xs_stride, int64_t rec_in_rows, int64_t nrows) -> int {
+    EVT_TRY(ln_stats_launch(x, xs_stride, have_rec ? w.rec[cur] : nullptr, rec_in_rows, w.xn, D, w.rec[cur ^ 1], nrows, D, st));
+    cur ^= 1;
+    have_rec = true;
+    return EVT_OK;
+  };
+  auto write_through = [&](GemmOp op) {
+    op.ln_in = w.rec[cur];
+    op.ln_out = w.rec[cur ^ 1];
+    op.xs = w.xn;
+    op.ldxs = D;
+    return op;
+  };
+  auto folded = [&](GemmOp op, const float* c) {
+    if (!m->fold) return op;
+    op.ln_in = w.rec[cur];
+    op.ln_c = c;
+    op.ln_eps = s.eps;
+    return op;
+  };
   for (int l = 0; l < s.layers; ++l) {
     const LayerW& lw = m->layers[l];
     const int a = lw.a;
@@ -491,10 +574,12 @@
       op.ldr = op.ldo = rs;
       return op;
     };
-    if (!xn_ready)
-      EVT_STAGE(EVT_STAGE_LN, layernorm_launch(w.resid, D, lw.ln1_g, lw.ln1_b, w.xn, adt, D, tf ? w.resid : nullptr, M, D, s.eps, st));
-    EVT_STAGE(EVT_STAGE_QKV, gemm_launch({.A = w.xn, .lda = D, .W = lw.wqkv, .ldw = D, .in_dtype = dt, .bias = lw.bqkv, .out = w.qkv,
-                                          .out_dtype = adt, .ldo = 3 * a, .M = M, .N = 3 * a, .K = D}, st));
+    if (!xn_ready) {
+      if (m->fold) EVT_STAGE(EVT_STAGE_LN, ln_fold_rows(w.resid, D, 1, M));
+      else EVT_STAGE(EVT_STAGE_LN, layernorm_launch(w.resid, D, lw.ln1_g, lw.ln1_b, w.xn, adt, D, tf ? w.resid : nullptr, M, D, s.eps, st));
+    }
+    EVT_STAGE(EVT_STAGE_QKV, gemm_launch(folded({.A = w.xn, .lda = D, .W = lw.wqkv, .ldw = D, .in_dtype = dt, .bias = lw.bqkv, .out = w.qkv,
+                                                 .out_dtype = adt, .ldo = 3 * a, .M = M, .N = 3 * a, .K = D}, lw.cqkv), st));
     xn_ready = false;
     const float* hmask = o.head_mask != nullptr ? o.head_mask + static_cast<size_t>(l) * o.head_mask_ld : nullptr;
     EVT_CHECK_ARG(hmask == nullptr || o.head_mask_ld >= s.heads[l], "head_mask_ld smaller than a layer's head count");
@@ -506,24 +591,33 @@
     else
       EVT_STAGE(EVT_STAGE_ATTN, attention_launch(w.qkv, 3 * a, ctx, a, hmask, batch, s.tokens, tail ? 1 : s.tokens, s.heads[l], s.head_size,
                                                  scale, st));
+    const GemmOp oproj = on_rows({.A = ctx, .lda = a, .W = lw.wo, .ldw = a, .in_dtype = dt, .bias = lw.bo, .residual = w.resid, .ldr = D,
+                                  .out = w.resid, .out_dtype = EVT_F32, .ldo = D, .M = M, .N = D, .K = a});
     if (!tail && row_ln && gemm_rowln_pays(D, a, tf)) {
       EVT_STAGE(EVT_STAGE_OPROJ, gemm_rowln_launch(ctx, a, lw.wo, a, lw.bo, w.resid, D, lw.ln2_g, lw.ln2_b, s.eps, tf, w.xn, D, M, D, a, st));
+    } else if (m->fold && !tail && gemm_write_through_ok(oproj)) {
+      EVT_STAGE(EVT_STAGE_OPROJ, gemm_launch(write_through(oproj), st));
+      cur ^= 1;
     } else {
-      EVT_STAGE(EVT_STAGE_OPROJ, gemm_launch(on_rows({.A = ctx, .lda = a, .W = lw.wo, .ldw = a, .in_dtype = dt, .bias = lw.bo, .residual = w.resid,
-                                                      .ldr = D, .out = w.resid, .out_dtype = EVT_F32, .ldo = D, .M = M, .N = D, .K = a}), st));
-      EVT_STAGE(EVT_STAGE_LN, layernorm_launch(w.resid, rs, lw.ln2_g, lw.ln2_b, w.xn, adt, D, tf ? w.resid : nullptr, rows, D, s.eps, st));
-    }
-    EVT_STAGE(EVT_STAGE_FC1, gemm_launch({.A = w.xn, .lda = D, .W = lw.w1, .ldw = D, .in_dtype = dt, .bias = lw.b1, .out = w.big,
-                                          .out_dtype = adt, .ldo = lw.inter_ld, .M = rows, .N = lw.inter, .K = D, .act = s.act}, st));
-    if (row_ln && l + 1 < s.layers && gemm_rowln_pays(D, lw.inter, tf)) {
+      EVT_STAGE(EVT_STAGE_OPROJ, gemm_launch(oproj, st));
+      if (m->fold) EVT_STAGE(EVT_STAGE_LN, ln_fold_rows(w.resid, rs, tail ? s.tokens : 1, rows));
+      else EVT_STAGE(EVT_STAGE_LN, layernorm_launch(w.resid, rs, lw.ln2_g, lw.ln2_b, w.xn, adt, D, tf ? w.resid : nullptr, rows, D, s.eps, st));
+    }
+    EVT_STAGE(EVT_STAGE_FC1, gemm_launch(folded({.A = w.xn, .lda = D, .W = lw.w1, .ldw = D, .in_dtype = dt, .bias = lw.b1, .out = w.big,
+                                                 .out_dtype = adt, .ldo = lw.inter_ld, .M = rows, .N = lw.inter, .K = D, .act = s.act}, lw.c1), st));
+    const GemmOp fc2 = on_rows({.A = w.big, .lda = lw.inter_ld, .W = lw.w2, .ldw = lw.inter_ld, .in_dtype = dt, .bias = lw.b2, .residual = w.resid,
+                                .ldr = D, .out = w.resid, .out_dtype = EVT_F32, .ldo = D, .M = M, .N = D, .K = lw.inter});
+    if (m->fold && !tail && l + 1 < s.layers && gemm_write_through_ok(fc2)) {
+      EVT_STAGE(EVT_STAGE_FC2, gemm_launch(write_through(fc2), st));
+      cur ^= 1;
+      xn_ready = true;
+    } else if (row_ln && l + 1 < s.layers && gemm_rowln_pays(D, lw.inter, tf)) {
       const LayerW& nx = m->layers[l + 1];
       EVT_STAGE(EVT_STAGE_FC2, gemm_rowln_launch(w.big, lw.inter_ld, lw.w2, lw.inter_ld, lw.b2, w.resid, D, nx.ln1_g, nx.ln1_b, s.eps, tf, w.xn,
                                                  D, M, D, lw.inter, st));
       xn_ready = true;
     } else {
-      EVT_STAGE(EVT_STAGE_FC2, gemm_launch(on_rows({.A = w.big, .lda = lw.inter_ld, .W = lw.w2, .ldw = lw.inter_ld, .in_dtype = dt, .bias = lw.b2,
-                                                    .residual = w.resid, .ldr = D, .out = w.resid, .out_dtype = EVT_F32, .ldo = D, .M = M, .N = D,
-                                                    .K = lw.inter}), st));
+      EVT_STAGE(EVT_STAGE_FC2, gemm_launch(fc2, st));
     }
   }
   const int head_rows = s.head_rows > 1 ? s.head_rows : 1;
@@ -618,6 +712,35 @@
   return layernorm_launch(resid, ldr, gamma, beta, xn, EVT_BF16, ldxn, copy_ln ? resid : nullptr, M, N, eps, st);
 }
 
+extern "C" int evt_layernorm_fold_stats(const float* x, int64_t x_stride, const void* rec_in, int64_t rec_in_rows, void* xs, int64_t ldxs,
+                                        void* rec_out, int64_t rows, int D, evt_stream stream) {
+  int rc = evt_device_check();
+  if (rc != EVT_OK) return rc;
+  return ln_stats_launch(x, x_stride, static_cast<const float2*>(rec_in), rec_in_rows, xs, ldxs, static_cast<float2*>(rec_out), rows, D,
+                         static_cast<cudaStream_t>(stream));
+}
+
+extern "C" int evt_gemm_layernorm_folded(const void* xs, int64_t ldxs, const void* W, int64_t ldw, const float* c, const float* d,
+                                         const void* rec, float eps, void* out, int64_t ldo, int64_t M, int N, int K, int act,
+                                         evt_stream stream) {
+  int rc = evt_device_check();
+  if (rc != EVT_OK) return rc;
+  EVT_CHECK_ARG(c != nullptr && rec != nullptr, "gemm_layernorm_folded: null pointer");
+  return gemm_launch({.A = xs, .lda = ldxs, .W = W, .ldw = ldw, .bias = d, .out = out, .ldo = ldo, .M = M, .N = N, .K = K, .act = act,
+                      .ln_in = static_cast<const float2*>(rec), .ln_c = c, .ln_eps = eps}, static_cast<cudaStream_t>(stream));
+}
+
+extern "C" int evt_gemm_residual_write_through(const void* A, int64_t lda, const void* W, int64_t ldw, const float* bias, float* resid,
+                                               int64_t ldr, const void* rec_in, void* rec_out, void* xs, int64_t ldxs, int64_t M, int N,
+                                               int K, evt_stream stream) {
+  int rc = evt_device_check();
+  if (rc != EVT_OK) return rc;
+  EVT_CHECK_ARG(resid != nullptr && xs != nullptr, "gemm_residual_write_through: null pointer");
+  return gemm_launch({.A = A, .lda = lda, .W = W, .ldw = ldw, .bias = bias, .residual = resid, .ldr = ldr, .out = resid, .out_dtype = EVT_F32,
+                      .ldo = ldr, .M = M, .N = N, .K = K, .ln_in = static_cast<const float2*>(rec_in), .ln_out = static_cast<float2*>(rec_out),
+                      .xs = xs, .ldxs = ldxs}, static_cast<cudaStream_t>(stream));
+}
+
 extern "C" int evt_gemm_residual_layernorm(const void* A, int64_t lda, const void* W, int64_t ldw, const float* bias, float* resid,
                                            int64_t ldr, const float* gamma, const float* beta, float eps, void* xn, int64_t ldxn,
                                            int64_t M, int N, int K, evt_stream stream) {
diff --git a/edgevisiontransformer_b200/csrc/ops.h b/edgevisiontransformer_b200/csrc/ops.h
--- a/edgevisiontransformer_b200/csrc/ops.h
+++ b/edgevisiontransformer_b200/csrc/ops.h
@@ -24,8 +24,15 @@
   int act = EVT_ACT_NONE;
   RowMap map = {};
   int max_k_splits = 0;
+  const float2* ln_in = nullptr;
+  float2* ln_out = nullptr;
+  const float* ln_c = nullptr;
+  void* xs = nullptr;
+  int64_t ldxs = 0;
+  float ln_eps = 0.f;
 };
 int gemm_launch(const GemmOp& op, cudaStream_t stream);
+bool gemm_write_through_ok(const GemmOp& op);
 int gemm_k_splits(const GemmOp& op);
 
 bool gemm_rowln_supported(int64_t M, int N, int K, bool copy_ln);
@@ -42,6 +49,8 @@
 
 int layernorm_launch(const float* x, int64_t x_stride, const float* gamma, const float* beta, void* y, int y_dtype,
                      int64_t y_stride, float* y_copy, int64_t rows, int D, float eps, cudaStream_t st);
+int ln_stats_launch(const float* x, int64_t x_stride, const float2* rec_in, int64_t rec_in_rows, void* xs, int64_t ldxs, float2* rec_out,
+                    int64_t rows, int D, cudaStream_t st);
 
 int im2col_launch(const void* pixels, int pixel_dtype, const float* scale3, const float* bias3, void* cols, int out_dtype, int B,
                   int H, int W, int P, cudaStream_t st, int row_stride = 0, int row_off = 0);
diff --git a/edgevisiontransformer_b200/ops.py b/edgevisiontransformer_b200/ops.py
--- a/edgevisiontransformer_b200/ops.py
+++ b/edgevisiontransformer_b200/ops.py
@@ -154,6 +154,46 @@
                                             float(eps), int(copy_ln), xn.data_ptr(), xn.stride(0), M, N, K, _stream())
     _lib.check(rc, "gemm_residual_layernorm")
     return xn
+
+
+def _records(rows: int, D: int, device) -> torch.Tensor:
+    return torch.empty((rows, 2 * (D // 128 + 1)), dtype=torch.float32, device=device)
+
+
+def layernorm_fold_stats(x: torch.Tensor, rec_in: Optional[torch.Tensor] = None):
+    _need_cuda(x, rec_in)
+    if x.dtype != torch.float32 or x.dim() != 2 or x.stride(1) != 1:
+        raise ValueError("layernorm_fold_stats wants 2-D f32 rows with unit inner stride")
+    M, D = x.shape
+    xs = torch.empty((M, D), dtype=torch.bfloat16, device=x.device)
+    rec = _records(M, D, x.device)
+    _lib.check(_lib.load().evt_layernorm_fold_stats(x.data_ptr(), x.stride(0), _ptr(rec_in), 1, xs.data_ptr(), D, rec.data_ptr(), M, D,
+                                                    _stream()), "layernorm_fold_stats")
+    return xs, rec
+
+
+def linear_layernorm_folded(xs: torch.Tensor, rec: torch.Tensor, w_folded: torch.Tensor, c: torch.Tensor, d: torch.Tensor, eps: float,
+                            act: int = _lib.ACT_NONE) -> torch.Tensor:
+    _need_cuda(xs, rec, w_folded, c, d)
+    M, K = xs.shape
+    N = w_folded.shape[0]
+    out = torch.empty((M, N), dtype=torch.bfloat16, device=xs.device)
+    _lib.check(_lib.load().evt_gemm_layernorm_folded(xs.data_ptr(), xs.stride(0), w_folded.data_ptr(), w_folded.stride(0),
+                                                     c.contiguous().data_ptr(), d.contiguous().data_ptr(), rec.data_ptr(), float(eps),
+                                                     out.data_ptr(), N, M, N, K, int(act), _stream()), "gemm_layernorm_folded")
+    return out
+
+
+def linear_residual_write_through(a: torch.Tensor, w: torch.Tensor, bias: Optional[torch.Tensor], resid: torch.Tensor,
+                                  rec_in: torch.Tensor):
+    _need_cuda(a, w, bias, resid, rec_in)
+    M, N = resid.shape
+    xs = torch.empty((M, N), dtype=torch.bfloat16, device=a.device)
+    rec = _records(M, N, a.device)
+    _lib.check(_lib.load().evt_gemm_residual_write_through(a.data_ptr(), a.stride(0), w.data_ptr(), w.stride(0), _ptr(bias),
+                                                           resid.data_ptr(), resid.stride(0), rec_in.data_ptr(), rec.data_ptr(),
+                                                           xs.data_ptr(), N, M, N, a.shape[1], _stream()), "gemm_residual_write_through")
+    return xs, rec
 
 
 def attention(qkv: torch.Tensor, B: int, S: int, heads: int, head_size: int = 64, scale: Optional[float] = None,
diff --git a/include/evt.h b/include/evt.h
--- a/include/evt.h
+++ b/include/evt.h
@@ -62,6 +62,14 @@
 int evt_gemm_residual_layernorm_ex(const void* A, int64_t lda, const void* W, int64_t ldw, const float* bias,
                                    float* resid, int64_t ldr, const float* gamma, const float* beta, float eps, int copy_ln,
                                    void* xn, int64_t ldxn, int64_t M, int N, int K, evt_stream stream);
+
+int evt_layernorm_fold_stats(const float* x, int64_t x_stride, const void* rec_in, int64_t rec_in_rows, void* xs, int64_t ldxs,
+                             void* rec_out, int64_t rows, int D, evt_stream stream);
+int evt_gemm_layernorm_folded(const void* xs, int64_t ldxs, const void* W, int64_t ldw, const float* c, const float* d, const void* rec,
+                              float eps, void* out, int64_t ldo, int64_t M, int N, int K, int act, evt_stream stream);
+int evt_gemm_residual_write_through(const void* A, int64_t lda, const void* W, int64_t ldw, const float* bias, float* resid,
+                                    int64_t ldr, const void* rec_in, void* rec_out, void* xs, int64_t ldxs, int64_t M, int N, int K,
+                                    evt_stream stream);
 
 #define EVT_ATTN_MAX_TOKENS 1026
 
```

Result: slower. 26100, median of 6 (-3.3%).
